# matiasrodlo/arxiv-rag

Measured on AMD Instinct MI355X. Metric: chunks embedded/sec + QPS@top-10, all-mpnet-base-v2 768-d, 1/2/4/8 MI355X, higher is better.
Workload: dtype bf16

## Files before the change

arxiv_rag_amd/_lib.py:

```python
from __future__ import annotations

import ctypes as C
import os
from pathlib import Path

_HERE = Path(__file__).resolve().parent
LIB_PATH = Path(os.environ.get("ARX_LIB", _HERE / "libarx_hip.so"))

K_CLASSES = ["search_groupmax", "gemm_qkv", "gemm_oproj", "gemm_fc1", "gemm_fc2", "attention",
             "layernorm", "embed", "pool", "search_select", "search_rescore", "gemm_raw"]


class EncoderConfigC(C.Structure):
    _fields_ = [(n, C.c_int32) for n in ("arch", "vocab_size", "hidden", "layers", "heads", "ffn", "max_pos",
                                         "pool", "pad_id", "rel_buckets", "rel_max_distance")] + [("ln_eps", C.c_float)]


class LayerWeightsC(C.Structure):
    _fields_ = [(n, C.c_void_p) for n in ("w_qkv", "b_qkv", "w_o", "b_o", "ln1_g", "ln1_b",
                                          "w_fc1", "b_fc1", "w_fc2", "b_fc2", "ln2_g", "ln2_b")]


class EncoderWeightsC(C.Structure):
    _fields_ = [(n, C.c_void_p) for n in ("word_emb", "pos_emb", "type_emb", "emb_ln_g", "emb_ln_b", "rel_bias")] \
               + [("layers", C.POINTER(LayerWeightsC))]


class TopkOptionsC(C.Structure):
    _fields_ = [("struct_bytes", C.c_int32), ("i8_max_queries", C.c_int32), ("max_row_norm", C.c_float), ("cu_limit", C.c_int32),
                ("flags", C.c_int32), ("debug_tau_mult", C.c_float), ("debug_drop_best", C.c_int32)]

    def __init__(self, **kw):
        super().__init__(**kw)
        self.struct_bytes = C.sizeof(TopkOptionsC)


class PairHeadC(C.Structure):
    _fields_ = [("struct_bytes", C.c_int32), ("n_labels", C.c_int32)] \
               + [(n, C.c_void_p) for n in ("type_emb", "pooler_w", "pooler_b", "cls_w", "cls_b")]

    def __init__(self, **kw):
        super().__init__(**kw)
        self.struct_bytes = C.sizeof(PairHeadC)


class GemmEpilogueC(C.Structure):
    _fields_ = [("struct_bytes", C.c_int32), ("mode", C.c_int32), ("variant", C.c_int32), ("eps", C.c_float)] \
               + [(n, C.c_void_p) for n in ("bias", "resid", "a_mean", "a_rstd", "s_vec", "r_mean", "r_rstd", "r_gamma", "r_beta")] \
               + [("row_cap", C.c_int64), ("part_sum", C.c_void_p), ("part_sq", C.c_void_p), ("part_ld", C.c_int64),
                  ("out_mean", C.c_void_p), ("out_rstd", C.c_void_p), ("n_rows", C.c_void_p)]

    def __init__(self, **kw):
        super().__init__(**kw)
        self.struct_bytes = C.sizeof(GemmEpilogueC)


TOPK_NO_PERSISTENT, TOPK_SCAN_ONLY, TOPK_TAIL_ONLY, TOPK_NO_SINGLE_ROW_TAIL, TOPK_I8_CENTRE_QUERY = 1, 2, 4, 8, 16


EXPORTS = {
    "arx_version": (C.c_int32, []),
    "arx_last_error": (C.c_char_p, []),
    "arx_build_info": (C.c_int32, []),
    "arx_mpnet_bucket": (C.c_int32, [C.c_int32, C.c_int32, C.c_int32]),
    "arx_encoder_workspace_bytes": (C.c_int64, [C.POINTER(EncoderConfigC), C.c_int32, C.c_int32]),
    "arx_encoder_create": (C.c_int32, [C.POINTER(EncoderConfigC), C.POINTER(EncoderWeightsC), C.c_int32, C.c_int32,
                                       C.POINTER(C.c_void_p)]),
    "arx_encoder_destroy": (None, [C.c_void_p]),
    "arx_encoder_forward": (C.c_int32, [C.c_void_p, C.c_void_p, C.c_int32, C.c_void_p, C.c_int32, C.c_int32, C.c_int32,
                                        C.c_void_p, C.c_int64, C.c_void_p, C.c_int64, C.c_int32, C.c_void_p]),
    "arx_encoder_attention": (C.c_int32, [C.c_void_p, C.c_void_p, C.c_void_p, C.c_int32, C.c_int32, C.c_void_p, C.c_void_p]),
    "arx_encoder_set_tap": (C.c_int32, [C.c_void_p, C.c_int32]),
    "arx_encoder_set_low_latency": (C.c_int32, [C.c_void_p, C.c_int32]),
    "arx_encoder_debug_hidden": (C.c_int32, [C.c_void_p, C.c_int32, C.c_void_p, C.c_int32, C.c_void_p]),
    "arx_encoder_set_pair_head": (C.c_int32, [C.c_void_p, C.POINTER(PairHeadC)]),
    "arx_encoder_score_pairs": (C.c_int32, [C.c_void_p, C.c_void_p, C.c_int32, C.c_void_p, C.c_void_p, C.c_int32, C.c_int32, C.c_int32,
                                            C.c_void_p, C.c_int64, C.c_void_p]),
    "arx_encoder_debug_cls": (C.c_int32, [C.c_void_p, C.c_void_p, C.c_int32, C.c_void_p]),
    "arx_pair_head_forward": (C.c_int32, [C.c_void_p, C.c_int64, C.c_int32, C.c_int32, C.POINTER(PairHeadC), C.c_void_p, C.c_int64,
                                          C.c_void_p]),
    "arx_topk_workspace_bytes": (C.c_int64, [C.c_int64, C.c_int32, C.c_int32, C.c_int32]),
    "arx_topk_search": (C.c_int32, [C.c_void_p, C.c_int64, C.c_void_p, C.c_int32, C.c_int32, C.c_int32, C.c_void_p,
                                    C.c_void_p, C.c_int64, C.c_void_p, C.c_int64, C.c_void_p]),
    "arx_topk_i8_index_bytes": (C.c_int64, [C.c_int64, C.c_int32]),
    "arx_topk_i8_index_info": (C.c_int32, [C.c_void_p, C.c_int64, C.c_int32, C.POINTER(C.c_float), C.c_void_p]),
    "arx_topk_build_i8": (C.c_int32, [C.c_void_p, C.c_int64, C.c_int32, C.c_void_p, C.c_void_p]),
    "arx_topk_search_i8": (C.c_int32, [C.c_void_p, C.c_void_p, C.c_int64, C.c_void_p, C.c_int32, C.c_int32, C.c_int32, C.c_void_p,
                                       C.c_void_p, C.c_int64, C.c_void_p, C.c_int64, C.c_void_p]),
    "arx_topk_workspace_bytes_i8": (C.c_int64, [C.c_int64, C.c_int32, C.c_int32, C.c_int32]),
    "arx_topk_search_opt": (C.c_int32, [C.c_void_p, C.c_void_p, C.c_int64, C.c_void_p, C.c_int32, C.c_int32, C.c_int32, C.c_void_p,
                                        C.c_void_p, C.c_int64, C.c_void_p, C.c_int64, C.POINTER(TopkOptionsC), C.c_void_p]),
    "arx_rows_max_norm_f16": (C.c_int32, [C.c_void_p, C.c_int64, C.c_int32, C.c_void_p, C.c_void_p]),
    "arx_stream_create_cu_mask": (C.c_int32, [C.POINTER(C.c_uint32), C.c_int32, C.POINTER(C.c_void_p)]),
    "arx_stream_destroy": (C.c_int32, [C.c_void_p]),
    "arx_device_cu_count": (C.c_int32, []),
    "arx_debug_cu_census": (C.c_int32, [C.c_void_p, C.c_int32, C.c_int32, C.c_void_p]),
    "arx_topk_stats": (C.c_int32, [C.c_void_p, C.POINTER(C.c_int64), C.POINTER(C.c_int64), C.c_void_p]),
    "arx_topk_merge": (C.c_int32, [C.c_void_p, C.c_void_p, C.c_int32, C.c_int32, C.c_int32, C.c_void_p, C.c_void_p,
                                   C.c_void_p]),
    "arx_topk_filtered_workspace_bytes": (C.c_int64, [C.c_int64, C.c_int32, C.c_int32, C.c_int32]),
    "arx_topk_search_filtered": (C.c_int32, [C.c_void_p, C.c_int64, C.c_void_p, C.c_int64, C.c_void_p, C.c_int32, C.c_int32, C.c_int32,
                                             C.c_void_p, C.c_void_p, C.c_int64, C.c_float, C.c_void_p, C.c_int64, C.c_void_p]),
    "arx_topk_search_filtered_tuned": (C.c_int32, [C.c_void_p, C.c_int64, C.c_void_p, C.c_int64, C.c_void_p, C.c_int32, C.c_int32, C.c_int32,
                                                   C.c_void_p, C.c_void_p, C.c_int64, C.c_float, C.c_void_p, C.c_int64, C.c_int32, C.c_int32,
                                                   C.c_void_p]),
    "arx_topk_filtered_stats": (C.c_int32, [C.c_void_p, C.POINTER(C.c_int64), C.POINTER(C.c_int64), C.c_void_p]),
    "arx_topk_prefix_workspace_bytes": (C.c_int64, [C.c_int64, C.c_int32, C.c_int32, C.c_int32]),
    "arx_topk_search_prefix": (C.c_int32, [C.c_void_p, C.c_int64, C.c_void_p, C.c_void_p, C.c_int32, C.c_int32, C.c_int32, C.c_void_p,
                                           C.c_void_p, C.c_int64, C.c_float, C.c_void_p, C.c_int64, C.c_void_p]),
    "arx_topk_search_prefix_tuned": (C.c_int32, [C.c_void_p, C.c_int64, C.c_void_p, C.c_void_p, C.c_int32, C.c_int32, C.c_int32, C.c_void_p,
                                                 C.c_void_p, C.c_int64, C.c_float, C.c_void_p, C.c_int64, C.c_int32, C.c_int32, C.c_void_p]),
    "arx_topk_prefix_stats": (C.c_int32, [C.c_void_p, C.POINTER(C.c_int64), C.POINTER(C.c_int64), C.c_void_p]),
    "arx_text_contains": (C.c_int32, [C.c_void_p, C.c_void_p, C.c_int64, C.c_void_p, C.c_void_p, C.c_int32, C.c_void_p, C.c_void_p]),
    "arx_bitmap_count": (C.c_int32, [C.c_void_p, C.c_int64, C.c_void_p, C.c_void_p]),
    "arx_gather_rows": (C.c_int32, [C.c_void_p, C.c_int64, C.c_int32, C.c_int64, C.c_void_p, C.c_int64, C.c_void_p, C.c_void_p]),
    "arx_mmr_select": (C.c_int32, [C.c_void_p, C.c_void_p, C.c_void_p, C.c_int32, C.c_int32, C.c_int32, C.c_int32, C.c_float, C.c_void_p,
                                   C.c_void_p, C.c_void_p]),
    "arx_bm25_workspace_bytes": (C.c_int64, [C.c_int64, C.c_int32, C.c_int32]),
    "arx_bm25_search": (C.c_int32, [C.c_void_p, C.c_void_p, C.c_void_p, C.c_int32, C.c_int64, C.c_void_p, C.c_void_p, C.c_int32, C.c_int32,
                                    C.c_void_p, C.c_void_p, C.c_int64, C.c_void_p, C.c_int64, C.c_void_p]),
    "arx_bm25_search_tuned": (C.c_int32, [C.c_void_p, C.c_void_p, C.c_void_p, C.c_int32, C.c_int64, C.c_void_p, C.c_void_p, C.c_int32,
                                          C.c_int32, C.c_void_p, C.c_void_p, C.c_int64, C.c_void_p, C.c_int64, C.c_int32, C.c_int32,
                                          C.c_void_p]),
    "arx_bm25_scores": (C.c_int32, [C.c_void_p, C.c_void_p, C.c_void_p, C.c_int32, C.c_int64, C.c_void_p, C.c_int32, C.c_int64, C.c_int64,
                                    C.c_int32, C.c_void_p, C.c_void_p]),
    "arx_gemm_bf16": (C.c_int32, [C.c_void_p, C.c_void_p, C.c_void_p, C.c_void_p, C.c_void_p, C.c_int32, C.c_int32, C.c_int32,
                                  C.c_int32, C.c_int32, C.c_void_p]),
    "arx_gemm_bf16_ex": (C.c_int32, [C.c_void_p, C.c_void_p, C.c_void_p, C.c_int32, C.c_int32, C.c_int32, C.POINTER(GemmEpilogueC),
                                     C.c_void_p]),
    "arx_fold_ln": (C.c_int32, [C.c_void_p, C.c_void_p, C.c_void_p, C.c_void_p, C.c_void_p, C.c_void_p, C.c_void_p, C.c_int32, C.c_int32,
                                C.c_void_p]),
    "arx_prof_classes": (C.c_int32, [C.c_uint32]),
    "arx_wp_create": (C.c_int32, [C.c_char_p, C.c_void_p, C.c_int32, C.c_int32, C.c_int32, C.c_int32, C.c_int32, C.c_int32, C.c_int32,
                                  C.c_char_p, C.c_void_p, C.c_int32, C.POINTER(C.c_void_p)]),
    "arx_wp_destroy": (None, [C.c_void_p]),
    "arx_wp_encode": (C.c_int32, [C.c_void_p, C.c_char_p, C.c_void_p, C.c_int64, C.c_int32, C.c_void_p, C.c_void_p, C.c_void_p, C.c_int32]),
    "arx_wp_miss_count": (C.c_int32, [C.c_void_p, C.POINTER(C.c_int64), C.POINTER(C.c_int64)]),
    "arx_wp_miss_fetch": (C.c_int32, [C.c_void_p, C.c_void_p, C.c_void_p]),
    "arx_wp_cache_add": (C.c_int32, [C.c_void_p, C.c_char_p, C.c_void_p, C.c_int64, C.c_void_p, C.c_void_p]),
    "arx_wp_cache_size": (C.c_int64, [C.c_void_p]),
    "arx_wp_version": (C.c_int32, []),
    "arx_adjacent_cosine": (C.c_int32, [C.c_void_p, C.c_int64, C.c_int32, C.c_int32, C.c_void_p, C.c_void_p]),
    "arx_f32_to_bf16": (C.c_int32, [C.c_void_p, C.c_void_p, C.c_int64, C.c_void_p]),
    "arx_fill_unit_rows_f16": (C.c_int32, [C.c_void_p, C.c_int64, C.c_int32, C.c_uint64, C.c_void_p]),
    "arx_fill_unit_rows_f16_at": (C.c_int32, [C.c_void_p, C.c_int64, C.c_int32, C.c_uint64, C.c_int64, C.c_void_p]),
    "arx_fill_clustered_rows_f16_at": (C.c_int32, [C.c_void_p, C.c_int64, C.c_int32, C.c_uint64, C.c_int64, C.c_int32, C.c_float, C.c_int32,
                                                   C.c_float, C.c_void_p]),
    "arx_prof_enable": (C.c_int32, [C.c_int32]),
    "arx_prof_reset": (C.c_int32, []),
    "arx_prof_read": (C.c_int32, [C.c_int32, C.POINTER(C.c_float), C.POINTER(C.c_int32)]),
}

_lib = None


class ArxError(RuntimeError):
    pass


def load():
    global _lib
    if _lib is not None:
        return _lib
    if not LIB_PATH.exists():
        raise ArxError(
            f"{LIB_PATH} not found: the HIP extension is not built. Run `python -c 'import __graft_entry__ as g; "
            f"g.build()'` (or arxiv_rag_amd/csrc/build.sh). There is no CPU fallback for this path.")
    lib = C.CDLL(str(LIB_PATH))
    for name, (res, args) in EXPORTS.items():
        fn = getattr(lib, name)
        fn.restype = res
        fn.argtypes = args
    _lib = lib
    return lib


def check(rc: int, what: str = ""):
    if rc != 0:
        msg = load().arx_last_error().decode("utf-8", "replace")
        raise ArxError(f"{what} failed (rc={rc}): {msg}")


def prof_classes(names=None):
    mask = 0xFFFFFFFF if names is None else sum(1 << K_CLASSES.index(n) for n in names)
    check(load().arx_prof_classes(mask), "arx_prof_classes")


def prof_enable(on: bool):
    check(load().arx_prof_enable(1 if on else 0), "arx_prof_enable")


def prof_reset():
    check(load().arx_prof_reset(), "arx_prof_reset")


def prof_read():
    lib = load()
    out = {}
    for i, name in enumerate(K_CLASSES):
        ms, n = C.c_float(0), C.c_int32(0)
        check(lib.arx_prof_read(i, C.byref(ms), C.byref(n)), "arx_prof_read")
        out[name] = (float(ms.value), int(n.value))
    return out
```

arxiv_rag_amd/csrc/encoder.hip:

```cpp
#include <math.h>
#include <stdlib.h>
#include <string.h>

#include <mutex>
#include <vector>

#include "arx_common.h"
#include "encoder_kernels.h"
#include "gemm.h"
#include "gemm8.h"
#include "gemm_small.h"

extern "C" int32_t arx_mpnet_bucket(int32_t rel, int32_t num_buckets, int32_t max_distance) {
    int n = -rel;
    const int nb = num_buckets / 2;
    int ret = 0;
    if (n < 0) { ret = nb; n = -n; }
    const int max_exact = nb / 2;
    if (n < max_exact) return ret + n;
    int v = max_exact + (int)floor(log((double)n / max_exact) / log((double)max_distance / max_exact) * (nb - max_exact) + 1e-6);
    if (v > nb - 1) v = nb - 1;
    return ret + v;
}

struct arx_encoder {
    arx_encoder_config cfg;
    arx_encoder_weights w;
    std::vector<arx_layer_weights> layers;
    int max_tokens, max_seqs, tok_pad;
    char* ws = nullptr;
    int64_t ws_bytes = 0;
    int32_t* cu = nullptr;
    uint16_t *x = nullptr, *x1 = nullptr, *qkv = nullptr, *ctx = nullptr, *y = nullptr, *hbuf = nullptr;
    float* bias_tbl = nullptr;
    uint16_t* tap = nullptr;
    int tap_layer = -1;
    int ln_fold = 1;
    char* fold_ws = nullptr;
    std::vector<uint16_t*> wqkv_f, wfc1_f;
    std::vector<float*> s_qkv, c_qkv, s_fc1, c_fc1;
    float *st1_sum = nullptr, *st1_sq = nullptr, *st2_sum = nullptr, *st2_sq = nullptr;
    float *part_s = nullptr, *part_q = nullptr;
    int variant = 89;
    int low_latency = 0;
    float* small_ws = nullptr;
    int attn_variant = 1;
    int attn_dev_word = 0;
    unsigned long long* attn_stamps = nullptr;
    arx_pair_head pair{};
    int has_pair = 0;
    float* cls_ws = nullptr;
};

struct WsLayout {
    int64_t cu, x, x1, qkv, ctx, y, hbuf, bias, stats, total;
};
static WsLayout ws_layout(const arx_encoder_config& c, int max_tokens, int max_seqs) {
    const int64_t tp = round_up64(max_tokens, 256);
    WsLayout l;
    int64_t o = 0;
    auto take = [&](int64_t bytes) { int64_t r = o; o += round_up64(bytes, 256); return r; };
    l.cu = take((int64_t)(max_seqs + 1) * 4);
    l.x = take(tp * c.hidden * 2);
    l.x1 = take(tp * c.hidden * 2);
    l.qkv = take(tp * c.hidden * 3 * 2);
    l.ctx = take(tp * c.hidden * 2);
    l.y = take(tp * c.hidden * 2);
    l.hbuf = take(tp * c.ffn * 2);
    l.bias = take((int64_t)c.heads * ARX_BIAS_ROW * 4);
    l.stats = take(tp * 4 * 4 + 2 * (int64_t)(c.hidden / 64) * tp * 4);
    l.total = o;
    return l;
}

static int check_cfg(const arx_encoder_config* c) {
    ARX_REQUIRE(c != nullptr, "cfg is null");
    ARX_REQUIRE(c->arch == ARX_ARCH_MPNET || c->arch == ARX_ARCH_BERT, "unknown arch %d", c->arch);
    ARX_REQUIRE(c->hidden > 0 && c->hidden % 64 == 0 && c->hidden <= 1024, "hidden=%d must be a multiple of 64, <= 1024", c->hidden);
    ARX_REQUIRE(c->heads > 0 && c->hidden % c->heads == 0, "hidden %% heads != 0");
    const int dh = c->hidden / c->heads;
    ARX_REQUIRE(dh == 32 || dh == 64, "head_dim=%d unsupported (32 or 64)", dh);
    ARX_REQUIRE(c->ffn > 0 && c->ffn % 64 == 0, "ffn=%d must be a multiple of 64", c->ffn);
    ARX_REQUIRE(c->layers > 0 && c->vocab_size > 0 && c->max_pos > 0, "bad layers/vocab/max_pos");
    ARX_REQUIRE(c->pool == ARX_POOL_MEAN || c->pool == ARX_POOL_CLS, "unknown pool %d", c->pool);
    return ARX_OK;
}

extern "C" int64_t arx_encoder_workspace_bytes(const arx_encoder_config* cfg, int32_t max_tokens, int32_t max_seqs) {
    if (check_cfg(cfg) != ARX_OK || max_tokens <= 0 || max_seqs <= 0) return -1;
    return ws_layout(*cfg, max_tokens, max_seqs).total;
}

extern "C" int32_t arx_encoder_create(const arx_encoder_config* cfg, const arx_encoder_weights* w, int32_t max_tokens,
                                      int32_t max_seqs, arx_encoder** out) {
    int rc = check_cfg(cfg);
    if (rc != ARX_OK) return rc;
    ARX_REQUIRE(w && out, "null weights/out");
    ARX_REQUIRE(max_tokens > 0 && max_seqs > 0, "max_tokens/max_seqs must be positive");
    ARX_REQUIRE(w->word_emb && w->pos_emb && w->emb_ln_g && w->emb_ln_b && w->layers, "missing embedding weights");
    ARX_REQUIRE(cfg->arch != ARX_ARCH_BERT || w->type_emb, "BERT needs type_emb");
    ARX_REQUIRE(cfg->arch != ARX_ARCH_MPNET || w->rel_bias, "MPNet needs rel_bias");
    for (int i = 0; i < cfg->layers; ++i) {
        const arx_layer_weights& L = w->layers[i];
        ARX_REQUIRE(L.w_qkv && L.b_qkv && L.w_o && L.b_o && L.ln1_g && L.ln1_b && L.w_fc1 && L.b_fc1 && L.w_fc2 &&
                        L.b_fc2 && L.ln2_g && L.ln2_b, "layer %d: missing weights", i);
    }
    arx_encoder* h = new arx_encoder();
    auto fail = [&](int code) {
        if (h->ws) (void)hipFree(h->ws);
        if (h->fold_ws) (void)hipFree(h->fold_ws);
        delete h;
        return code;
    };
    h->cfg = *cfg;
    h->w = *w;
    h->layers.assign(w->layers, w->layers + cfg->layers);
    h->w.layers = h->layers.data();
    h->max_tokens = max_tokens;
    h->max_seqs = max_seqs;
    h->tok_pad = (int)round_up64(max_tokens, 256);
    const char* e = getenv("ARX_GEMM_VARIANT");
    h->variant = e ? atoi(e) : 89;
    const char* av = getenv("ARX_ATTN_VARIANT");
    h->attn_variant = av ? atoi(av) : 1;
#ifdef ARX_DEV_VARIANTS
    const char* g = getenv("ARX_GEMM_GLDS");
    if (g && g[0] == '0') h->variant = 4;
#endif
    const WsLayout l = ws_layout(*cfg, max_tokens, max_seqs);
    hipError_t he = hipMalloc((void**)&h->ws, l.total);
    if (he != hipSuccess) {
        arx_set_error("hipMalloc(%lld bytes workspace): %s", (long long)l.total, hipGetErrorString(he));
        h->ws = nullptr;
        return fail(ARX_ERR_HIP);
    }
    h->ws_bytes = l.total;
    (void)hipMemset(h->ws, 0, l.total);
    h->cu = (int32_t*)(h->ws + l.cu);
    h->x = (uint16_t*)(h->ws + l.x);
    h->x1 = (uint16_t*)(h->ws + l.x1);
    h->qkv = (uint16_t*)(h->ws + l.qkv);
    h->ctx = (uint16_t*)(h->ws + l.ctx);
    h->y = (uint16_t*)(h->ws + l.y);
    h->hbuf = (uint16_t*)(h->ws + l.hbuf);
    h->bias_tbl = (float*)(h->ws + l.bias);
    {
        const int64_t tp = round_up64(max_tokens, 256);
        float* st = (float*)(h->ws + l.stats);
        h->st1_sum = st; h->st1_sq = st + tp; h->st2_sum = st + 2 * tp; h->st2_sq = st + 3 * tp;
        h->part_s = st + 4 * tp; h->part_q = h->part_s + (int64_t)(cfg->hidden / 64) * tp;
    }
    const char* lf = getenv("ARX_LN_FOLD");
    h->ln_fold = lf ? atoi(lf) : 1;
    if (h->ln_fold) {
        const int64_t H = cfg->hidden, F = cfg->ffn, Lc = cfg->layers;
        const int64_t per = round_up64(3 * H * H * 2, 256) + round_up64(F * H * 2, 256) + 2 * round_up64(3 * H * 4, 256) + 2 * round_up64(F * 4, 256);
        he = hipMalloc((void**)&h->fold_ws, per * Lc);
        if (he != hipSuccess) {
            arx_set_error("hipMalloc(folded weights): %s", hipGetErrorString(he));
            h->fold_ws = nullptr;
            return fail(ARX_ERR_HIP);
        }
        char* pws = h->fold_ws;
        auto takep = [&](int64_t bytes) { char* r = pws; pws += round_up64(bytes, 256); return r; };
        for (int i = 0; i < Lc; ++i) {
            const arx_layer_weights& L = h->layers[i];
            uint16_t* wq = (uint16_t*)takep(3 * H * H * 2); uint16_t* w1 = (uint16_t*)takep(F * H * 2);
            float* sq = (float*)takep(3 * H * 4); float* cq = (float*)takep(3 * H * 4);
            float* s1 = (float*)takep(F * 4); float* c1 = (float*)takep(F * 4);
            h->wqkv_f.push_back(wq); h->wfc1_f.push_back(w1);
            h->s_qkv.push_back(sq); h->c_qkv.push_back(cq); h->s_fc1.push_back(s1); h->c_fc1.push_back(c1);
            fold_ln_kernel<<<cdiv(F, 4), 256>>>((const uint16_t*)L.w_fc1, L.ln1_g, L.ln1_b, L.b_fc1, w1, s1, c1, (int)F, (int)H);
            if (i > 0) {
                const arx_layer_weights& P = h->layers[i - 1];
                fold_ln_kernel<<<cdiv(3 * H, 4), 256>>>((const uint16_t*)L.w_qkv, P.ln2_g, P.ln2_b, L.b_qkv, wq, sq, cq, (int)(3 * H), (int)H);
            }
        }
        he = hipDeviceSynchronize();
        if (he != hipSuccess) {
            arx_set_error("fold_ln_kernel: %s", hipGetErrorString(he));
            return fail(ARX_ERR_HIP);
        }
    }
    if (cfg->arch == ARX_ARCH_MPNET) {
        std::vector<float> rb((size_t)cfg->rel_buckets * cfg->heads);
        he = hipMemcpy(rb.data(), w->rel_bias, rb.size() * 4, hipMemcpyDeviceToHost);
        if (he != hipSuccess) {
            arx_set_error("copy rel_bias: %s", hipGetErrorString(he));
            return fail(ARX_ERR_HIP);
        }
        std::vector<float> tbl((size_t)cfg->heads * ARX_BIAS_ROW);
        const float log2e = 1.4426950408889634f;
        for (int d = -ARX_BIAS_CENTER; d <= ARX_BIAS_CENTER; ++d) {
            const int bk = arx_mpnet_bucket(d, cfg->rel_buckets, cfg->rel_max_distance);
            for (int hd = 0; hd < cfg->heads; ++hd)
                tbl[(size_t)hd * ARX_BIAS_ROW + d + ARX_BIAS_CENTER] = rb[(size_t)bk * cfg->heads + hd] * log2e;
        }
        he = hipMemcpy(h->bias_tbl, tbl.data(), tbl.size() * 4, hipMemcpyHostToDevice);
        if (he != hipSuccess) {
            arx_set_error("upload bias table: %s", hipGetErrorString(he));
            return fail(ARX_ERR_HIP);
        }
    }
    *out = h;
    return ARX_OK;
}

extern "C" void arx_encoder_destroy(arx_encoder* h) {
    if (!h) return;
    if (h->ws) (void)hipFree(h->ws);
    if (h->tap) (void)hipFree(h->tap);
    if (h->fold_ws) (void)hipFree(h->fold_ws);
    if (h->small_ws) (void)hipFree(h->small_ws);
    if (h->cls_ws) (void)hipFree(h->cls_ws);
    delete h;
}

extern "C" int32_t arx_encoder_set_low_latency(arx_encoder* h, int32_t on) {
    ARX_REQUIRE(h, "null handle");
    if (on && !h->small_ws) ARX_HIP_CHECK(hipMalloc((void**)&h->small_ws, ARX_SMALL_WS_BYTES));
    h->low_latency = on ? 1 : 0;
    return ARX_OK;
}

extern "C" int32_t arx_encoder_set_tap(arx_encoder* h, int32_t layer) {
    ARX_REQUIRE(h, "null handle");
    ARX_REQUIRE(layer >= -1 && layer <= h->cfg.layers, "tap layer out of range");
    if (layer >= 0 && !h->tap) ARX_HIP_CHECK(hipMalloc((void**)&h->tap, (int64_t)h->tok_pad * h->cfg.hidden * 2));
    h->tap_layer = layer;
    return ARX_OK;
}

extern "C" int32_t arx_encoder_debug_hidden(arx_encoder* h, int32_t , float* dst, int32_t n_tokens, void* stream) {
    ARX_REQUIRE(h && h->tap && dst, "no tap recorded");
    ARX_REQUIRE(n_tokens > 0 && n_tokens <= h->max_tokens, "n_tokens out of range");
    const int64_t n = (int64_t)n_tokens * h->cfg.hidden;
    bf16_to_f32_kernel<<<cdiv(n, 256), 256, 0, (hipStream_t)stream>>>(h->tap, dst, n);
    ARX_HIP_CHECK(hipGetLastError());
    return ARX_OK;
}

template <typename Kern>
static int launch_gemm_kernel(Kern kern, int smem, int threads, int BM, int BN, const uint16_t* A, int64_t lda,
                              const uint16_t* W, int64_t ldw, int M, int N, int K, const EpiParams& ep, hipStream_t st) {
    ARX_HIP_CHECK(arx_func_smem((const void*)kern, smem));
    const int tm = cdiv(M, BM), tn = cdiv(N, BN);
    kern<<<tm * tn, threads, smem, st>>>((const bf16_t*)A, lda, (const bf16_t*)W, ldw, M, N, K, tm, tn, ep);
    ARX_HIP_CHECK(hipGetLastError());
    return ARX_OK;
}

static bool fits_u32_offsets(int64_t M, int64_t lda, int64_t N, int64_t ldw, const EpiParams& ep) {
    return M * lda < (1ll << 31) && N * ldw < (1ll << 31) && M * ep.ldc < (1ll << 32) && (!ep.resid || M * ep.ldr < (1ll << 32));
}

template <int MODE>
int arx_launch_gemm(int variant, const uint16_t* A, int64_t lda, const uint16_t* W, int64_t ldw, int M, int N, int K,
                    const EpiParams& ep, hipStream_t st) {
    if (K % 64 != 0 || N % 8 != 0) {
        arx_set_error("gemm: K=%d must be a multiple of 64 and N=%d of 8", K, N);
        return ARX_ERR_ARG;
    }
    const bool wide = (N % 256 == 0);
    const bool wide8 = (N % 128 == 0 && N >= 256);
#ifdef ARX_DEV_VARIANTS
    if constexpr (MODE <= EPI_BIAS_RESID) {
        if (variant == 0) {
            if (wide) return launch_gemm_kernel(gemm_bf16_kernel<256, 256, 2, 4, true, MODE>, GemmMainloop<bf16_t, 256, 256, 2, 4, true>::SMEM_BYTES, 512, 256, 256, A, lda, W, ldw, M, N, K, ep, st);
            return launch_gemm_kernel(gemm_bf16_kernel<256, 128, 4, 2, true, MODE>, GemmMainloop<bf16_t, 256, 128, 4, 2, true>::SMEM_BYTES, 512, 256, 128, A, lda, W, ldw, M, N, K, ep, st);
        }
        if (variant == 4) {
            if (wide) return launch_gemm_kernel(gemm_bf16_kernel<256, 256, 2, 4, false, MODE>, GemmMainloop<bf16_t, 256, 256, 2, 4, false>::SMEM_BYTES, 512, 256, 256, A, lda, W, ldw, M, N, K, ep, st);
            return launch_gemm_kernel(gemm_bf16_kernel<256, 128, 4, 2, false, MODE>, GemmMainloop<bf16_t, 256, 128, 4, 2, false>::SMEM_BYTES, 512, 256, 128, A, lda, W, ldw, M, N, K, ep, st);
        }
    }
#endif
    if (variant == 71)
        return launch_gemm_kernel(gemm_v0e2_kernel<128, 128, 2, 2, MODE, 67>, GemmMainloop<bf16_t, 128, 128, 2, 2, true, 67>::SMEM_BYTES, 256, 128, 128, A, lda, W, ldw, M, N, K, ep, st);
    if (variant == 89) variant = (K <= 1024) ? 9 : 8;
    if (variant == 9 && (K / 64) % 2 != 0) variant = 8;
    if ((variant == 8 || variant == 9) && wide8 && !fits_u32_offsets(M, lda, N, ldw, ep)) {
        static bool said = false;
        if (!said) {
            said = true;
            fprintf(stderr, "[arx] gemm M=%d N=%d K=%d: operand or output offsets exceed 32 bits, using the 2-stage kernel (64-bit offsets)\n", M, N, K);
        }
        variant = 13;
    }
    if (variant == 9 && wide8) {
        auto kern = gemm_8phase_persistent_kernel<MODE>;
        ARX_HIP_CHECK(arx_func_smem((const void*)kern, Gemm8Phase<bf16_t, 0>::SMEM_BYTES));
        const int n_cu = arx_device_cus();
        const int tm = cdiv(M, 256), tn = cdiv(N, 256);
        int grid = TileWalk::grid(tm, tn) < n_cu ? TileWalk::grid(tm, tn) : n_cu;
        grid = grid / 8 * 8 > 0 ? grid / 8 * 8 : grid;
        kern<<<grid, 512, Gemm8Phase<bf16_t, 0>::SMEM_BYTES, st>>>((const bf16_t*)A, lda, (const bf16_t*)W, ldw, M, N, K, tm, tn, ep);
        ARX_HIP_CHECK(hipGetLastError());
        return ARX_OK;
    }
    if (variant == 8 && wide8) {
        auto kern = gemm_8phase_kernel<MODE>;
        ARX_HIP_CHECK(arx_func_smem((const void*)kern, Gemm8Phase<bf16_t, 0>::SMEM_BYTES));
        const int tm = cdiv(M, 256), tn = cdiv(N, 256);
        kern<<<TileWalk::grid(tm, tn), 512, Gemm8Phase<bf16_t, 0>::SMEM_BYTES, st>>>((const bf16_t*)A, lda, (const bf16_t*)W, ldw, M, N, K, tm, tn, ep);
        ARX_HIP_CHECK(hipGetLastError());
        return ARX_OK;
    }
#ifdef ARX_DEV_VARIANTS
    if (variant == 34 && wide)
        return launch_gemm_kernel(gemm_v0e2_kernel<256, 256, 2, 4, MODE, 64 + 4096>, GemmMainloop<bf16_t, 256, 256, 2, 4, true, 64 + 4096>::SMEM_BYTES, 512, 256, 256, A, lda, W, ldw, M, N, K, ep, st);
    if (variant == 33 && wide)
        return launch_gemm_kernel(gemm_a3w2_kernel<256, 256, 2, 4, MODE>, 3 * 256 * 128 + 2 * 256 * 128, 512, 256, 256, A, lda, W, ldw, M, N, K, ep, st);
    if (variant == 1) {
        if (wide) return launch_gemm_kernel(gemm_v0e2_kernel<256, 256, 2, 4, MODE>, GemmMainloop<bf16_t, 256, 256, 2, 4, true>::SMEM_BYTES, 512, 256, 256, A, lda, W, ldw, M, N, K, ep, st);
        return launch_gemm_kernel(gemm_v0e2_kernel<256, 128, 4, 2, MODE>, GemmMainloop<bf16_t, 256, 128, 4, 2, true>::SMEM_BYTES, 512, 256, 128, A, lda, W, ldw, M, N, K, ep, st);
    }
    if (variant == 15 && wide)
        return launch_gemm_kernel(gemm_v0e2_kernel<256, 256, 2, 4, MODE, 3>, GemmMainloop<bf16_t, 256, 256, 2, 4, true, 3>::SMEM_BYTES, 512, 256, 256, A, lda, W, ldw, M, N, K, ep, st);
    if (variant == 3 && wide)
        return launch_gemm_kernel(gemm_ring_kernel<256, 256, 2, 4, 4, MODE>, GemmRing<bf16_t, 256, 256, 2, 4, 4>::SMEM_BYTES, 512, 256, 256, A, lda, W, ldw, M, N, K, ep, st);
    if (variant == 2 || variant == 3)
        return launch_gemm_kernel(gemm_ring_kernel<256, 128, 2, 2, 3, MODE>, GemmRing<bf16_t, 256, 128, 2, 2, 3>::SMEM_BYTES, 256, 256, 128, A, lda, W, ldw, M, N, K, ep, st);
#endif
    if (!wide) return launch_gemm_kernel(gemm_v0e2_kernel<256, 128, 4, 2, MODE, 67>, GemmMainloop<bf16_t, 256, 128, 4, 2, true, 67>::SMEM_BYTES, 512, 256, 128, A, lda, W, ldw, M, N, K, ep, st);
    return launch_gemm_kernel(gemm_v0e2_kernel<256, 256, 2, 4, MODE, 67>, GemmMainloop<bf16_t, 256, 256, 2, 4, true, 67>::SMEM_BYTES, 512, 256, 256, A, lda, W, ldw, M, N, K, ep, st);
}

template <int MODE>
static int launch_gemm(int cls, int variant, const uint16_t* A, int64_t lda, const uint16_t* W, int64_t ldw, int M, int N, int K,
                       const EpiParams& ep, hipStream_t st, float* small_ws = nullptr) {
    ProfScope ps(cls, st);
    if (variant == 70) return launch_gemm_small<MODE>(A, lda, W, ldw, M, N, K, ep, small_ws, st);
#ifdef ARX_DEV_VARIANTS
    static const int dev_bw = getenv("ARX_DEV_BW") ? atoi(getenv("ARX_DEV_BW")) : 0;
    const char* stg = getenv("ARX_DEV_STAGGER");
    if (dev_bw || stg) {
        EpiParams e2 = ep; e2.dev_bw = dev_bw;
        if (stg) { int a = 0, b = 8, c = 0; sscanf(stg, "%d,%d,%d", &a, &b, &c); e2.dev_stagger = a; e2.dev_slots = b > 0 ? b : 8; e2.dev_store = c; }
        return arx_launch_gemm<MODE>(variant, A, lda, W, ldw, M, N, K, e2, st);
    }
#endif
    return arx_launch_gemm<MODE>(variant, A, lda, W, ldw, M, N, K, ep, st);
}

extern "C" int32_t arx_gemm_bf16(const void* A, const void* W, const float* bias, const void* resid, void* C, int32_t M,
                                 int32_t N, int32_t K, int32_t mode, int32_t variant, void* stream) {
    ARX_REQUIRE(A && W && bias && C, "null pointer argument");
    ARX_REQUIRE(M > 0 && N > 0 && K > 0, "bad sizes");
    ARX_REQUIRE(mode != EPI_BIAS_RESID || resid, "mode 2 needs resid");
    EpiParams ep{(uint16_t*)C, N, bias, (const uint16_t*)resid, N};
    hipStream_t st = (hipStream_t)stream;
#ifdef ARX_DEV_VARIANTS
    ep.dev_store = (variant / 100) % 10; ep.dev_bw = variant / 1000; variant %= 100;
    if (const char* stg = getenv("ARX_DEV_STAGGER")) { int a = 0, b = 8; sscanf(stg, "%d,%d", &a, &b); ep.dev_stagger = a; ep.dev_slots = b > 0 ? b : 8; }
#endif
#ifdef ARX_STAMP
    {
        static unsigned long long* d = nullptr;
        const int tiles = cdiv(M, 256) * cdiv(N, 256);
        if (!d) ARX_HIP_CHECK(hipMalloc(&d, (size_t)8 * 32 * 2 * 16384));
        if (getenv("ARX_STAMP_DUMP") && tiles <= 16384) {
            ep.stamps = d;
            int rc = ARX_ERR_ARG;
            if (mode == EPI_BIAS) rc = arx_launch_gemm<EPI_BIAS>(variant, (const uint16_t*)A, K, (const uint16_t*)W, K, M, N, K, ep, st);
            if (mode == EPI_BIAS_GELU) rc = arx_launch_gemm<EPI_BIAS_GELU>(variant, (const uint16_t*)A, K, (const uint16_t*)W, K, M, N, K, ep, st);
            if (mode == EPI_BIAS_RESID) rc = arx_launch_gemm<EPI_BIAS_RESID>(variant, (const uint16_t*)A, K, (const uint16_t*)W, K, M, N, K, ep, st);
            ARX_HIP_CHECK(hipStreamSynchronize(st));
            std::vector<unsigned long long> hbuf((size_t)tiles * 64);
            ARX_HIP_CHECK(hipMemcpy(hbuf.data(), d, hbuf.size() * 8, hipMemcpyDeviceToHost));
            double loop[2] = {0, 0}, epi[2] = {0, 0}, pro[2] = {0, 0}, x45[2] = {0, 0}, x67[2] = {0, 0};
            unsigned long long tmin = ~0ull, tmax = 0;
            for (int t = 0; t < tiles; ++t)
                for (int g = 0; g < 2; ++g) {
                    const unsigned long long* o = &hbuf[((size_t)t * 2 + g) * 32];
                    loop[g] += (double)(o[1] - o[3]); epi[g] += (double)(o[2] - o[1]); pro[g] += (double)(o[3] - o[0]);
                    if (variant == 9) { x45[g] += (double)(o[5] - o[4]); x67[g] += (double)(o[7] - o[6]); }
                    else x45[g] += (double)(o[4] - o[2]);
                    tmin = o[0] < tmin ? o[0] : tmin; tmax = o[2] > tmax ? o[2] : tmax;
                }
            if (variant == 9) {
                double gap = 0, period = 0; int n = 0;
                for (int t = 0; t + 256 < tiles; ++t) { const unsigned long long* a = &hbuf[(size_t)t * 64]; const unsigned long long* b = &hbuf[(size_t)(t + 256) * 64];
                    gap += (double)(b[0] - a[2]); period += (double)(b[0] - a[0]); ++n; }
                if (n) fprintf(stderr, "[stamp] persistent: g0 tile period %.0f clk, epilogue-end -> next loop start %.0f clk\n", period / n, gap / n);
            }
            if (const char* sf = getenv("ARX_STAMP_FILE")) {
                if (FILE* f = fopen(sf, "wb")) { fwrite(hbuf.data(), 8, hbuf.size(), f); fclose(f); }
            }
            if (variant == 9) {
                const int nkt = K / 64 < 16 ? K / 64 : 16;
                fprintf(stderr, "[stamp] k-tile durations g0:");
                for (int k = 0; k + 1 < nkt; ++k) { double a = 0; int n = 0; for (int t = 256; t < tiles; ++t) { const unsigned long long* o = &hbuf[(size_t)t * 64]; a += (double)(o[9 + k] - o[8 + k]); ++n; } fprintf(stderr, " %.0f", a / (n ? n : 1)); }
                fprintf(stderr, "\n");
            }
            fprintf(stderr, "[stamp] %s g0 %.0f g1 %.0f clk%s g0 %.0f g1 %.0f\n", variant == 9 ? "wait at k-tile 0:" : "store drain after the epilogue:", x45[0] / tiles, x45[1] / tiles,
                    variant == 9 ? ", at k-tile 1:" : " (-)", x67[0] / tiles, x67[1] / tiles);
            fprintf(stderr, "[stamp] M=%d N=%d K=%d mode=%d tiles=%d: prologue %.0f / %.0f, loop g0 %.0f g1 %.0f clk, epilogue g0 %.0f g1 %.0f clk, span %.0f clk, tiles/CU %.1f\n",
                    M, N, K, mode, tiles, pro[0] / tiles, pro[1] / tiles, loop[0] / tiles, loop[1] / tiles, epi[0] / tiles, epi[1] / tiles, (double)(tmax - tmin), tiles / 256.0);
            return rc;
        }
    }
#endif
    ProfScope ps(ARX_K_GEMM_RAW, st);
    if (variant == 70) {
        float* ws = nullptr;
        ARX_HIP_CHECK(hipMallocAsync((void**)&ws, ARX_SMALL_WS_BYTES, st));
        int rc = ARX_ERR_ARG;
        switch (mode) {
        case EPI_BIAS: rc = launch_gemm_small<EPI_BIAS>((const uint16_t*)A, K, (const uint16_t*)W, K, M, N, K, ep, ws, st); break;
        case EPI_BIAS_GELU: rc = launch_gemm_small<EPI_BIAS_GELU>((const uint16_t*)A, K, (const uint16_t*)W, K, M, N, K, ep, ws, st); break;
        case EPI_BIAS_RESID: rc = launch_gemm_small<EPI_BIAS_RESID>((const uint16_t*)A, K, (const uint16_t*)W, K, M, N, K, ep, ws, st); break;
        default: arx_set_error("unknown gemm mode %d", mode);
        }
        (void)hipFreeAsync(ws, st);
        return rc;
    }
    switch (mode) {
    case EPI_BIAS: return arx_launch_gemm<EPI_BIAS>(variant, (const uint16_t*)A, K, (const uint16_t*)W, K, M, N, K, ep, st);
    case EPI_BIAS_GELU: return arx_launch_gemm<EPI_BIAS_GELU>(variant, (const uint16_t*)A, K, (const uint16_t*)W, K, M, N, K, ep, st);
    case EPI_BIAS_RESID: return arx_launch_gemm<EPI_BIAS_RESID>(variant, (const uint16_t*)A, K, (const uint16_t*)W, K, M, N, K, ep, st);
    }
    arx_set_error("unknown gemm mode %d", mode);
    return ARX_ERR_ARG;
}

template <int DH, bool HB, int NW>
static int launch_attn_cfg(arx_encoder* h, int n_seqs, int max_len, hipStream_t st) {
    auto kern = attention_kernel<DH, HB, NW>;
    const int Lk = (max_len + 31) & ~31;
    const int smem = AttnSmem<DH>::total(Lk, HB);
    ARX_HIP_CHECK(arx_func_smem((const void*)kern, smem));
    const float scale_log2e = 1.4426950408889634f / sqrtf((float)DH);
    dim3 grid(cdiv(max_len, 32 * NW), h->cfg.heads, n_seqs);
    ProfScope ps(ARX_K_ATTENTION, st);
    kern<<<grid, NW * 64, smem, st>>>(h->qkv, h->ctx, h->cu, h->bias_tbl, h->cfg.hidden, scale_log2e);
    ARX_HIP_CHECK(hipGetLastError());
    return ARX_OK;
}

template <int DH, bool HB, int NW>
static int launch_attn_tr_cfg(arx_encoder* h, int n_seqs, int max_len, hipStream_t st) {
    auto kern = attention_tr_kernel<DH, HB, NW>;
    const int Lk = (max_len + 31) & ~31;
    const int smem = AttnSmem3<DH>::total(Lk, HB);
    ARX_HIP_CHECK(arx_func_smem((const void*)kern, smem));
    const float scale_log2e = 1.4426950408889634f / sqrtf((float)DH);
    dim3 grid(cdiv(max_len, 32 * NW), h->cfg.heads, n_seqs);
    ProfScope ps(ARX_K_ATTENTION, st);
    kern<<<grid, NW * 64, smem, st>>>(h->qkv, h->ctx, h->cu, h->bias_tbl, h->cfg.hidden, scale_log2e, h->attn_dev_word, h->attn_stamps);
    ARX_HIP_CHECK(hipGetLastError());
    return ARX_OK;
}

#ifdef ARX_DEV_VARIANTS
template <int DH, bool HB, int NSLOT>
static int launch_attn_ring_cfg(arx_encoder* h, int n_seqs, int max_len, hipStream_t st) {
    auto kern = attention_ring_kernel<DH, HB, NSLOT>;
    const int C0 = (max_len + 31) & ~31;
    const int smem = AttnRing<DH, NSLOT>::total(C0, HB);
    ARX_HIP_CHECK(arx_func_smem((const void*)kern, smem));
    int G = arx_device_cus() / h->cfg.heads;
    G = G < 1 ? 1 : (G > n_seqs ? n_seqs : G);
    const float scale_log2e = 1.4426950408889634f / sqrtf((float)DH);
    ProfScope ps(ARX_K_ATTENTION, st);
    kern<<<G * h->cfg.heads, 512, smem, st>>>(h->qkv, h->ctx, h->cu, h->bias_tbl, h->cfg.hidden, n_seqs, C0, scale_log2e);
    ARX_HIP_CHECK(hipGetLastError());
    return ARX_OK;
}

template <bool HB>
static int launch_attn_ring16_cfg(arx_encoder* h, int n_seqs, int max_len, hipStream_t st) {
    auto kern = attention_ring16_kernel<HB>;
    const int C0 = (max_len + 31) & ~31;
    const int smem = AttnRing16<8>::total(C0, HB);
    ARX_HIP_CHECK(arx_func_smem((const void*)kern, smem));
    int G = arx_device_cus() / h->cfg.heads;
    G = G < 1 ? 1 : (G > n_seqs ? n_seqs : G);
    const float scale_log2e = 1.4426950408889634f / sqrtf(64.0f);
    ProfScope ps(ARX_K_ATTENTION, st);
    kern<<<G * h->cfg.heads, 1024, smem, st>>>(h->qkv, h->ctx, h->cu, h->bias_tbl, h->cfg.hidden, n_seqs, C0, scale_log2e);
    ARX_HIP_CHECK(hipGetLastError());
    return ARX_OK;
}

#endif

static int launch_attn(arx_encoder* h, int n_seqs, int max_len, hipStream_t st) {
    const int dh = h->cfg.hidden / h->cfg.heads;
    const bool hb = h->cfg.arch == ARX_ARCH_MPNET;
#ifdef ARX_DEV_VARIANTS
    if (h->attn_variant == 4 && dh == 64 && max_len > 128 && max_len <= 256)
        return hb ? launch_attn_ring16_cfg<true>(h, n_seqs, max_len, st) : launch_attn_ring16_cfg<false>(h, n_seqs, max_len, st);
    if (h->attn_variant == 2 && max_len > 128 && max_len <= 256) {
        if (dh == 64) return hb ? launch_attn_ring_cfg<64, true, 8>(h, n_seqs, max_len, st) : launch_attn_ring_cfg<64, false, 8>(h, n_seqs, max_len, st);
        return hb ? launch_attn_ring_cfg<32, true, 8>(h, n_seqs, max_len, st) : launch_attn_ring_cfg<32, false, 8>(h, n_seqs, max_len, st);
    }
#endif
    if (h->attn_variant >= 1) {
        const bool w8 = max_len > 128;
        if (dh == 64) {
            if (hb) return w8 ? launch_attn_tr_cfg<64, true, 8>(h, n_seqs, max_len, st) : launch_attn_tr_cfg<64, true, 4>(h, n_seqs, max_len, st);
            return w8 ? launch_attn_tr_cfg<64, false, 8>(h, n_seqs, max_len, st) : launch_attn_tr_cfg<64, false, 4>(h, n_seqs, max_len, st);
        }
        if (hb) return w8 ? launch_attn_tr_cfg<32, true, 8>(h, n_seqs, max_len, st) : launch_attn_tr_cfg<32, true, 4>(h, n_seqs, max_len, st);
        return w8 ? launch_attn_tr_cfg<32, false, 8>(h, n_seqs, max_len, st) : launch_attn_tr_cfg<32, false, 4>(h, n_seqs, max_len, st);
    }
    const bool big = max_len > 256;
    if (dh == 64) {
        if (hb) return big ? launch_attn_cfg<64, true, 8>(h, n_seqs, max_len, st) : launch_attn_cfg<64, true, 4>(h, n_seqs, max_len, st);
        return big ? launch_attn_cfg<64, false, 8>(h, n_seqs, max_len, st) : launch_attn_cfg<64, false, 4>(h, n_seqs, max_len, st);
    }
    if (hb) return big ? launch_attn_cfg<32, true, 8>(h, n_seqs, max_len, st) : launch_attn_cfg<32, true, 4>(h, n_seqs, max_len, st);
    return big ? launch_attn_cfg<32, false, 8>(h, n_seqs, max_len, st) : launch_attn_cfg<32, false, 4>(h, n_seqs, max_len, st);
}

extern "C" int32_t arx_encoder_attention(arx_encoder* h, const void* qkv, const int32_t* lens, int32_t n_seqs, int32_t max_len,
                                         void* ctx, void* stream) {
    ARX_REQUIRE(h && qkv && lens && ctx, "null pointer argument");
    ARX_REQUIRE(n_seqs > 0 && n_seqs <= h->max_seqs && max_len > 0 && max_len <= 512, "bad n_seqs/max_len");
    hipStream_t st = (hipStream_t)stream;
    scan_lens_kernel<<<1, 256, 0, st>>>(lens, h->cu, n_seqs);
    ARX_HIP_CHECK(hipGetLastError());
    uint16_t* q0 = h->qkv; uint16_t* c0 = h->ctx;
    h->qkv = (uint16_t*)qkv; h->ctx = (uint16_t*)ctx;
    const int rc = launch_attn(h, n_seqs, max_len, st);
    h->qkv = q0; h->ctx = c0;
    return rc;
}

static void launch_ln_finalize(int T, int nparts, const float* ps, const float* pq, int64_t ld, const int32_t* n_rows, float inv_h,
                               float eps, float* mean, float* rstd, hipStream_t st) {
    const int grid = cdiv(T, 256);
    switch (nparts) {
    case 6: ln_finalize_kernel<6><<<grid, 256, 0, st>>>(ps, pq, ld, nparts, n_rows, inv_h, eps, mean, rstd); break;
    case 12: ln_finalize_kernel<12><<<grid, 256, 0, st>>>(ps, pq, ld, nparts, n_rows, inv_h, eps, mean, rstd); break;
    case 16: ln_finalize_kernel<16><<<grid, 256, 0, st>>>(ps, pq, ld, nparts, n_rows, inv_h, eps, mean, rstd); break;
    default: ln_finalize_kernel<0><<<grid, 256, 0, st>>>(ps, pq, ld, nparts, n_rows, inv_h, eps, mean, rstd); break;
    }
}

template <int MODE>
static int gemm_ex_run(int variant, const uint16_t* A, const uint16_t* W, int M, int N, int K, const EpiParams& ep, const arx_gemm_epilogue* e,
                       hipStream_t st) {
    constexpr bool STATS = (MODE == EPI_RESID_STATS || MODE == EPI_LNRESID_STATS);
    int rc;
    if (variant == 70) {
        float* ws = nullptr;
        ARX_HIP_CHECK(hipMallocAsync((void**)&ws, ARX_SMALL_WS_BYTES, st));
        rc = launch_gemm<MODE>(ARX_K_GEMM_RAW, variant, A, K, W, K, M, N, K, ep, st, ws);
        (void)hipFreeAsync(ws, st);
        return rc;
    }
    if ((rc = launch_gemm<MODE>(ARX_K_GEMM_RAW, variant, A, K, W, K, M, N, K, ep, st)) != ARX_OK) return rc;
    if (STATS) {
        launch_ln_finalize(M, N / 64, e->part_sum, e->part_sq, e->part_ld, e->n_rows, ep.inv_h, ep.eps, e->out_mean, e->out_rstd, st);
        ARX_HIP_CHECK(hipGetLastError());
    }
    return ARX_OK;
}

extern "C" int32_t arx_gemm_bf16_ex(const void* A, const void* W, void* C, int32_t M, int32_t N, int32_t K, const arx_gemm_epilogue* e,
                                    void* stream) {
    ARX_REQUIRE(A && W && C && e, "null pointer argument");
    ARX_REQUIRE(e->struct_bytes == (int32_t)sizeof(arx_gemm_epilogue), "arx_gemm_epilogue: struct_bytes=%d, this library expects %d",
                e->struct_bytes, (int)sizeof(arx_gemm_epilogue));
    ARX_REQUIRE(M > 0 && N > 0 && K > 0, "bad sizes");
    ARX_REQUIRE(K % 64 == 0 && N % 8 == 0, "gemm: K=%d must be a multiple of 64 and N=%d of 8", K, N);
    const int mode = e->mode, variant = e->variant;
    ARX_REQUIRE(mode >= EPI_BIAS && mode <= EPI_LNRESID_STATS, "unknown gemm mode %d", mode);
    ARX_REQUIRE(variant == 89 || variant == 8 || variant == 9 || variant == 13 || variant == 70 || variant == 71,
                "gemm variant %d is not a shipped schedule (89, 8, 9, 13, 70, 71)", variant);
    const bool ln_in = (mode == EPI_LN_BIAS || mode == EPI_LN_BIAS_GELU), stats = (mode == EPI_RESID_STATS || mode == EPI_LNRESID_STATS);
    const bool staged = (variant == 89 || variant == 8 || variant == 9);
    ARX_REQUIRE(e->bias, "mode %d needs bias", mode);
    ARX_REQUIRE(!(mode == EPI_BIAS_RESID || stats) || e->resid, "mode %d needs resid", mode);
    ARX_REQUIRE(!ln_in || (e->a_mean && e->a_rstd && e->s_vec), "mode %d needs a_mean, a_rstd and s_vec", mode);
    ARX_REQUIRE(mode != EPI_LNRESID_STATS || (e->r_mean && e->r_rstd && e->r_gamma && e->r_beta), "mode 6 needs r_mean, r_rstd, r_gamma and r_beta");
    if (ln_in || mode == EPI_LNRESID_STATS)
        ARX_REQUIRE(e->row_cap >= (staged ? round_up64(M, 256) : (int64_t)M),
                    "row_cap=%lld: the row vectors must be readable up to row %lld (M=%d%s)", (long long)e->row_cap,
                    (long long)(staged ? round_up64(M, 256) : (int64_t)M), M, staged ? " rounded up to 256: variants 89, 8, 9 stage whole tiles" : "");
    if (stats) {
        ARX_REQUIRE(N % 64 == 0, "statistics modes need N %% 64 == 0 (one partial per 64-column slice), N=%d", N);
        ARX_REQUIRE(e->out_mean && e->out_rstd, "mode %d needs out_mean and out_rstd", mode);
        if (variant != 70) ARX_REQUIRE(e->part_sum && e->part_sq && e->part_ld >= M && e->n_rows,
                                       "mode %d on a tile kernel needs part_sum, part_sq, part_ld >= M and n_rows", mode);
    }
    if (variant == 70) {
        ARX_REQUIRE(M <= ARX_SMALL_M && N % 64 == 0, "small-batch gemm: M=%d (<= %d) N=%d (%% 64)", M, ARX_SMALL_M, N);
        ARX_REQUIRE(!stats || N <= 1024, "small-batch gemm: statistics modes take N <= 1024, N=%d", N);
    }
    EpiParams ep{(uint16_t*)C, N, e->bias, (const uint16_t*)e->resid, N};
    ep.a_sum = e->a_mean; ep.a_sq = e->a_rstd; ep.s_vec = e->s_vec;
    ep.r_sum = e->r_mean; ep.r_sq = e->r_rstd; ep.r_gamma = e->r_gamma; ep.r_beta = e->r_beta;
    ep.o_sum = e->part_sum; ep.o_sq = e->part_sq; ep.o_ld = e->part_ld;
    ep.fin_mean = e->out_mean; ep.fin_rstd = e->out_rstd;
    ep.inv_h = 1.0f / (float)N; ep.eps = e->eps;
    hipStream_t st = (hipStream_t)stream;
    const uint16_t* a = (const uint16_t*)A; const uint16_t* w = (const uint16_t*)W;
    switch (mode) {
    case EPI_BIAS: return gemm_ex_run<EPI_BIAS>(variant, a, w, M, N, K, ep, e, st);
    case EPI_BIAS_GELU: return gemm_ex_run<EPI_BIAS_GELU>(variant, a, w, M, N, K, ep, e, st);
    case EPI_BIAS_RESID: return gemm_ex_run<EPI_BIAS_RESID>(variant, a, w, M, N, K, ep, e, st);
    case EPI_LN_BIAS: return gemm_ex_run<EPI_LN_BIAS>(variant, a, w, M, N, K, ep, e, st);
    case EPI_LN_BIAS_GELU: return gemm_ex_run<EPI_LN_BIAS_GELU>(variant, a, w, M, N, K, ep, e, st);
    case EPI_RESID_STATS: return gemm_ex_run<EPI_RESID_STATS>(variant, a, w, M, N, K, ep, e, st);
    default: return gemm_ex_run<EPI_LNRESID_STATS>(variant, a, w, M, N, K, ep, e, st);
    }
}

extern "C" int32_t arx_fold_ln(const void* W, const float* gamma, const float* beta, const float* bias, void* Wf, float* s, float* c,
                               int32_t N, int32_t K, void* stream) {
    ARX_REQUIRE(W && gamma && beta && bias && Wf && s && c, "null pointer argument");
    ARX_REQUIRE(N > 0 && K > 0, "bad sizes");
    fold_ln_kernel<<<cdiv(N, 4), 256, 0, (hipStream_t)stream>>>((const uint16_t*)W, gamma, beta, bias, (uint16_t*)Wf, s, c, (int)N, (int)K);
    ARX_HIP_CHECK(hipGetLastError());
    return ARX_OK;
}

static int32_t encoder_run(arx_encoder* h, const int32_t* ids, int32_t seq_stride, const int32_t* lens, const int32_t* seg_b,
                           int32_t n_seqs, int32_t max_len, int32_t total_tokens, float* out_f32,
                           int64_t out_stride, void* out_f16, int64_t out16_stride, int32_t normalize,
                           void* stream) {
    ARX_REQUIRE(h && ids && lens, "null handle/ids/lens");
    ARX_REQUIRE(out_f32 || out_f16, "no output buffer");
    ARX_REQUIRE(n_seqs > 0 && max_len > 0 && max_len <= 512, "n_seqs=%d max_len=%d (max_len must be in 1..512)", n_seqs, max_len);
    ARX_REQUIRE(seq_stride >= max_len, "seq_stride < max_len");
    ARX_REQUIRE(total_tokens > 0 && (int64_t)total_tokens <= (int64_t)n_seqs * max_len, "total_tokens out of range");
    if (n_seqs > h->max_seqs || total_tokens > h->max_tokens) {
        arx_set_error("batch (%d seqs, %d tokens) exceeds handle capacity (%d, %d)", n_seqs, total_tokens, h->max_seqs, h->max_tokens);
        return ARX_ERR_CAPACITY;
    }
    ARX_REQUIRE(!out_f32 || out_stride >= h->cfg.hidden, "out_stride < hidden");
    ARX_REQUIRE(!out_f16 || out16_stride >= h->cfg.hidden, "out16_stride < hidden");
    hipStream_t st = (hipStream_t)stream;
    const arx_encoder_config& c = h->cfg;
    const int H = c.hidden, F = c.ffn, T = total_tokens;
    int rc;

    scan_lens_kernel<<<1, 256, 0, st>>>(lens, h->cu, n_seqs);
    ARX_HIP_CHECK(hipGetLastError());
    {
        ProfScope ps(ARX_K_EMBED, st);
        dim3 grid(cdiv(max_len, 4), n_seqs);
        if (c.arch == ARX_ARCH_MPNET)
            embed_ln_kernel<ARX_ARCH_MPNET><<<grid, 256, 0, st>>>(ids, seq_stride, lens, h->cu, h->w.word_emb, h->w.pos_emb, nullptr,
                                                                  h->w.emb_ln_g, h->w.emb_ln_b, h->x, H, c.vocab_size, c.max_pos, c.pad_id, c.ln_eps);
        else if (seg_b)
            embed_ln_kernel<ARX_ARCH_BERT, true><<<grid, 256, 0, st>>>(ids, seq_stride, lens, h->cu, h->w.word_emb, h->w.pos_emb,
                                                                       h->pair.type_emb, h->w.emb_ln_g, h->w.emb_ln_b, h->x, H,
                                                                       c.vocab_size, c.max_pos, c.pad_id, c.ln_eps, seg_b);
        else
            embed_ln_kernel<ARX_ARCH_BERT><<<grid, 256, 0, st>>>(ids, seq_stride, lens, h->cu, h->w.word_emb, h->w.pos_emb, h->w.type_emb,
                                                                 h->w.emb_ln_g, h->w.emb_ln_b, h->x, H, c.vocab_size, c.max_pos, c.pad_id, c.ln_eps);
        ARX_HIP_CHECK(hipGetLastError());
    }
    const int ln_grid = cdiv(T, 4);
    const int64_t tp = round_up64(h->max_tokens, 256);
    if (!h->ln_fold) {
        auto tap = [&](int layer) -> int {
            if (h->tap_layer == layer && h->tap) ARX_HIP_CHECK(hipMemcpyAsync(h->tap, h->x, (int64_t)T * H * 2, hipMemcpyDeviceToDevice, st));
            return ARX_OK;
        };
        if ((rc = tap(0)) != ARX_OK) return rc;
        for (int li = 0; li < c.layers; ++li) {
            const arx_layer_weights& L = h->layers[li];
            EpiParams ep;
            ep = EpiParams{h->qkv, 3 * (int64_t)H, L.b_qkv, nullptr, 0};
            if ((rc = launch_gemm<EPI_BIAS>(ARX_K_GEMM_QKV, h->variant, h->x, H, (const uint16_t*)L.w_qkv, H, T, 3 * H, H, ep, st)) != ARX_OK) return rc;
            if ((rc = launch_attn(h, n_seqs, max_len, st)) != ARX_OK) return rc;
            ep = EpiParams{h->y, H, L.b_o, h->x, H};
            if ((rc = launch_gemm<EPI_BIAS_RESID>(ARX_K_GEMM_OPROJ, h->variant, h->ctx, H, (const uint16_t*)L.w_o, H, T, H, H, ep, st)) != ARX_OK) return rc;
            { ProfScope ps(ARX_K_LAYERNORM, st);
              layernorm_kernel<<<ln_grid, 256, 0, st>>>(h->y, h->x1, L.ln1_g, L.ln1_b, h->cu + n_seqs, H, c.ln_eps); }
            ARX_HIP_CHECK(hipGetLastError());
            ep = EpiParams{h->hbuf, F, L.b_fc1, nullptr, 0};
            if ((rc = launch_gemm<EPI_BIAS_GELU>(ARX_K_GEMM_FC1, h->variant, h->x1, H, (const uint16_t*)L.w_fc1, H, T, F, H, ep, st)) != ARX_OK) return rc;
            ep = EpiParams{h->y, H, L.b_fc2, h->x1, H};
            if ((rc = launch_gemm<EPI_BIAS_RESID>(ARX_K_GEMM_FC2, h->variant, h->hbuf, F, (const uint16_t*)L.w_fc2, F, T, H, F, ep, st)) != ARX_OK) return rc;
            { ProfScope ps(ARX_K_LAYERNORM, st);
              layernorm_kernel<<<ln_grid, 256, 0, st>>>(h->y, h->x, L.ln2_g, L.ln2_b, h->cu + n_seqs, H, c.ln_eps); }
            ARX_HIP_CHECK(hipGetLastError());
            if ((rc = tap(li + 1)) != ARX_OK) return rc;
        }
        ProfScope pps(ARX_K_POOL, st);
        pool_norm_kernel<<<n_seqs, 256, 0, st>>>(h->x, h->cu, H, c.pool, normalize, out_f32, out_stride, (f16_t*)out_f16, out16_stride,
                                                 nullptr, nullptr, nullptr, nullptr, 0.f);
        ARX_HIP_CHECK(hipGetLastError());
        return ARX_OK;
    }

    const float inv_h = 1.0f / (float)H;
    const int gv = !h->low_latency ? h->variant : (T <= ARX_SMALL_M ? 70 : (T <= ARX_MEDIUM_M ? 71 : h->variant));
    if (h->tap_layer == 0 && h->tap) ARX_HIP_CHECK(hipMemcpyAsync(h->tap, h->x, (int64_t)T * H * 2, hipMemcpyDeviceToDevice, st));
    for (int li = 0; li < c.layers; ++li) {
        const arx_layer_weights& L = h->layers[li];
        EpiParams ep;
        if (li == 0) {
            ep = EpiParams{h->qkv, 3 * (int64_t)H, L.b_qkv, nullptr, 0};
            if ((rc = launch_gemm<EPI_BIAS>(ARX_K_GEMM_QKV, gv, h->x, H, (const uint16_t*)L.w_qkv, H, T, 3 * H, H, ep, st, h->small_ws)) != ARX_OK) return rc;
        } else {
            ep = EpiParams{h->qkv, 3 * (int64_t)H, h->c_qkv[li], nullptr, 0};
            ep.a_sum = h->st2_sum; ep.a_sq = h->st2_sq; ep.s_vec = h->s_qkv[li]; ep.inv_h = inv_h; ep.eps = c.ln_eps;
            if ((rc = launch_gemm<EPI_LN_BIAS>(ARX_K_GEMM_QKV, gv, h->x, H, h->wqkv_f[li], H, T, 3 * H, H, ep, st, h->small_ws)) != ARX_OK) return rc;
        }
        if ((rc = launch_attn(h, n_seqs, max_len, st)) != ARX_OK) return rc;
        ep = EpiParams{h->x1, H, L.b_o, h->x, H};
        ep.o_sum = h->part_s; ep.o_sq = h->part_q; ep.o_ld = tp; ep.inv_h = inv_h; ep.eps = c.ln_eps;
        ep.fin_mean = h->st1_sum; ep.fin_rstd = h->st1_sq;
        if (li == 0) {
            if ((rc = launch_gemm<EPI_RESID_STATS>(ARX_K_GEMM_OPROJ, gv, h->ctx, H, (const uint16_t*)L.w_o, H, T, H, H, ep, st, h->small_ws)) != ARX_OK) return rc;
        } else {
            const arx_layer_weights& P = h->layers[li - 1];
            ep.r_sum = h->st2_sum; ep.r_sq = h->st2_sq; ep.r_gamma = P.ln2_g; ep.r_beta = P.ln2_b;
            if ((rc = launch_gemm<EPI_LNRESID_STATS>(ARX_K_GEMM_OPROJ, gv, h->ctx, H, (const uint16_t*)L.w_o, H, T, H, H, ep, st, h->small_ws)) != ARX_OK) return rc;
        }
        if (gv != 70) { ProfScope ps(ARX_K_LAYERNORM, st);
          launch_ln_finalize(T, H / 64, h->part_s, h->part_q, tp, h->cu + n_seqs, inv_h, c.ln_eps, h->st1_sum, h->st1_sq, st); }
        ARX_HIP_CHECK(hipGetLastError());
        ep = EpiParams{h->hbuf, F, h->c_fc1[li], nullptr, 0};
        ep.a_sum = h->st1_sum; ep.a_sq = h->st1_sq; ep.s_vec = h->s_fc1[li]; ep.inv_h = inv_h; ep.eps = c.ln_eps;
        if ((rc = launch_gemm<EPI_LN_BIAS_GELU>(ARX_K_GEMM_FC1, gv, h->x1, H, h->wfc1_f[li], H, T, F, H, ep, st, h->small_ws)) != ARX_OK) return rc;
        ep = EpiParams{h->x, H, L.b_fc2, h->x1, H};
        ep.r_sum = h->st1_sum; ep.r_sq = h->st1_sq; ep.r_gamma = L.ln1_g; ep.r_beta = L.ln1_b;
        ep.o_sum = h->part_s; ep.o_sq = h->part_q; ep.o_ld = tp; ep.inv_h = inv_h; ep.eps = c.ln_eps;
        ep.fin_mean = h->st2_sum; ep.fin_rstd = h->st2_sq;
        if ((rc = launch_gemm<EPI_LNRESID_STATS>(ARX_K_GEMM_FC2, gv, h->hbuf, F, (const uint16_t*)L.w_fc2, F, T, H, F, ep, st, h->small_ws)) != ARX_OK) return rc;
        if (gv != 70) { ProfScope ps(ARX_K_LAYERNORM, st);
          launch_ln_finalize(T, H / 64, h->part_s, h->part_q, tp, h->cu + n_seqs, inv_h, c.ln_eps, h->st2_sum, h->st2_sq, st); }
        ARX_HIP_CHECK(hipGetLastError());
        if (h->tap_layer == li + 1 && h->tap) {
            layernorm_kernel<<<ln_grid, 256, 0, st>>>(h->x, h->tap, L.ln2_g, L.ln2_b, h->cu + n_seqs, H, c.ln_eps);
            ARX_HIP_CHECK(hipGetLastError());
        }
    }
    {
        const arx_layer_weights& Ll = h->layers[c.layers - 1];
        ProfScope pps(ARX_K_POOL, st);
        pool_norm_kernel<<<n_seqs, 256, 0, st>>>(h->x, h->cu, H, c.pool, normalize, out_f32, out_stride, (f16_t*)out_f16, out16_stride,
                                                 h->st2_sum, h->st2_sq, Ll.ln2_g, Ll.ln2_b, c.ln_eps);
        ARX_HIP_CHECK(hipGetLastError());
    }
    return ARX_OK;
}

extern "C" int32_t arx_encoder_forward(arx_encoder* h, const int32_t* ids, int32_t seq_stride, const int32_t* lens,
                                       int32_t n_seqs, int32_t max_len, int32_t total_tokens, float* out_f32,
                                       int64_t out_stride, void* out_f16, int64_t out16_stride, int32_t normalize,
                                       void* stream) {
    return encoder_run(h, ids, seq_stride, lens, nullptr, n_seqs, max_len, total_tokens, out_f32, out_stride, out_f16, out16_stride,
                       normalize, stream);
}

static int check_pair_head(const arx_pair_head* p, int hidden) {
    ARX_REQUIRE(p, "null pair head");
    ARX_REQUIRE(p->struct_bytes >= (int32_t)sizeof(arx_pair_head), "arx_pair_head.struct_bytes=%d < %d", p->struct_bytes,
                (int)sizeof(arx_pair_head));
    ARX_REQUIRE(p->n_labels >= 1 && p->n_labels <= 16, "n_labels=%d must be in 1..16", p->n_labels);
    ARX_REQUIRE(p->pooler_w && p->pooler_b && p->cls_w && p->cls_b, "pair head: missing pooler / classifier weights");
    ARX_REQUIRE(hidden > 0 && hidden <= 1024, "hidden=%d must be in 1..1024", hidden);
    return ARX_OK;
}

static int launch_pair_head(const float* cls, int64_t ld, int n, int H, const arx_pair_head& p, float* out, int64_t ld_out,
                            hipStream_t st) {
    const int smem = 2 * PH_ROWS * H * (int)sizeof(float);
    ARX_HIP_CHECK(arx_func_smem((const void*)pair_head_kernel, smem));
    pair_head_kernel<<<cdiv(n, PH_ROWS), 256, smem, st>>>(cls, ld, n, H, p.pooler_w, p.pooler_b, p.cls_w, p.cls_b, p.n_labels, out,
                                                            ld_out);
    ARX_HIP_CHECK(hipGetLastError());
    return ARX_OK;
}

extern "C" int32_t arx_encoder_set_pair_head(arx_encoder* h, const arx_pair_head* head) {
    ARX_REQUIRE(h, "null handle");
    ARX_REQUIRE(h->cfg.arch == ARX_ARCH_BERT && h->cfg.pool == ARX_POOL_CLS, "a pair head needs a BERT handle with CLS pooling");
    const int rc = check_pair_head(head, h->cfg.hidden);
    if (rc != ARX_OK) return rc;
    ARX_REQUIRE(head->type_emb, "pair head: missing token-type table");
    if (!h->cls_ws) ARX_HIP_CHECK(hipMalloc((void**)&h->cls_ws, (int64_t)h->max_seqs * h->cfg.hidden * sizeof(float)));
    h->pair = *head;
    h->has_pair = 1;
    return ARX_OK;
}

extern "C" int32_t arx_encoder_score_pairs(arx_encoder* h, const int32_t* ids, int32_t seq_stride, const int32_t* lens,
                                           const int32_t* seg_b, int32_t n_seqs, int32_t max_len, int32_t total_tokens,
                                           float* out_logits, int64_t out_stride, void* stream) {
    ARX_REQUIRE(h && out_logits, "null handle/out_logits");
    ARX_REQUIRE(h->has_pair, "no pair head set (arx_encoder_set_pair_head)");
    ARX_REQUIRE(out_stride >= h->pair.n_labels, "out_stride < n_labels");
    int rc = encoder_run(h, ids, seq_stride, lens, seg_b, n_seqs, max_len, total_tokens, h->cls_ws, h->cfg.hidden, nullptr, 0, 0,
                         stream);
    if (rc != ARX_OK) return rc;
    return launch_pair_head(h->cls_ws, h->cfg.hidden, n_seqs, h->cfg.hidden, h->pair, out_logits, out_stride, (hipStream_t)stream);
}

extern "C" int32_t arx_encoder_debug_cls(arx_encoder* h, float* dst, int32_t n, void* stream) {
    ARX_REQUIRE(h && h->cls_ws && dst, "no pair head set / null dst");
    ARX_REQUIRE(n > 0 && n <= h->max_seqs, "n out of range");
    ARX_HIP_CHECK(hipMemcpyAsync(dst, h->cls_ws, (int64_t)n * h->cfg.hidden * sizeof(float), hipMemcpyDeviceToDevice, (hipStream_t)stream));
    return ARX_OK;
}

extern "C" int32_t arx_pair_head_forward(const float* cls_rows, int64_t ld, int32_t n, int32_t hidden, const arx_pair_head* head,
                                         float* out_logits, int64_t out_stride, void* stream) {
    const int rc = check_pair_head(head, hidden);
    if (rc != ARX_OK) return rc;
    ARX_REQUIRE(n >= 0 && ld >= hidden && out_stride >= head->n_labels, "bad n / ld / out_stride");
    if (n == 0) return ARX_OK;
    ARX_REQUIRE(cls_rows && out_logits, "null cls_rows/out_logits");
    return launch_pair_head(cls_rows, ld, n, hidden, *head, out_logits, out_stride, (hipStream_t)stream);
}

#ifdef ARX_DEV_VARIANTS
extern "C" int32_t arx_dev_attn_set(arx_encoder* h, int32_t word, void* stamps) {
    h->attn_dev_word = word;
    h->attn_stamps = (unsigned long long*)stamps;
    return ARX_OK;
}
#endif

extern "C" int32_t arx_build_info(void) {
#ifdef ARX_DEV_VARIANTS
    return 1;
#else
    return 0;
#endif
}

extern "C" int32_t arx_adjacent_cosine(const float* emb, int64_t ld, int32_t n, int32_t dim, float* out, void* stream) {
    ARX_REQUIRE(n >= 0 && dim > 0 && dim % 4 == 0 && ld >= dim, "bad sizes (dim must be a multiple of 4)");
    if (n < 2) return ARX_OK;
    ARX_REQUIRE(emb && out, "null pointer argument");
    adjacent_cosine_kernel<<<cdiv(n - 1, 4), 256, 0, (hipStream_t)stream>>>(emb, ld, n, dim, out);
    ARX_HIP_CHECK(hipGetLastError());
    return ARX_OK;
}

extern "C" int32_t arx_f32_to_bf16(const float* src, void* dst, int64_t n, void* stream) {
    ARX_REQUIRE(src && dst && n >= 0, "bad args");
    if (n == 0) return ARX_OK;
    f32_to_bf16_kernel<<<cdiv(n, 256), 256, 0, (hipStream_t)stream>>>(src, (uint16_t*)dst, n);
    ARX_HIP_CHECK(hipGetLastError());
    return ARX_OK;
}
```

arxiv_rag_amd/csrc/encoder_kernels.h:

```cpp
#pragma once
#include <type_traits>

#include "arx_common.h"

__global__ void scan_lens_kernel(const int32_t* __restrict__ lens, int32_t* __restrict__ cu, int n) {
    __shared__ int32_t part[1024];
    const int tid = threadIdx.x, nt = blockDim.x;
    const int per = (n + nt - 1) / nt;
    const int b0 = tid * per, b1 = min(n, b0 + per);
    int s = 0;
    for (int b = b0; b < b1; ++b) s += lens[b];
    part[tid] = s;
    __syncthreads();
    if (tid == 0) {
        int run = 0;
        for (int i = 0; i < nt; ++i) { int v = part[i]; part[i] = run; run += v; }
        cu[n] = run;
    }
    __syncthreads();
    int run = part[tid];
    for (int b = b0; b < b1; ++b) { cu[b] = run; run += lens[b]; }
}

template <int ARCH, bool SEG = false>
__global__ __launch_bounds__(256) void embed_ln_kernel(const int32_t* __restrict__ ids, int seq_stride,
                                                        const int32_t* __restrict__ lens, const int32_t* __restrict__ cu,
                                                        const float* __restrict__ word, const float* __restrict__ pos,
                                                        const float* __restrict__ type0, const float* __restrict__ g,
                                                        const float* __restrict__ bta, uint16_t* __restrict__ x,
                                                        int H, int vocab, int max_pos, int pad_id, float eps,
                                                        const int32_t* __restrict__ seg_b = nullptr) {
    const int b = blockIdx.y, lane = threadIdx.x & 63, w = threadIdx.x >> 6;
    const int s = blockIdx.x * 4 + w;
    const int L = lens[b];
    if (s >= L) return;
    const int32_t* row = ids + (int64_t)b * seq_stride;
    int id = row[s];
    id = id < 0 ? 0 : (id >= vocab ? vocab - 1 : id);
    int pid;
    if (ARCH == ARX_ARCH_MPNET) {
        int cnt = 0;
        for (int c0 = 0; c0 <= s; c0 += 64) {
            const int i = c0 + lane;
            const bool np = (i <= s) && (row[i] != pad_id);
            cnt += __popcll(__ballot(np));
        }
        pid = (row[s] != pad_id) ? cnt + pad_id : pad_id;
    } else {
        pid = s;
    }
    pid = pid >= max_pos ? max_pos - 1 : pid;
    const float* wr = word + (int64_t)id * H;
    const float* pr = pos + (int64_t)pid * H;
    const float* tr = type0;
    if (SEG) tr += (s >= seg_b[b]) ? H : 0;
    f32x4 v[4];
    float sum = 0.f;
    const int nch = H >> 2;
#pragma unroll
    for (int c = 0; c < 4; ++c) {
        const int ch = lane + 64 * c;
        if (ch < nch) {
            f32x4 a = *reinterpret_cast<const f32x4*>(wr + ch * 4);
            const f32x4 p4 = *reinterpret_cast<const f32x4*>(pr + ch * 4);
            a += p4;
            if (ARCH == ARX_ARCH_BERT) a += *reinterpret_cast<const f32x4*>(tr + ch * 4);
            v[c] = a;
            sum += a[0] + a[1] + a[2] + a[3];
        } else {
            v[c] = f32x4{0.f, 0.f, 0.f, 0.f};
        }
    }
    const float mean = wave_sum(sum) / (float)H;
    float sq = 0.f;
#pragma unroll
    for (int c = 0; c < 4; ++c) {
        const int ch = lane + 64 * c;
        if (ch < nch) {
            const f32x4 d = v[c] - mean;
            sq += d[0] * d[0] + d[1] * d[1] + d[2] * d[2] + d[3] * d[3];
        }
    }
    const float rstd = rsqrtf(wave_sum(sq) / (float)H + eps);
    uint16_t* out = x + (int64_t)(cu[b] + s) * H;
#pragma unroll
    for (int c = 0; c < 4; ++c) {
        const int ch = lane + 64 * c;
        if (ch < nch) {
            const f32x4 gg = *reinterpret_cast<const f32x4*>(g + ch * 4);
            const f32x4 bb = *reinterpret_cast<const f32x4*>(bta + ch * 4);
            const f32x4 y = (v[c] - mean) * rstd * gg + bb;
            u32x2 o;
            o[0] = pack_bf16x2(y[0], y[1]); o[1] = pack_bf16x2(y[2], y[3]);
            *reinterpret_cast<u32x2*>(out + ch * 4) = o;
        }
    }
}

__global__ __launch_bounds__(256) void layernorm_kernel(const uint16_t* __restrict__ y, uint16_t* __restrict__ x,
                                                         const float* __restrict__ g, const float* __restrict__ bta,
                                                         const int32_t* __restrict__ n_rows_ptr, int H, float eps) {
    const int lane = threadIdx.x & 63;
    const int r = blockIdx.x * 4 + (threadIdx.x >> 6);
    if (r >= *n_rows_ptr) return;
    const uint16_t* in = y + (int64_t)r * H;
    const int nch = H >> 3;
    float v[2][8];
    float sum = 0.f;
#pragma unroll
    for (int c = 0; c < 2; ++c) {
        const int ch = lane + 64 * c;
        if (ch < nch) {
            const u32x4 q = *reinterpret_cast<const u32x4*>(in + ch * 8);
#pragma unroll
            for (int e = 0; e < 4; ++e) {
                unpack_bf16x2(q[e], v[c][2 * e], v[c][2 * e + 1]);
                sum += v[c][2 * e] + v[c][2 * e + 1];
            }
        }
    }
    const float mean = wave_sum(sum) / (float)H;
    float sq = 0.f;
#pragma unroll
    for (int c = 0; c < 2; ++c)
        if (lane + 64 * c < nch) {
#pragma unroll
            for (int e = 0; e < 8; ++e) { const float d = v[c][e] - mean; sq += d * d; }
        }
    const float rstd = rsqrtf(wave_sum(sq) / (float)H + eps);
    uint16_t* out = x + (int64_t)r * H;
#pragma unroll
    for (int c = 0; c < 2; ++c) {
        const int ch = lane + 64 * c;
        if (ch < nch) {
            const f32x4 g0 = *reinterpret_cast<const f32x4*>(g + ch * 8), g1 = *reinterpret_cast<const f32x4*>(g + ch * 8 + 4);
            const f32x4 b0 = *reinterpret_cast<const f32x4*>(bta + ch * 8), b1 = *reinterpret_cast<const f32x4*>(bta + ch * 8 + 4);
            float o[8];
#pragma unroll
            for (int e = 0; e < 4; ++e) {
                o[e] = (v[c][e] - mean) * rstd * g0[e] + b0[e];
                o[e + 4] = (v[c][e + 4] - mean) * rstd * g1[e] + b1[e];
            }
            u32x4 q;
            q[0] = pack_bf16x2(o[0], o[1]); q[1] = pack_bf16x2(o[2], o[3]);
            q[2] = pack_bf16x2(o[4], o[5]); q[3] = pack_bf16x2(o[6], o[7]);
            *reinterpret_cast<u32x4*>(out + ch * 8) = q;
        }
    }
}

template <int DH> struct AttnSmem {
    static __host__ __device__ int k_bytes(int Lk) { return Lk * DH * 2; }
    static __host__ __device__ int vt_stride(int Lk) { return Lk + 8; }
    static __host__ __device__ int vt_bytes(int Lk) { return DH * (Lk + 8) * 2; }
    static __host__ __device__ int bias_stride(int Lk) { return 2 * Lk + 8; }
    static __host__ __device__ int bias_bytes(int Lk, bool has) { return has ? 4 * (2 * Lk + 8) * 4 : 0; }
    static __host__ __device__ int total(int Lk, bool has) { return k_bytes(Lk) + vt_bytes(Lk) + bias_bytes(Lk, has); }
};

#define ARX_BIAS_CENTER 640
#define ARX_BIAS_ROW (2 * ARX_BIAS_CENTER + 1)

template <int DH, bool HAS_BIAS, int NW>
__global__ __launch_bounds__(NW * 64) void attention_kernel(const uint16_t* __restrict__ qkv, uint16_t* __restrict__ ctx,
                                                             const int32_t* __restrict__ cu,
                                                             const float* __restrict__ bias_tbl,
                                                             int H, float scale_log2e) {
    constexpr int NT = NW * 64;
    constexpr int CPR = DH / 8;
    constexpr int RPB = 256 / (DH * 2);
    constexpr int KS = DH / 16;
    constexpr int DB = DH / 32;
    extern __shared__ __attribute__((aligned(16))) char smem[];

    const int b = blockIdx.z, h = blockIdx.y;
    const int t0 = cu[b];
    const int L = cu[b + 1] - t0;
    const int q0 = blockIdx.x * (32 * NW);
    if (q0 >= L) return;
    const int Lk = (L + 31) & ~31;
    const int tid = threadIdx.x, lane = tid & 63, wid = tid >> 6;
    const int64_t ld = 3 * (int64_t)H;
    const uint16_t* Qg = qkv + (int64_t)t0 * ld + h * DH;
    const uint16_t* Kg = Qg + H;
    const uint16_t* Vg = Qg + 2 * H;

    char* Ks = smem;
    uint16_t* Vt = reinterpret_cast<uint16_t*>(smem + AttnSmem<DH>::k_bytes(Lk));
    float* Bs = reinterpret_cast<float*>(smem + AttnSmem<DH>::k_bytes(Lk) + AttnSmem<DH>::vt_bytes(Lk));
    const int vts = AttnSmem<DH>::vt_stride(Lk);
    const int bst = AttnSmem<DH>::bias_stride(Lk);

    for (int cid = tid; cid < Lk * CPR; cid += NT) {
        const int row = cid / CPR, pc = cid % CPR;
        const int c = pc ^ ((row / RPB) & (CPR - 1));
        u32x4 kv = u32x4{0u, 0u, 0u, 0u}, vv = u32x4{0u, 0u, 0u, 0u};
        if (row < L) {
            kv = *reinterpret_cast<const u32x4*>(Kg + (int64_t)row * ld + c * 8);
            vv = *reinterpret_cast<const u32x4*>(Vg + (int64_t)row * ld + pc * 8);
        }
        *reinterpret_cast<u32x4*>(Ks + (int64_t)cid * 16) = kv;
        const int k16 = row & 15;
        const int pos = (row & ~15) + (((k16 >> 2) & 1) << 3) + ((k16 >> 3) << 2) + (k16 & 3);
#pragma unroll
        for (int e = 0; e < 4; ++e) {
            Vt[(pc * 8 + 2 * e) * vts + pos] = (uint16_t)(vv[e] & 0xffffu);
            Vt[(pc * 8 + 2 * e + 1) * vts + pos] = (uint16_t)(vv[e] >> 16);
        }
    }
    if (HAS_BIAS) {
        const float* bt = bias_tbl + (int64_t)h * ARX_BIAS_ROW + ARX_BIAS_CENTER;
        for (int i = tid; i < 4 * bst; i += NT) {
            const int c = i / bst, j = i % bst;
            int d = j + c - Lk;
            d = d < -ARX_BIAS_CENTER ? -ARX_BIAS_CENTER : (d > ARX_BIAS_CENTER ? ARX_BIAS_CENTER : d);
            Bs[i] = bt[d];
        }
    }
    __syncthreads();

    const int qw = q0 + wid * 32;
    if (qw >= L) return;
    const int ql = lane & 31, hh = lane >> 5;
    const int q = qw + ql;
    const int qc = q < L ? q : L - 1;
    bf16x8 qf[KS];
#pragma unroll
    for (int ks = 0; ks < KS; ++ks)
        qf[ks] = *reinterpret_cast<const bf16x8*>(Qg + (int64_t)qc * ld + ks * 16 + hh * 8);

    f32x16 o[DB];
#pragma unroll
    for (int d = 0; d < DB; ++d)
#pragma unroll
        for (int r = 0; r < 16; ++r) o[d][r] = 0.f;
    float m_run = -INFINITY, l_run = 0.f;

    const int bc = (4 - (qc & 3)) & 3;
    const float* brow = Bs + bc * bst + (Lk - qc - bc);
    const int krow_sw = ((ql / RPB) & (CPR - 1));

    const int nkt = Lk >> 5;
    for (int kt = 0; kt < nkt; ++kt) {
        f32x16 s;
#pragma unroll
        for (int r = 0; r < 16; ++r) s[r] = 0.f;
        const char* krow = Ks + (int64_t)(kt * 32 + ql) * (DH * 2);
#pragma unroll
        for (int ks = 0; ks < KS; ++ks) {
            const bf16x8 kf = *reinterpret_cast<const bf16x8*>(krow + (((2 * ks + hh) ^ krow_sw) << 4));
            s = __builtin_amdgcn_mfma_f32_32x32x16_bf16(kf, qf[ks], s, 0, 0, 0);
        }
        float mx = -INFINITY;
#pragma unroll
        for (int g4 = 0; g4 < 4; ++g4) {
            const int kb = kt * 32 + 8 * g4 + 4 * hh;
            f32x4 bv = f32x4{0.f, 0.f, 0.f, 0.f};
            if (HAS_BIAS) bv = *reinterpret_cast<const f32x4*>(brow + kb);
#pragma unroll
            for (int e = 0; e < 4; ++e) {
                float v = s[g4 * 4 + e] * scale_log2e + bv[e];
                v = (kb + e < L) ? v : -INFINITY;
                s[g4 * 4 + e] = v;
                mx = fmaxf(mx, v);
            }
        }
        mx = fmaxf(mx, __shfl_xor(mx, 32));
        const float m_new = fmaxf(m_run, mx);
        const float alpha = exp2f(m_run - m_new);
        m_run = m_new;
        float rs = 0.f;
#pragma unroll
        for (int r = 0; r < 16; ++r) { s[r] = exp2f(s[r] - m_new); rs += s[r]; }
        l_run = l_run * alpha + rs;
#pragma unroll
        for (int d = 0; d < DB; ++d)
#pragma unroll
            for (int r = 0; r < 16; ++r) o[d][r] *= alpha;
        bf16x8 pf[2];
#pragma unroll
        for (int ss = 0; ss < 2; ++ss)
#pragma unroll
            for (int e = 0; e < 8; ++e) pf[ss][e] = (bf16_t)s[8 * ss + e];
#pragma unroll
        for (int d = 0; d < DB; ++d) {
            const uint16_t* vrow = Vt + (int64_t)(d * 32 + ql) * vts + kt * 32 + hh * 8;
#pragma unroll
            for (int ss = 0; ss < 2; ++ss) {
                const bf16x8 vf = *reinterpret_cast<const bf16x8*>(vrow + ss * 16);
                o[d] = __builtin_amdgcn_mfma_f32_32x32x16_bf16(vf, pf[ss], o[d], 0, 0, 0);
            }
        }
    }
    const float l_tot = l_run + __shfl_xor(l_run, 32);
    const float inv = 1.0f / l_tot;
    if (q < L) {
        uint16_t* orow = ctx + (int64_t)(t0 + q) * H + h * DH;
#pragma unroll
        for (int d = 0; d < DB; ++d)
#pragma unroll
            for (int g4 = 0; g4 < 4; ++g4) {
                u32x2 w2;
                w2[0] = pack_bf16x2(o[d][g4 * 4 + 0] * inv, o[d][g4 * 4 + 1] * inv);
                w2[1] = pack_bf16x2(o[d][g4 * 4 + 2] * inv, o[d][g4 * 4 + 3] * inv);
                *reinterpret_cast<u32x2*>(orow + d * 32 + 8 * g4 + 4 * hh) = w2;
            }
    }
}

typedef short s16x4 __attribute__((ext_vector_type(4)));
template <int DH> struct AttnSmem2 {
    static __host__ __device__ int kv_bytes(int Lk) { return Lk * DH * 2; }
    static __host__ __device__ int bias_stride(int Lk) { return 2 * Lk + 8; }
    static __host__ __device__ int total(int Lk, bool has) { return 2 * kv_bytes(Lk) + (has ? 4 * (2 * Lk + 8) * 4 : 0); }
};

template <int DH> struct AttnSmem3 {
    static __host__ __device__ int kv_bytes(int Lk) { return Lk * DH * 2; }
    static __host__ __device__ int bias_stride(int Lk) { return ((2 * Lk + 8 + 63) & ~63) + 64; }
    static __host__ __device__ int total(int Lk, bool has) { return 2 * kv_bytes(Lk) + (has ? 4 * bias_stride(Lk) * 4 : 0); }
};
__device__ __forceinline__ int attn_bias_off(int c) { return c == 0 ? 0 : (c == 1 ? 20 : (c == 2 ? 36 : 52)); }

template <int DH, bool HAS_BIAS, int NW>
__global__ __launch_bounds__(NW * 64, NW / 2) void attention_tr_kernel(const uint16_t* __restrict__ qkv, uint16_t* __restrict__ ctx,
                                                                        const int32_t* __restrict__ cu,
                                                                        const float* __restrict__ bias_tbl, int H,
                                                                        float scale_log2e, int dev_word, unsigned long long* dev_stamps) {
    constexpr int NT = NW * 64;
    constexpr int CPR = DH / 8;
    constexpr int RPB = 256 / (DH * 2);
#ifdef ARX_DEV_VARIANTS
    const unsigned lin = blockIdx.x + gridDim.x * (blockIdx.y + gridDim.y * blockIdx.z);
    if (dev_stamps && threadIdx.x == 0) {
        dev_stamps[4 * lin] = wall_clock64();
        dev_stamps[4 * lin + 3] = ((unsigned long long)__builtin_amdgcn_s_getreg((31 << 11) | 20) << 32) | (unsigned)__builtin_amdgcn_s_getreg((31 << 11) | 4);
    }
#endif
    constexpr int KS = DH / 16;
    constexpr int DB = DH / 32;
    constexpr int ROWB = DH * 2;
    constexpr int RPI = NT / CPR;
    extern __shared__ __attribute__((aligned(16))) char smem[];
    const int b = blockIdx.z, h = blockIdx.y;
    const int t0 = cu[b];
    const int L = cu[b + 1] - t0;
    const int q0 = blockIdx.x * (32 * NW);
    if (q0 >= L) return;
    const int Lk = (L + 31) & ~31;
    const int tid = threadIdx.x, lane = tid & 63, wid = tid >> 6;
    const uint32_t ld = 3u * (uint32_t)H;
    const uint16_t* Qg = qkv + (int64_t)t0 * ld + h * DH;
    const uint16_t* Kg = Qg + H;
    const uint16_t* Vg = Qg + 2 * H;
    char* Ks = smem;
    char* Vs = smem + AttnSmem3<DH>::kv_bytes(Lk);
    float* Bs = reinterpret_cast<float*>(smem + 2 * AttnSmem3<DH>::kv_bytes(Lk));
    const int bst = AttnSmem3<DH>::bias_stride(Lk);

    const int ql = lane & 31, hh = lane >> 5;
    const int qw = q0 + wid * 32;
    const int q = qw + ql;
    const int qc = q < L ? q : L - 1;
    bf16x8 qf[KS];
#pragma unroll
    for (int ks = 0; ks < KS; ++ks)
        qf[ks] = *reinterpret_cast<const bf16x8*>(Qg + (uint32_t)qc * ld + ks * 16 + hh * 8);
    {
        static_assert(RPI % 16 == 0, "staging pass must keep the swizzle terms constant per thread");
        typedef __attribute__((address_space(3))) void lds_v;
        typedef const __attribute__((address_space(1))) void gbl_v;
        const int pc = tid % CPR, r0 = tid / CPR;
        const int kc = pc ^ ((r0 / RPB) & (CPR - 1));
        const int vc = (DH == 64) ? (pc ^ (((r0 >> 1) & 1) << 2)) : pc;
        uint32_t lo = (uint32_t)(tid & ~63) * 16;
        int LkS = Lk;
#ifdef ARX_DEV_VARIANTS
        if (dev_word == 5) LkS = 0;
#endif
        for (int row = r0; row < LkS; row += RPI, lo += NT * 16) {
            const uint32_t gr = (uint32_t)(row < L ? row : L - 1) * ld;
            __builtin_amdgcn_global_load_lds((gbl_v*)(Kg + gr + kc * 8), (lds_v*)(Ks + lo), 16, 0, 0);
            __builtin_amdgcn_global_load_lds((gbl_v*)(Vg + gr + vc * 8), (lds_v*)(Vs + lo), 16, 0, 0);
        }
    }
    if (HAS_BIAS) {
        const float* bt = bias_tbl + (int64_t)h * ARX_BIAS_ROW + ARX_BIAS_CENTER;
        const int span = 2 * Lk + 8;
        for (int i = tid; i < 4 * span; i += NT) {
            const int c = (i >= span) + (i >= 2 * span) + (i >= 3 * span), j = i - c * span;
            int d = j + c - Lk;
            d = d < -ARX_BIAS_CENTER ? -ARX_BIAS_CENTER : (d > ARX_BIAS_CENTER ? ARX_BIAS_CENTER : d);
            Bs[c * bst + attn_bias_off(c) + j] = bt[d];
        }
    }
    __syncthreads();
#ifdef ARX_DEV_VARIANTS
    if (dev_stamps && threadIdx.x == 0) dev_stamps[4 * lin + 1] = wall_clock64();
    if (dev_word == 3) {
        if (q < L && qf[0][0] == 0x7fc1 && qf[1 % KS][1] == 0x7fc2) ctx[(int64_t)(t0 + q) * H + h * DH] = 1;
        return;
    }
#endif

    if (qw >= L) return;
    f32x16 o[DB];
    auto lds_bases = [&](const float*& bb, const char* (&kb)[KS], const char* (&vb)[DB]) {
        int lane = threadIdx.x & 63;
        asm volatile("" : "+v"(lane));
        const int ql = lane & 31, hh = lane >> 5;
        int qc = q0 + wid * 32 + ql;
        qc = qc < L ? qc : L - 1;
        const int bc = (4 - (qc & 3)) & 3;
        bb = Bs + bc * bst + attn_bias_off(bc) + (Lk - qc - bc) + 4 * hh;
        const int krow_sw = ((ql / RPB) & (CPR - 1));
#pragma unroll
        for (int ks = 0; ks < KS; ++ks) kb[ks] = Ks + ql * ROWB + (((2 * ks + hh) ^ krow_sw) << 4);
        const int g16 = lane >> 4, q_ = (lane & 15) >> 2, p_ = lane & 3;
        const int vsw = (DH == 64) ? (((q_ >> 1) & 1) << 2) : 0;
#pragma unroll
        for (int d = 0; d < DB; ++d) {
            const int col = 32 * d + 16 * (g16 & 1) + 4 * p_;
            vb[d] = Vs + (4 * hh + q_) * ROWB + (((col >> 3) ^ vsw) << 4) + ((p_ & 1) << 3);
        }
    };
    typedef __attribute__((address_space(3))) s16x4 lds_s16x4;
    typedef short s16x8 __attribute__((ext_vector_type(8)));
    f32x4 lsum;
    const s16x4 one4 = s16x4{0x3f80, 0x3f80, 0x3f80, 0x3f80};
    const int nkt = Lk >> 5;
    const int nfull = (L & 31) ? nkt - 1 : nkt;
    float l_tot;

    bool redo = false;
#ifdef ARX_DEV_VARIANTS
    redo = dev_word == 6;
#endif
    if (!redo) {
#pragma unroll
        for (int d = 0; d < DB; ++d)
#pragma unroll
            for (int r = 0; r < 16; ++r) o[d][r] = 0.f;
        lsum = f32x4{0.f, 0.f, 0.f, 0.f};
        typedef const __attribute__((address_space(3))) char* lds_cptr;
        typedef const __attribute__((address_space(3))) float* lds_fptr;
        lds_fptr bp;
        lds_cptr kp[KS], vp[DB];
        {
            const float* bb;
            const char* kb[KS];
            const char* vb[DB];
            lds_bases(bb, kb, vb);
            bp = (lds_fptr)bb;
#pragma unroll
            for (int ks = 0; ks < KS; ++ks) kp[ks] = (lds_cptr)kb[ks];
#pragma unroll
            for (int d = 0; d < DB; ++d) vp[d] = (lds_cptr)vb[d];
        }
        bf16x8 kf[KS];
#pragma unroll
        for (int ks = 0; ks < KS; ++ks) kf[ks] = *reinterpret_cast<const __attribute__((address_space(3))) bf16x8*>(kp[ks]);
        auto advance = [&](int n) {
            bp += 32 * n;
            asm volatile("" : "+v"(bp));
#pragma unroll
            for (int ks = 0; ks < KS; ++ks) { kp[ks] += 32 * ROWB * n; asm volatile("" : "+v"(kp[ks])); }
#pragma unroll
            for (int d = 0; d < DB; ++d) { vp[d] += 32 * ROWB * n; asm volatile("" : "+v"(vp[d])); }
            __builtin_amdgcn_sched_barrier(0);
        };
        auto fast = [&](auto masked_tag, auto off_tag, int kt) {
            constexpr bool MASKED = decltype(masked_tag)::value;
            constexpr int OFF = decltype(off_tag)::value;
            f32x16 s;
#pragma unroll
            for (int r = 0; r < 16; ++r) s[r] = 0.f;
#pragma unroll
            for (int ks = 0; ks < KS; ++ks) s = __builtin_amdgcn_mfma_f32_32x32x16_bf16(kf[ks], qf[ks], s, 0, 0, 0);
            __builtin_amdgcn_sched_barrier(0);
            f32x4 bv[4];
#pragma unroll
            for (int g4 = 0; g4 < 4; ++g4) bv[g4] = HAS_BIAS ? *reinterpret_cast<const __attribute__((address_space(3))) f32x4*>(bp + OFF * 32 + 8 * g4) : f32x4{0.f, 0.f, 0.f, 0.f};
            s16x4 vt[DB][4];
#pragma unroll
            for (int d = 0; d < DB; ++d)
#pragma unroll
                for (int j = 0; j < 4; ++j) vt[d][j] = __builtin_amdgcn_ds_read_tr16_b64_v4i16((lds_s16x4*)(vp[d] + (OFF * 32 + 8 * j) * ROWB));
            __builtin_amdgcn_sched_barrier(0);
            typedef float f32x2 __attribute__((ext_vector_type(2)));
            const f32x2 sc2 = f32x2{scale_log2e, scale_log2e};
#pragma unroll
            for (int g4 = 0; g4 < 4; ++g4)
#pragma unroll
                for (int e = 0; e < 4; e += 2) {
                    f32x2 v = __builtin_elementwise_fma(f32x2{s[g4 * 4 + e], s[g4 * 4 + e + 1]}, sc2, f32x2{bv[g4][e], bv[g4][e + 1]});
                    if (MASKED) {
                        v[0] = (kt * 32 + 8 * g4 + 4 * hh + e < L) ? v[0] : -INFINITY;
                        v[1] = (kt * 32 + 8 * g4 + 4 * hh + e + 1 < L) ? v[1] : -INFINITY;
                    }
                    s[g4 * 4 + e] = v[0]; s[g4 * 4 + e + 1] = v[1];
                }
            __builtin_amdgcn_sched_barrier(0);
#pragma unroll
            for (int r = 0; r < 16; ++r) s[r] = __builtin_amdgcn_exp2f(s[r]);
            uint32_t pw[8];
#pragma unroll
            for (int j = 0; j < 8; ++j) pw[j] = pack_bf16x2(s[2 * j], s[2 * j + 1]);
            __builtin_amdgcn_sched_barrier(0);
            if (!MASKED) {
#pragma unroll
                for (int ks = 0; ks < KS; ++ks) kf[ks] = *reinterpret_cast<const __attribute__((address_space(3))) bf16x8*>(kp[ks] + (OFF + 1) * 32 * ROWB);
            }
            __builtin_amdgcn_sched_barrier(0);
            bf16x8 pf[2];
#pragma unroll
            for (int ss = 0; ss < 2; ++ss) pf[ss] = __builtin_bit_cast(bf16x8, u32x4{pw[4 * ss], pw[4 * ss + 1], pw[4 * ss + 2], pw[4 * ss + 3]});
#pragma unroll
            for (int j = 0; j < 4; ++j)
                lsum = __builtin_amdgcn_mfma_f32_4x4x4bf16_1k(one4, __builtin_bit_cast(s16x4, u32x2{pw[2 * j], pw[2 * j + 1]}), lsum, 0, 0, 0);
#pragma unroll
            for (int d = 0; d < DB; ++d)
#pragma unroll
                for (int ss = 0; ss < 2; ++ss) {
                    s16x8 v8;
#pragma unroll
                    for (int e = 0; e < 4; ++e) { v8[e] = vt[d][2 * ss][e]; v8[4 + e] = vt[d][2 * ss + 1][e]; }
                    o[d] = __builtin_amdgcn_mfma_f32_32x32x16_bf16(__builtin_bit_cast(bf16x8, v8), pf[ss], o[d], 0, 0, 0);
                }
            __builtin_amdgcn_sched_barrier(0);
        };
        int kt = 0;
        for (; kt + 2 <= nfull; kt += 2) {
            fast(std::false_type{}, std::integral_constant<int, 0>{}, kt);
            fast(std::false_type{}, std::integral_constant<int, 1>{}, kt + 1);
            advance(2);
        }
        if (kt < nfull) { fast(std::false_type{}, std::integral_constant<int, 0>{}, kt); advance(1); }
        if (nfull < nkt) fast(std::true_type{}, std::integral_constant<int, 0>{}, nkt - 1);
        l_tot = lsum[0] + __shfl_xor(lsum[0], 32);
        redo = !__all(l_tot > 0x1p-100f && l_tot < 0x1p100f);
    }
    if (redo) {
#pragma unroll
    for (int d = 0; d < DB; ++d)
#pragma unroll
        for (int r = 0; r < 16; ++r) o[d][r] = 0.f;
    float m_run = -INFINITY;
    const float* bptr;
    const char* kptr[KS];
    const char* vptr[DB];
    lds_bases(bptr, kptr, vptr);
    constexpr float THR = 8.0f;
    const float inv_scale = 1.0f / scale_log2e;
    lsum = f32x4{0.f, 0.f, 0.f, 0.f};
    auto tile = [&](auto masked_tag, auto first_tag, int kt) {
        constexpr bool MASKED = decltype(masked_tag)::value;
        constexpr bool FIRST = decltype(first_tag)::value;
        f32x16 s;
        const float s0 = FIRST ? 0.f : -m_run * inv_scale;
#pragma unroll
        for (int r = 0; r < 16; ++r) s[r] = s0;
#pragma unroll
        for (int ks = 0; ks < KS; ++ks) {
            const bf16x8 kf = *reinterpret_cast<const bf16x8*>(kptr[ks]);
            s = __builtin_amdgcn_mfma_f32_32x32x16_bf16(kf, qf[ks], s, 0, 0, 0);
        }
#pragma unroll
        for (int g4 = 0; g4 < 4; ++g4) {
            f32x4 bv = f32x4{0.f, 0.f, 0.f, 0.f};
            if (HAS_BIAS) bv = *reinterpret_cast<const f32x4*>(bptr + 8 * g4);
#pragma unroll
            for (int e = 0; e < 4; ++e) {
                float v = fmaf(s[g4 * 4 + e], scale_log2e, bv[e]);
                if (MASKED) v = (kt * 32 + 8 * g4 + 4 * hh + e < L) ? v : -INFINITY;
                s[g4 * 4 + e] = v;
            }
        }
        float mx = -INFINITY;
#pragma unroll
        for (int r = 0; r < 16; r += 2) mx = fmaxf(mx, fmaxf(s[r], s[r + 1]));
        mx = fmaxf(mx, __shfl_xor(mx, 32));
        if (FIRST) {
            m_run = mx;
#pragma unroll
            for (int r = 0; r < 16; ++r) s[r] -= mx;
        } else if (__any(mx > THR)) {
            const float d = fmaxf(mx, 0.f);
            const float alpha = __builtin_amdgcn_exp2f(-d);
            m_run += d;
#pragma unroll
            for (int r = 0; r < 16; ++r) s[r] -= d;
#pragma unroll
            for (int r = 0; r < 4; ++r) lsum[r] *= alpha;
#pragma unroll
            for (int dd = 0; dd < DB; ++dd)
#pragma unroll
                for (int r = 0; r < 16; ++r) o[dd][r] *= alpha;
        }
#pragma unroll
        for (int r = 0; r < 16; ++r) s[r] = __builtin_amdgcn_exp2f(s[r]);
        uint32_t pw[8];
#pragma unroll
        for (int j = 0; j < 8; ++j) pw[j] = pack_bf16x2(s[2 * j], s[2 * j + 1]);
        bf16x8 pf[2];
#pragma unroll
        for (int ss = 0; ss < 2; ++ss) pf[ss] = __builtin_bit_cast(bf16x8, u32x4{pw[4 * ss], pw[4 * ss + 1], pw[4 * ss + 2], pw[4 * ss + 3]});
#pragma unroll
        for (int j = 0; j < 4; ++j)
            lsum = __builtin_amdgcn_mfma_f32_4x4x4bf16_1k(one4, __builtin_bit_cast(s16x4, u32x2{pw[2 * j], pw[2 * j + 1]}), lsum, 0, 0, 0);
#pragma unroll
        for (int d = 0; d < DB; ++d) {
#pragma unroll
            for (int ss = 0; ss < 2; ++ss) {
                const s16x4 lo = __builtin_amdgcn_ds_read_tr16_b64_v4i16((lds_s16x4*)(vptr[d] + (16 * ss) * ROWB));
                const s16x4 hi = __builtin_amdgcn_ds_read_tr16_b64_v4i16((lds_s16x4*)(vptr[d] + (16 * ss + 8) * ROWB));
                s16x8 v8;
#pragma unroll
                for (int e = 0; e < 4; ++e) { v8[e] = lo[e]; v8[4 + e] = hi[e]; }
                o[d] = __builtin_amdgcn_mfma_f32_32x32x16_bf16(__builtin_bit_cast(bf16x8, v8), pf[ss], o[d], 0, 0, 0);
            }
        }
        bptr += 32;
#pragma unroll
        for (int ks = 0; ks < KS; ++ks) kptr[ks] += 32 * ROWB;
#pragma unroll
        for (int d = 0; d < DB; ++d) vptr[d] += 32 * ROWB;
    };
    if (nfull > 0) tile(std::false_type{}, std::true_type{}, 0); else tile(std::true_type{}, std::true_type{}, 0);
    for (int kt = 1; kt < nfull; ++kt) tile(std::false_type{}, std::false_type{}, kt);
    if (nfull < nkt && nkt > 1) tile(std::true_type{}, std::false_type{}, nkt - 1);
    l_tot = lsum[0] + __shfl_xor(lsum[0], 32);
    }

    const float inv = 1.0f / l_tot;
    u32x4 pc[DB][2];
#pragma unroll
    for (int d = 0; d < DB; ++d) {
        uint32_t w[4][2];
#pragma unroll
        for (int g4 = 0; g4 < 4; ++g4) {
            w[g4][0] = pack_bf16x2(o[d][g4 * 4 + 0] * inv, o[d][g4 * 4 + 1] * inv);
            w[g4][1] = pack_bf16x2(o[d][g4 * 4 + 2] * inv, o[d][g4 * 4 + 3] * inv);
        }
#pragma unroll
        for (int g = 0; g < 2; ++g)
#pragma unroll
            for (int k = 0; k < 2; ++k) {
                const auto sw = __builtin_amdgcn_permlane32_swap(w[g][k], w[g + 2][k], false, false);
                pc[d][g][k] = sw[0]; pc[d][g][2 + k] = sw[1];
            }
    }
    if (q < L) {
        uint16_t* orow = ctx + (int64_t)(t0 + q) * H + h * DH + 16 * hh;
#pragma unroll
        for (int d = 0; d < DB; ++d) {
            *reinterpret_cast<u32x4*>(orow + d * 32) = pc[d][0];
            *reinterpret_cast<u32x4*>(orow + d * 32 + 8) = pc[d][1];
        }
    }
#ifdef ARX_DEV_VARIANTS
    if (dev_stamps && (threadIdx.x & 63) == 0) atomicMax(&dev_stamps[4 * lin + 2], (unsigned long long)wall_clock64());
#endif
}

#ifdef ARX_DEV_VARIANTS
template <int DH, int NSLOT_ = 8> struct AttnRing {
    static constexpr int NT = 512, NSLOT = NSLOT_, AHEAD = NSLOT - 1, SLOT_KEYS = 64;
    static constexpr int ROWB = DH * 2;
    static constexpr int SLOT_BYTES = 2 * SLOT_KEYS * ROWB;
    static constexpr int GPS = SLOT_BYTES / (NT * 16);
    static_assert(GPS >= 1 && GPS * NT * 16 == SLOT_BYTES, "slot must be whole passes of the block");
    static __host__ __device__ int bias_stride(int C0) { return (2 * C0 + 8 + 52 + 63) & ~63; }
    static __host__ __device__ int total(int C0, bool has) { return NSLOT * SLOT_BYTES + (has ? 4 * bias_stride(C0) * 4 : 0); }
};

#define ARX_VMCNT_CASE(N) case N: asm volatile("s_waitcnt vmcnt(" #N ")" ::: "memory"); break;
#define ARX_VMCNT_CASE4(A, B, C_, D) ARX_VMCNT_CASE(A) ARX_VMCNT_CASE(B) ARX_VMCNT_CASE(C_) ARX_VMCNT_CASE(D)
__device__ __forceinline__ void attn_wait_vm(int n) {
    switch (n) {
    ARX_VMCNT_CASE4(0, 1, 2, 3) ARX_VMCNT_CASE4(4, 5, 6, 7) ARX_VMCNT_CASE4(8, 9, 10, 11) ARX_VMCNT_CASE4(12, 13, 14, 15)
    ARX_VMCNT_CASE4(16, 17, 18, 19) ARX_VMCNT_CASE4(20, 21, 22, 23) ARX_VMCNT_CASE4(24, 25, 26, 27) ARX_VMCNT_CASE4(28, 29, 30, 31)
    ARX_VMCNT_CASE4(32, 33, 34, 35) ARX_VMCNT_CASE4(36, 37, 38, 39) ARX_VMCNT_CASE4(40, 41, 42, 43) ARX_VMCNT_CASE(44)
    default: asm volatile("s_waitcnt vmcnt(0)" ::: "memory"); break;
    }
}
#undef ARX_VMCNT_CASE4
#undef ARX_VMCNT_CASE

template <int DH, int NSLOT> struct AttnStream {
    using R = AttnRing<DH, NSLOT>;
    static constexpr int NT = R::NT, ROWB = R::ROWB, SLOT_BYTES = R::SLOT_BYTES, GPS = R::GPS, CPR = DH / 8, RPB = 256 / R::ROWB;
    const uint16_t* qkv; const int32_t* cu; char* ring;
    int H, h, G, n_seqs;
    uint32_t ld;
    int p_b, p_t0, p_L, p_step, p_nqp, p_nsteps, p_slot, c_slot;
    int inflight, pend_st;
    unsigned st_bits;

    __device__ __forceinline__ void p_load_item() {
        p_L = 0; p_step = 0;
        while (p_b < n_seqs) {
            const __attribute__((address_space(4))) int32_t* cuc = (const __attribute__((address_space(4))) int32_t*)cu;
            const int t0 = cuc[p_b], L = cuc[p_b + 1] - t0;
            if (L > 0) { p_t0 = t0; p_L = L; p_nqp = L > 128 ? 2 : 1; p_nsteps = p_nqp + ((L + 63) >> 6); break; }
            p_b += G;
        }
    }
    __device__ __forceinline__ void issue_next() {
        const uint16_t* base = qkv + (int64_t)p_t0 * ld + h * DH;
        const bool isq = p_step < p_nqp;
        const int r0 = isq ? 128 * p_step : 64 * (p_step - p_nqp);
        int t = threadIdx.x;
        asm volatile("" : "+v"(t));
        char* dst = ring + p_slot * SLOT_BYTES + (__builtin_amdgcn_readfirstlane(t) & ~63) * 16;
#pragma unroll
        for (int it = 0; it < GPS; ++it) {
            const int cid = it * NT + t, r128 = cid / CPR, pcn = cid % CPR;
            int row, col0, c;
            if (isq) { row = r0 + r128; col0 = 0; c = pcn ^ ((r128 / RPB) & (CPR - 1)); }
            else if (r128 < 64) { row = r0 + r128; col0 = H; c = pcn ^ ((r128 / RPB) & (CPR - 1)); }
            else { row = r0 + r128 - 64; col0 = 2 * H; c = (DH == 64) ? (pcn ^ (((r128 >> 1) & 1) << 2)) : pcn; }
            row = row < p_L ? row : p_L - 1;
            __builtin_amdgcn_global_load_lds((const __attribute__((address_space(1))) void*)(base + (uint32_t)row * ld + col0 + c * 8),
                                             (__attribute__((address_space(3))) void*)(dst + it * NT * 16), 16, 0, 0);
        }
        if (pend_st) st_bits |= 1u << inflight;
        pend_st = 0;
        ++inflight;
        p_slot = (p_slot + 1) & (R::NSLOT - 1);
        if (++p_step == p_nsteps) { p_b += G; p_load_item(); }
    }
    __device__ __forceinline__ const char* step_begin() {
        attn_wait_vm((inflight - 1) * GPS + (DH / 8) * __builtin_popcount(st_bits >> 1) + pend_st);
        asm volatile("" ::: "memory");
        __builtin_amdgcn_s_barrier();
        asm volatile("" ::: "memory");
        st_bits >>= 1;
        --inflight;
        if (p_L > 0) issue_next();
        const char* slot = ring + c_slot * SLOT_BYTES;
        c_slot = (c_slot + 1) & (R::NSLOT - 1);
        return slot;
    }
};

template <int DH, bool HAS_BIAS, bool MASKED, bool first>
__device__ __forceinline__ void attn_ring_tile(const char* kbase, int k0, int v0, const bf16x8 (&qf)[DH / 16], f32x16 (&o)[DH / 32],
                                               f32x4& lsum, float& m_run, const float* bp, int kt, int hh, int L,
                                               float scale_log2e, float inv_scale) {
    constexpr int KS = DH / 16, DB = DH / 32, ROWB = DH * 2;
    constexpr float THR = 8.0f;
    typedef __attribute__((address_space(3))) s16x4 lds_s16x4;
    typedef short s16x8 __attribute__((ext_vector_type(8)));
    f32x16 s;
    const float s0 = first ? 0.f : -m_run * inv_scale;
#pragma unroll
    for (int r = 0; r < 16; ++r) s[r] = s0;
#pragma unroll
    for (int ks = 0; ks < KS; ++ks) {
        const bf16x8 kf = *reinterpret_cast<const bf16x8*>(kbase + (k0 ^ (ks << 5)));
        s = __builtin_amdgcn_mfma_f32_32x32x16_bf16(kf, qf[ks], s, 0, 0, 0);
    }
#pragma unroll
    for (int g4 = 0; g4 < 4; ++g4) {
        f32x4 bv = f32x4{0.f, 0.f, 0.f, 0.f};
        if (HAS_BIAS) bv = *reinterpret_cast<const f32x4*>(bp + 8 * g4);
#pragma unroll
        for (int e = 0; e < 4; ++e) {
            float v = fmaf(s[g4 * 4 + e], scale_log2e, bv[e]);
            if (MASKED) v = (kt * 32 + 8 * g4 + 4 * hh + e < L) ? v : -INFINITY;
            s[g4 * 4 + e] = v;
        }
    }
    float mx = -INFINITY;
#pragma unroll
    for (int r = 0; r < 16; r += 2) mx = fmaxf(mx, fmaxf(s[r], s[r + 1]));
    mx = fmaxf(mx, __shfl_xor(mx, 32));
    if (first) {
        m_run = mx;
#pragma unroll
        for (int r = 0; r < 16; ++r) s[r] -= mx;
    } else if (__any(mx > THR)) {
        const float d = fmaxf(mx, 0.f);
        const float alpha = __builtin_amdgcn_exp2f(-d);
        m_run += d;
#pragma unroll
        for (int r = 0; r < 16; ++r) s[r] -= d;
#pragma unroll
        for (int r = 0; r < 4; ++r) lsum[r] *= alpha;
#pragma unroll
        for (int dd = 0; dd < DB; ++dd)
#pragma unroll
            for (int r = 0; r < 16; ++r) o[dd][r] *= alpha;
    }
#pragma unroll
    for (int r = 0; r < 16; ++r) s[r] = __builtin_amdgcn_exp2f(s[r]);
    uint32_t pw[8];
#pragma unroll
    for (int j = 0; j < 8; ++j) pw[j] = pack_bf16x2(s[2 * j], s[2 * j + 1]);
    bf16x8 pf[2];
#pragma unroll
    for (int ss = 0; ss < 2; ++ss) pf[ss] = __builtin_bit_cast(bf16x8, u32x4{pw[4 * ss], pw[4 * ss + 1], pw[4 * ss + 2], pw[4 * ss + 3]});
    const s16x4 one4 = s16x4{0x3f80, 0x3f80, 0x3f80, 0x3f80};
#pragma unroll
    for (int j = 0; j < 4; ++j)
        lsum = __builtin_amdgcn_mfma_f32_4x4x4bf16_1k(one4, __builtin_bit_cast(s16x4, u32x2{pw[2 * j], pw[2 * j + 1]}), lsum, 0, 0, 0);
    const uint32_t vaddr = (uint32_t)(size_t)(const __attribute__((address_space(3))) char*)kbase + (uint32_t)v0;
#pragma unroll
    for (int d = 0; d < DB; ++d) {
        const uint32_t va = vaddr ^ (uint32_t)(d << 6);
        s16x4 vt[2][2];
#pragma unroll
        for (int ss = 0; ss < 2; ++ss) {
            asm volatile("ds_read_b64_tr_b16 %0, %1 offset:%2" : "=v"(vt[ss][0]) : "v"(va), "n"((16 * ss) * ROWB));
            asm volatile("ds_read_b64_tr_b16 %0, %1 offset:%2" : "=v"(vt[ss][1]) : "v"(va), "n"((16 * ss + 8) * ROWB));
        }
        asm volatile("s_waitcnt lgkmcnt(0)" : "+v"(vt[0][0]), "+v"(vt[0][1]), "+v"(vt[1][0]), "+v"(vt[1][1]) :: "memory");
#pragma unroll
        for (int ss = 0; ss < 2; ++ss) {
            s16x8 v8;
#pragma unroll
            for (int e = 0; e < 4; ++e) { v8[e] = vt[ss][0][e]; v8[4 + e] = vt[ss][1][e]; }
            o[d] = __builtin_amdgcn_mfma_f32_32x32x16_bf16(__builtin_bit_cast(bf16x8, v8), pf[ss], o[d], 0, 0, 0);
        }
    }
}

template <int DH, bool HAS_BIAS, int NSLOT>
__global__ __launch_bounds__(512, 2) void attention_ring_kernel(const uint16_t* __restrict__ qkv, uint16_t* __restrict__ ctx,
                                                                 const int32_t* __restrict__ cu,
                                                                 const float* __restrict__ bias_tbl, int H, int n_seqs,
                                                                 int C0, float scale_log2e) {
    using R = AttnRing<DH, NSLOT>;
    constexpr int NT = R::NT, ROWB = R::ROWB, SLOT_BYTES = R::SLOT_BYTES, GPS = R::GPS;
    constexpr int CPR = DH / 8;
    constexpr int RPB = 256 / ROWB;
    constexpr int KS = DH / 16;
    constexpr int DB = DH / 32;
    constexpr int NSTORE = DB * 4;
    static_assert((R::AHEAD - 1) * GPS + 4 * NSTORE <= 44, "attn_wait_vm covers AHEAD - 1 younger slot-loads plus four items' stores");
    extern __shared__ __attribute__((aligned(16))) char smem[];
    const int tid = threadIdx.x, lane = tid & 63, wid = __builtin_amdgcn_readfirstlane(tid >> 6);
    const int heads = H / DH;
    const int h = blockIdx.x % heads, g = blockIdx.x / heads, G = gridDim.x / heads;
    float* const Bs = reinterpret_cast<float*>(smem + R::NSLOT * SLOT_BYTES);
    const int bst = R::bias_stride(C0);

    if (HAS_BIAS) {
        const float* bt = bias_tbl + (int64_t)h * ARX_BIAS_ROW + ARX_BIAS_CENTER;
        const int span = 2 * C0 + 8;
        for (int i = tid; i < 4 * span; i += NT) {
            const int c = i / span, j = i - c * span;
            int d = j + c - C0;
            d = d < -ARX_BIAS_CENTER ? -ARX_BIAS_CENTER : (d > ARX_BIAS_CENTER ? ARX_BIAS_CENTER : d);
            Bs[c * bst + attn_bias_off(c) + j] = bt[d];
        }
    }
    __syncthreads();

    AttnStream<DH, NSLOT> st;
    st.qkv = qkv; st.cu = cu; st.ring = smem; st.H = H; st.h = h; st.G = G; st.n_seqs = n_seqs; st.ld = 3u * (uint32_t)H;
    st.p_b = g; st.p_t0 = 0; st.p_L = 0; st.p_step = 0; st.p_nqp = 0; st.p_nsteps = 0; st.p_slot = 0; st.c_slot = 0;
    st.inflight = 0; st.pend_st = 0; st.st_bits = 0u;
    st.p_load_item();
    if (st.p_L == 0) return;
#pragma unroll 1
    for (int i = 0; i < R::AHEAD && st.p_L > 0; ++i) st.issue_next();

    const int ql = lane & 31, hh = lane >> 5;
    const int k0 = ql * ROWB + ((hh ^ ((ql / RPB) & (CPR - 1))) << 4);
    const int q_ = (lane & 15) >> 2, p_ = lane & 3;
    const int vsw = (DH == 64) ? (((q_ >> 1) & 1) << 2) : 0;
    const int v0 = 64 * ROWB + (4 * hh + q_) * ROWB + ((((16 * ((lane >> 4) & 1) + 4 * p_) >> 3) ^ vsw) << 4) + ((p_ & 1) << 3);
    const float inv_scale = 1.0f / scale_log2e;

    int b = g;
#pragma unroll 1
    for (;;) {
        int t0 = 0, L = 0;
        while (b < n_seqs) {
            const __attribute__((address_space(4))) int32_t* cuc = (const __attribute__((address_space(4))) int32_t*)cu;
            t0 = cuc[b]; L = cuc[b + 1] - t0;
            if (L > 0) break;
            b += G;
        }
        if (b >= n_seqs) break;
        const int nqp = L > 128 ? 2 : 1, nkv = (L + 63) >> 6, nkt = (L + 31) >> 5;
        const bool wave_on = wid * 32 < L;
        bf16x8 qf[KS];
        f32x16 o[DB];
        f32x4 lsum = f32x4{0.f, 0.f, 0.f, 0.f};
        float m_run = 0.f;
#pragma unroll
        for (int ks = 0; ks < KS; ++ks)
#pragma unroll
            for (int e = 0; e < 8; ++e) qf[ks][e] = (bf16_t)0.f;
#pragma unroll
        for (int d = 0; d < DB; ++d)
#pragma unroll
            for (int r = 0; r < 16; ++r) o[d][r] = 0.f;
        const int q = wid * 32 + ql, qc = q < L ? q : L - 1;
        const int bc = (4 - (qc & 3)) & 3;
        const float* bptr = Bs + bc * bst + attn_bias_off(bc) + (C0 - qc - bc) + 4 * hh;

#pragma unroll 1
        for (int p = 0; p < nqp; ++p) {
            const char* slot = st.step_begin();
            if (wave_on && (wid >> 2) == p) {
                const int r = (wid & 3) * 32 + ql;
                const char* qrow = slot + r * ROWB;
                const int sw = (r / RPB) & (CPR - 1);
#pragma unroll
                for (int ks = 0; ks < KS; ++ks) qf[ks] = *reinterpret_cast<const bf16x8*>(qrow + (((2 * ks + hh) ^ sw) << 4));
            }
        }
        const bool ragged = (L & 31) != 0;
#pragma unroll 1
        for (int sidx = 0; sidx < nkv; ++sidx) {
            const char* slot = st.step_begin();
            if (wave_on) {
#pragma unroll 1
                for (int t2 = 0; t2 < 2; ++t2) {
                    const int kt = 2 * sidx + t2;
                    if (kt >= nkt) break;
                    const char* kbase = slot + t2 * 32 * ROWB;
                    const bool msk = ragged && kt == nkt - 1;
                    if (kt == 0) {
                        if (msk) attn_ring_tile<DH, HAS_BIAS, true, true>(kbase, k0, v0, qf, o, lsum, m_run, bptr, kt, hh, L, scale_log2e, inv_scale);
                        else attn_ring_tile<DH, HAS_BIAS, false, true>(kbase, k0, v0, qf, o, lsum, m_run, bptr, kt, hh, L, scale_log2e, inv_scale);
                    } else {
                        if (msk) attn_ring_tile<DH, HAS_BIAS, true, false>(kbase, k0, v0, qf, o, lsum, m_run, bptr + 32 * kt, kt, hh, L, scale_log2e, inv_scale);
                        else attn_ring_tile<DH, HAS_BIAS, false, false>(kbase, k0, v0, qf, o, lsum, m_run, bptr + 32 * kt, kt, hh, L, scale_log2e, inv_scale);
                    }
                }
            }
        }
        if (wave_on) {
            const float l_tot = lsum[0] + __shfl_xor(lsum[0], 32);
            const float inv = 1.0f / l_tot;
            uint16_t* orow = ctx + (int64_t)(t0 + qc) * H + h * DH + 4 * hh;
            if (q < L) {
#pragma unroll
                for (int d = 0; d < DB; ++d)
#pragma unroll
                    for (int g4 = 0; g4 < 4; ++g4) {
                        u32x2 w2;
                        w2[0] = pack_bf16x2(o[d][g4 * 4 + 0] * inv, o[d][g4 * 4 + 1] * inv);
                        w2[1] = pack_bf16x2(o[d][g4 * 4 + 2] * inv, o[d][g4 * 4 + 3] * inv);
                        asm volatile("global_store_dwordx2 %0, %1, off\n\ts_nop 1" :: "v"(orow + d * 32 + 8 * g4), "v"(w2) : "memory");
                    }
            }
            st.pend_st += NSTORE;
        }
        b += G;
    }
}

template <int NSLOT_ = 8> struct AttnRing16 {
    static constexpr int DH = 64, NT = 1024, NSLOT = NSLOT_, AHEAD = NSLOT - 1;
    static constexpr int ROWB = DH * 2, SLOT_BYTES = 128 * ROWB;
    static __host__ __device__ int bias_stride(int C0) { return (2 * C0 + 8 + 52 + 63) & ~63; }
    static __host__ __device__ int total(int C0, bool has) { return NSLOT * SLOT_BYTES + (has ? 4 * bias_stride(C0) * 4 : 0); }
// ... 454 lines not shown
```

arxiv_rag_amd/encoder.py:

```python
from __future__ import annotations

import ctypes as C
from typing import Dict, List, Optional, Sequence, Union

import numpy as np
import torch

from . import _lib
from .config import ARCH_MPNET, EncoderConfig
from .weights import layer_keys


def _dev_ptr(t: Optional[torch.Tensor]) -> Optional[int]:
    return None if t is None else t.data_ptr()


class HipEncoder:

    def __init__(self, cfg: EncoderConfig, state_dict: Dict[str, np.ndarray], device: Union[str, torch.device] = "cuda:0",
                 max_tokens: int = 32 * 512, max_seqs: int = 32):
        self.lib = _lib.load()
        if not torch.cuda.is_available():
            raise _lib.ArxError("no HIP device visible: the encoder has no CPU path")
        self.cfg = cfg
        self.device = torch.device(device)
        torch.cuda.set_device(self.device)
        self._w: List[torch.Tensor] = []
        self._handle = C.c_void_p(None)
        self._cap = (0, 0)
        self._upload(state_dict)
        self._ensure_capacity(max_tokens, max_seqs)

    def _f32(self, a: np.ndarray) -> torch.Tensor:
        t = torch.from_numpy(np.ascontiguousarray(a, dtype=np.float32)).to(self.device)
        self._w.append(t)
        return t

    def _bf16(self, a: np.ndarray) -> torch.Tensor:
        src = torch.from_numpy(np.ascontiguousarray(a, dtype=np.float32)).to(self.device)
        dst = torch.empty(src.shape, dtype=torch.bfloat16, device=self.device)
        _lib.check(self.lib.arx_f32_to_bf16(src.data_ptr(), dst.data_ptr(), src.numel(),
                                            torch.cuda.current_stream().cuda_stream), "arx_f32_to_bf16")
        self._w.append(dst)
        return dst

    def _upload(self, sd: Dict[str, np.ndarray]):
        cfg = self.cfg
        self._layers_c = (_lib.LayerWeightsC * cfg.layers)()
        for i in range(cfg.layers):
            k = layer_keys(cfg, i)
            wqkv = np.concatenate([sd[k["q"] + ".weight"], sd[k["k"] + ".weight"], sd[k["v"] + ".weight"]], 0)
            bqkv = np.concatenate([sd[k["q"] + ".bias"], sd[k["k"] + ".bias"], sd[k["v"] + ".bias"]], 0)
            L = self._layers_c[i]
            L.w_qkv = self._bf16(wqkv).data_ptr(); L.b_qkv = self._f32(bqkv).data_ptr()
            L.w_o = self._bf16(sd[k["o"] + ".weight"]).data_ptr(); L.b_o = self._f32(sd[k["o"] + ".bias"]).data_ptr()
            L.ln1_g = self._f32(sd[k["ln1"] + ".weight"]).data_ptr(); L.ln1_b = self._f32(sd[k["ln1"] + ".bias"]).data_ptr()
            L.w_fc1 = self._bf16(sd[k["fc1"] + ".weight"]).data_ptr(); L.b_fc1 = self._f32(sd[k["fc1"] + ".bias"]).data_ptr()
            L.w_fc2 = self._bf16(sd[k["fc2"] + ".weight"]).data_ptr(); L.b_fc2 = self._f32(sd[k["fc2"] + ".bias"]).data_ptr()
            L.ln2_g = self._f32(sd[k["ln2"] + ".weight"]).data_ptr(); L.ln2_b = self._f32(sd[k["ln2"] + ".bias"]).data_ptr()
        w = _lib.EncoderWeightsC()
        w.word_emb = self._f32(sd["embeddings.word_embeddings.weight"]).data_ptr()
        w.pos_emb = self._f32(sd["embeddings.position_embeddings.weight"]).data_ptr()
        w.emb_ln_g = self._f32(sd["embeddings.LayerNorm.weight"]).data_ptr()
        w.emb_ln_b = self._f32(sd["embeddings.LayerNorm.bias"]).data_ptr()
        if cfg.arch == ARCH_MPNET:
            w.type_emb = None
            w.rel_bias = self._f32(sd["encoder.relative_attention_bias.weight"]).data_ptr()
        else:
            w.type_emb = self._f32(sd["embeddings.token_type_embeddings.weight"][0]).data_ptr()
            w.rel_bias = None
        w.layers = C.cast(self._layers_c, C.POINTER(_lib.LayerWeightsC))
        self._weights_c = w
        c = _lib.EncoderConfigC(cfg.arch, cfg.vocab_size, cfg.hidden, cfg.layers, cfg.heads, cfg.ffn, cfg.max_pos,
                                cfg.pool, cfg.pad_id, cfg.rel_buckets, cfg.rel_max_distance, cfg.ln_eps)
        self._cfg_c = c
        torch.cuda.synchronize(self.device)

    def _ensure_capacity(self, max_tokens: int, max_seqs: int):
        if max_tokens <= self._cap[0] and max_seqs <= self._cap[1]:
            return
        max_tokens = max(max_tokens, self._cap[0]); max_seqs = max(max_seqs, self._cap[1])
        self.close()
        h = C.c_void_p(None)
        _lib.check(self.lib.arx_encoder_create(C.byref(self._cfg_c), C.byref(self._weights_c), max_tokens, max_seqs,
                                               C.byref(h)), "arx_encoder_create")
        self._handle = h
        self._cap = (max_tokens, max_seqs)
        self._low_latency = False

    def close(self):
        if getattr(self, "_handle", None) is not None and self._handle.value:
            torch.cuda.synchronize(self.device)
            self.lib.arx_encoder_destroy(self._handle)
            self._handle = C.c_void_p(None)
            self._cap = (0, 0)

    def __del__(self):
        try:
            self.close()
        except Exception:
            pass

    def forward_tokens(self, ids: torch.Tensor, lens: torch.Tensor, max_len: int, total_tokens: int,
                       out: Optional[torch.Tensor] = None, out_f16: Optional[torch.Tensor] = None,
                       normalize: bool = True, low_latency: bool = False) -> Optional[torch.Tensor]:
        B, S = ids.shape
        assert ids.dtype == torch.int32 and lens.dtype == torch.int32 and ids.is_contiguous() and lens.is_contiguous()
        self._ensure_capacity(total_tokens, B)
        if bool(low_latency) != self._low_latency:
            _lib.check(self.lib.arx_encoder_set_low_latency(self._handle, 1 if low_latency else 0), "arx_encoder_set_low_latency")
            self._low_latency = bool(low_latency)
        if out is None and out_f16 is None:
            out = torch.empty((B, self.cfg.hidden), dtype=torch.float32, device=self.device)
        rc = self.lib.arx_encoder_forward(
            self._handle, ids.data_ptr(), S, lens.data_ptr(), B, max_len, total_tokens,
            _dev_ptr(out), 0 if out is None else out.stride(0),
            _dev_ptr(out_f16), 0 if out_f16 is None else out_f16.stride(0),
            1 if normalize else 0, torch.cuda.current_stream().cuda_stream)
        _lib.check(rc, "arx_encoder_forward")
        return out

    def encode_tokens(self, ids: np.ndarray, lens: np.ndarray, normalize: bool = True, low_latency: bool = False) -> torch.Tensor:
        ids = np.ascontiguousarray(ids, dtype=np.int32)
        lens = np.ascontiguousarray(lens, dtype=np.int32)
        if ids.shape[0] == 0:
            return torch.empty((0, self.cfg.hidden), dtype=torch.float32, device=self.device)
        max_len = max(int(lens.max()), 1)
        total = max(int(lens.sum()), 1)
        d_ids = torch.from_numpy(ids).to(self.device, non_blocking=True)
        d_lens = torch.from_numpy(lens).to(self.device, non_blocking=True)
        return self.forward_tokens(d_ids, d_lens, max_len, total, normalize=normalize, low_latency=low_latency)

    @staticmethod
    def _pad_batch(seqs: Sequence[Sequence[int]], idx: Sequence[int], pad_id: int):
        lens = np.fromiter((len(seqs[i]) for i in idx), np.int32, len(idx))
        S = max(int(lens.max()) if len(idx) else 1, 1)
        ids = np.full((len(idx), S), pad_id, np.int32)
        tot = int(lens.sum())
        if tot:
            flat = np.concatenate([np.asarray(seqs[i], np.int32) for i in idx if len(seqs[i])])
            rows = np.repeat(np.arange(len(idx)), lens)
            starts = np.cumsum(lens) - lens
            cols = np.arange(tot) - np.repeat(starts, lens)
            ids[rows, cols] = flat
        return ids, lens

    def encode_ragged(self, seqs: Sequence[Sequence[int]], batch_size: int = 256, normalize: bool = True,
                      on_device: bool = False, out_f16: Optional[torch.Tensor] = None, low_latency: bool = False):
        n = len(seqs)
        if n == 0:
            return (torch.zeros((0, self.cfg.hidden), dtype=torch.float32, device=self.device) if on_device
                    else np.zeros((0, self.cfg.hidden), np.float32))
        order = sorted(range(n), key=lambda i: -len(seqs[i]))
        dev_out = torch.empty((n, self.cfg.hidden), dtype=torch.float32, device=self.device)
        dev16 = self._f16_stage(n, out_f16)
        for s0 in range(0, n, batch_size):
            idx = order[s0:s0 + batch_size]
            ids, lens = self._pad_batch(seqs, idx, self.cfg.pad_id)
            d_ids = torch.from_numpy(ids).to(self.device, non_blocking=True)
            d_lens = torch.from_numpy(lens).to(self.device, non_blocking=True)
            self.forward_tokens(d_ids, d_lens, ids.shape[1], max(int(lens.sum()), 1), out=dev_out[s0:s0 + len(idx)],
                                out_f16=None if dev16 is None else dev16[s0:s0 + len(idx)], normalize=normalize,
                                low_latency=low_latency)
        order_t = torch.as_tensor(order, device=self.device) if (on_device or dev16 is not None) else None
        if dev16 is not None:
            out_f16[:, :self.cfg.hidden].index_copy_(0, order_t, dev16)
        if on_device:
            out = torch.empty_like(dev_out)
            out[order_t] = dev_out
            return out
        out = np.empty((n, self.cfg.hidden), np.float32)
        out[np.asarray(order)] = dev_out.cpu().numpy()
        return out

    def _f16_stage(self, n: int, out_f16: Optional[torch.Tensor]) -> Optional[torch.Tensor]:
        if out_f16 is None:
            return None
        assert out_f16.is_cuda and out_f16.dtype == torch.float16 and out_f16.dim() == 2 and out_f16.stride(1) == 1
        assert out_f16.shape[0] == n and out_f16.shape[1] >= self.cfg.hidden, "out_f16 must be [n, >= hidden]"
        return torch.empty((n, self.cfg.hidden), dtype=torch.float16, device=self.device)

    def encode_packed(self, ids: np.ndarray, lens: np.ndarray, batch_size: int = 256, normalize: bool = True,
                      on_device: bool = False, out_f16: Optional[torch.Tensor] = None, low_latency: bool = False):
        n = int(len(lens))
        if n == 0:
            return (torch.zeros((0, self.cfg.hidden), dtype=torch.float32, device=self.device) if on_device
                    else np.zeros((0, self.cfg.hidden), np.float32))
        lens = np.ascontiguousarray(lens, dtype=np.int32)
        order = np.argsort(-lens.astype(np.int64), kind="stable")
        dev_out = torch.empty((n, self.cfg.hidden), dtype=torch.float32, device=self.device)
        dev16 = self._f16_stage(n, out_f16)
        for s0 in range(0, n, batch_size):
            idx = order[s0:s0 + batch_size]
            bl = lens[idx]
            ml = max(int(bl.max()), 1)
            d_ids = torch.from_numpy(np.ascontiguousarray(ids[idx, :ml], dtype=np.int32)).to(self.device, non_blocking=True)
            d_lens = torch.from_numpy(np.ascontiguousarray(bl)).to(self.device, non_blocking=True)
            self.forward_tokens(d_ids, d_lens, ml, max(int(bl.sum()), 1), out=dev_out[s0:s0 + len(idx)],
                                out_f16=None if dev16 is None else dev16[s0:s0 + len(idx)], normalize=normalize,
                                low_latency=low_latency)
        order_t = torch.from_numpy(order).to(self.device) if (on_device or dev16 is not None) else None
        if dev16 is not None:
            out_f16[:, :self.cfg.hidden].index_copy_(0, order_t, dev16)
        if on_device:
            out = torch.empty_like(dev_out)
            out[order_t] = dev_out
            return out
        out = np.empty((n, self.cfg.hidden), np.float32)
        out[order] = dev_out.cpu().numpy()
        return out

    def tap_hidden(self, ids: np.ndarray, lens: np.ndarray, layer: int, low_latency: bool = False) -> np.ndarray:
        _lib.check(self.lib.arx_encoder_set_tap(self._handle, layer), "arx_encoder_set_tap")
        self.encode_tokens(ids, lens, low_latency=low_latency)
        T = int(np.asarray(lens).sum())
        dst = torch.empty((T, self.cfg.hidden), dtype=torch.float32, device=self.device)
        _lib.check(self.lib.arx_encoder_debug_hidden(self._handle, layer, dst.data_ptr(), T,
                                                     torch.cuda.current_stream().cuda_stream), "arx_encoder_debug_hidden")
        _lib.check(self.lib.arx_encoder_set_tap(self._handle, -1), "arx_encoder_set_tap")
        return dst.cpu().numpy()


def adjacent_cosines(embeddings: torch.Tensor) -> torch.Tensor:
    lib = _lib.load()
    e = embeddings
    assert e.is_cuda and e.dtype == torch.float32 and e.dim() == 2 and e.stride(1) == 1
    n, d = e.shape
    out = torch.empty((max(n - 1, 0),), dtype=torch.float32, device=e.device)
    _lib.check(lib.arx_adjacent_cosine(e.data_ptr(), e.stride(0), n, d, out.data_ptr(),
                                       torch.cuda.current_stream().cuda_stream), "arx_adjacent_cosine")
    return out


class HipSentenceEncoder:

    def __init__(self, cfg: EncoderConfig, state_dict, tokenizer, device="cuda:0", max_batch: int = 1024):
        self.cfg = cfg
        self.tokenizer = tokenizer
        self.max_seq_length = cfg.max_seq_length
        self.encoder = HipEncoder(cfg, state_dict, device=device)
        self.max_batch = max_batch
        self.slab_texts = 8192
        self.first_slab_texts = 1024
        self.coalesce_batches = True

    def get_sentence_embedding_dimension(self) -> int:
        return self.cfg.hidden

    def tokenize(self, sentences: Sequence[str]) -> List[List[int]]:
        return self.tokenizer.encode_batch(list(sentences), self.max_seq_length)

    def _tokenize_any(self, sentences: Sequence[str]):
        if hasattr(self.tokenizer, "encode_batch_packed"):
            ids, lens = self.tokenizer.encode_batch_packed(list(sentences), self.max_seq_length)
            return ("packed", ids, lens)
        return ("ragged", self.tokenize(sentences))

    def _encode_tokens_any(self, toks, bs: int, normalize: bool, on_device: bool = False, out_f16=None, low_latency: bool = False):
        if toks[0] == "packed":
            return self.encoder.encode_packed(toks[1], toks[2], batch_size=bs, normalize=normalize, on_device=on_device,
                                              out_f16=out_f16, low_latency=low_latency)
        return self.encoder.encode_ragged(toks[1], batch_size=bs, normalize=normalize, on_device=on_device, out_f16=out_f16,
                                          low_latency=low_latency)

    def encode_device(self, sentences: Sequence[str], batch_size: int = 32, normalize_embeddings: bool = False) -> torch.Tensor:
        bs = max(1, min(batch_size, self.max_batch))
        return self._encode_tokens_any(self._tokenize_any(list(sentences)), bs, normalize_embeddings, on_device=True)

    def encode(self, sentences, batch_size: int = 32, show_progress_bar=None, convert_to_numpy: bool = True,
               convert_to_tensor: bool = False, normalize_embeddings: bool = False, device_f16_out: Optional[torch.Tensor] = None,
               low_latency: bool = False, **_ignored):
        single = isinstance(sentences, str)
        if single:
            sentences = [sentences]
        sentences = list(sentences)
        bs = self.max_batch if self.coalesce_batches else max(1, min(batch_size, self.max_batch))
        slab = max(bs, self.slab_texts)
        first = max(bs, self.first_slab_texts)
        if len(sentences) <= first:
            emb = self._encode_tokens_any(self._tokenize_any(sentences), bs, normalize_embeddings, out_f16=device_f16_out,
                                          low_latency=low_latency)
        else:
            from concurrent.futures import ThreadPoolExecutor
            bounds, size, s0 = [], first, 0
            while s0 < len(sentences):
                bounds.append((s0, min(len(sentences), s0 + size)))
                s0 += size
                size = min(slab, size * 2)
            parts = []
            with ThreadPoolExecutor(max_workers=1) as ex:
                fut = ex.submit(self._tokenize_any, sentences[bounds[0][0]:bounds[0][1]])
                for bi in range(len(bounds)):
                    seqs = fut.result()
                    if bi + 1 < len(bounds):
                        fut = ex.submit(self._tokenize_any, sentences[bounds[bi + 1][0]:bounds[bi + 1][1]])
                    o16 = None if device_f16_out is None else device_f16_out[bounds[bi][0]:bounds[bi][1]]
                    parts.append(self._encode_tokens_any(seqs, bs, normalize_embeddings, out_f16=o16))
            emb = np.concatenate(parts, 0)
        if convert_to_tensor:
            emb = torch.from_numpy(emb)
        return emb[0] if single else emb
```

include/arx.h:

```cpp
#ifndef ARX_H
#define ARX_H

#include <stdint.h>

#ifdef __cplusplus
extern "C" {
#endif

#define ARX_VERSION 111

#define ARX_OK            0
#define ARX_ERR_ARG      -1
#define ARX_ERR_HIP      -2
#define ARX_ERR_CAPACITY -3

#define ARX_ARCH_MPNET 0
#define ARX_ARCH_BERT  1
#define ARX_POOL_MEAN  0
#define ARX_POOL_CLS   1

typedef struct {
    int32_t arch;
    int32_t vocab_size;
    int32_t hidden;
    int32_t layers;
    int32_t heads;
    int32_t ffn;
    int32_t max_pos;
    int32_t pool;
    int32_t pad_id;
    int32_t rel_buckets;
    int32_t rel_max_distance;
    float   ln_eps;
} arx_encoder_config;

typedef struct {
    const void*  w_qkv;
    const float* b_qkv;
    const void*  w_o;
    const float* b_o;
    const float* ln1_g; const float* ln1_b;
    const void*  w_fc1;
    const float* b_fc1;
    const void*  w_fc2;
    const float* b_fc2;
    const float* ln2_g; const float* ln2_b;
} arx_layer_weights;

typedef struct {
    const float* word_emb;
    const float* pos_emb;
    const float* type_emb;
    const float* emb_ln_g; const float* emb_ln_b;
    const float* rel_bias;
    const arx_layer_weights* layers;
} arx_encoder_weights;

typedef struct arx_encoder arx_encoder;

int32_t     arx_version(void);
const char* arx_last_error(void);

int32_t arx_mpnet_bucket(int32_t relative_position, int32_t num_buckets, int32_t max_distance);

int64_t arx_encoder_workspace_bytes(const arx_encoder_config* cfg, int32_t max_tokens, int32_t max_seqs);

int32_t arx_encoder_create(const arx_encoder_config* cfg, const arx_encoder_weights* w,
                           int32_t max_tokens, int32_t max_seqs, arx_encoder** out);
void    arx_encoder_destroy(arx_encoder* h);

int32_t arx_encoder_forward(arx_encoder* h, const int32_t* ids, int32_t seq_stride,
                            const int32_t* lens, int32_t n_seqs, int32_t max_len, int32_t total_tokens,
                            float* out_f32, int64_t out_stride,
                            void* out_f16, int64_t out16_stride,
                            int32_t normalize, void* stream);

int32_t arx_encoder_attention(arx_encoder* h, const void* qkv, const int32_t* lens, int32_t n_seqs, int32_t max_len,
                              void* ctx, void* stream);

int32_t arx_encoder_debug_hidden(arx_encoder* h, int32_t layer_slot, float* dst, int32_t n_tokens, void* stream);

int32_t arx_encoder_set_low_latency(arx_encoder* h, int32_t on);

int32_t arx_encoder_set_tap(arx_encoder* h, int32_t layer);

typedef struct {
    int32_t struct_bytes;
    int32_t n_labels;
    const float* type_emb;
    const float* pooler_w; const float* pooler_b;
    const float* cls_w;    const float* cls_b;
} arx_pair_head;

int32_t arx_encoder_set_pair_head(arx_encoder* h, const arx_pair_head* head);
int32_t arx_encoder_score_pairs(arx_encoder* h, const int32_t* ids, int32_t seq_stride, const int32_t* lens, const int32_t* seg_b,
                                int32_t n_seqs, int32_t max_len, int32_t total_tokens, float* out_logits, int64_t out_stride,
                                void* stream);
int32_t arx_encoder_debug_cls(arx_encoder* h, float* dst, int32_t n, void* stream);
int32_t arx_pair_head_forward(const float* cls_rows, int64_t ld, int32_t n, int32_t hidden, const arx_pair_head* head,
                              float* out_logits, int64_t out_stride, void* stream);

int32_t arx_build_info(void);

int64_t arx_topk_workspace_bytes(int64_t n_rows, int32_t n_queries, int32_t dim, int32_t k);
int32_t arx_topk_search(const void* corpus, int64_t n_rows, const void* queries, int32_t n_queries,
                        int32_t dim, int32_t k, float* out_scores, int64_t* out_ids, int64_t idx_base,
                        void* ws, int64_t ws_bytes, void* stream);

int64_t arx_topk_i8_index_bytes(int64_t n_rows, int32_t dim);
int64_t arx_topk_workspace_bytes_i8(int64_t n_rows, int32_t n_queries, int32_t dim, int32_t k);
int32_t arx_topk_build_i8(const void* corpus, int64_t n_rows, int32_t dim, void* index_i8, void* stream);
int32_t arx_topk_i8_index_info(const void* index_i8, int64_t n_rows, int32_t dim, float* host_out, void* stream);
int32_t arx_topk_search_i8(const void* corpus, const void* index_i8, int64_t n_rows, const void* queries, int32_t n_queries,
                           int32_t dim, int32_t k, float* out_scores, int64_t* out_ids, int64_t idx_base,
                           void* ws, int64_t ws_bytes, void* stream);

#define ARX_TOPK_NO_PERSISTENT 1
#define ARX_TOPK_NO_SINGLE_ROW_TAIL 8
#define ARX_TOPK_I8_CENTRE_QUERY 16
#define ARX_TOPK_SCAN_ONLY     2
#define ARX_TOPK_TAIL_ONLY     4
typedef struct {
    int32_t struct_bytes;
    int32_t i8_max_queries;
    float   max_row_norm;
    int32_t cu_limit;
    int32_t flags;
    float   debug_tau_mult;
    int32_t debug_drop_best;
} arx_topk_options;
int32_t arx_topk_search_opt(const void* corpus, const void* index_i8, int64_t n_rows, const void* queries, int32_t n_queries,
                            int32_t dim, int32_t k, float* out_scores, int64_t* out_ids, int64_t idx_base,
                            void* ws, int64_t ws_bytes, const arx_topk_options* opt, void* stream);

int32_t arx_rows_max_norm_f16(const void* rows, int64_t n_rows, int32_t dim, float* out_max, void* stream);

int32_t arx_topk_stats(const void* ws, int64_t* flagged_queries, int64_t* extra_groups, void* stream);

int32_t arx_stream_create_cu_mask(const uint32_t* cu_mask, int32_t n_words, void** out);
int32_t arx_stream_destroy(void* stream);
int32_t arx_device_cu_count(void);
int32_t arx_debug_cu_census(uint32_t* out, int32_t n_blocks, int32_t spin_cycles, void* stream);

int32_t arx_topk_merge(const float* scores, const int64_t* ids, int32_t n_parts, int32_t n_queries,
                       int32_t k, float* out_scores, int64_t* out_ids, void* stream);

int64_t arx_topk_filtered_workspace_bytes(int64_t n_rows, int32_t n_queries, int32_t dim, int32_t k);
int32_t arx_topk_search_filtered(const void* corpus, int64_t n_rows, const uint64_t* allow, int64_t n_allowed, const void* queries,
                                 int32_t n_queries, int32_t dim, int32_t k, float* out_scores, int64_t* out_ids, int64_t idx_base,
                                 float max_row_norm, void* ws, int64_t ws_bytes, void* stream);
int32_t arx_topk_search_filtered_tuned(const void* corpus, int64_t n_rows, const uint64_t* allow, int64_t n_allowed, const void* queries,
                                       int32_t n_queries, int32_t dim, int32_t k, float* out_scores, int64_t* out_ids, int64_t idx_base,
                                       float max_row_norm, void* ws, int64_t ws_bytes, int32_t path, int32_t cand_cap, void* stream);
int32_t arx_topk_filtered_stats(const void* ws, int64_t* overflowed_queries, int64_t* candidate_groups, void* stream);

int64_t arx_topk_prefix_workspace_bytes(int64_t n_rows, int32_t n_queries, int32_t dim, int32_t k);
int32_t arx_topk_search_prefix(const void* corpus, int64_t n_rows, const void* queries, const int64_t* row_limit, int32_t n_queries,
                               int32_t dim, int32_t k, float* out_scores, int64_t* out_ids, int64_t idx_base, float max_row_norm,
                               void* ws, int64_t ws_bytes, void* stream);
int32_t arx_topk_search_prefix_tuned(const void* corpus, int64_t n_rows, const void* queries, const int64_t* row_limit, int32_t n_queries,
                                     int32_t dim, int32_t k, float* out_scores, int64_t* out_ids, int64_t idx_base, float max_row_norm,
                                     void* ws, int64_t ws_bytes, int32_t path, int32_t cand_cap, void* stream);
int32_t arx_topk_prefix_stats(const void* ws, int64_t* overflowed_queries, int64_t* candidate_groups, void* stream);

int32_t arx_text_contains(const uint8_t* blob, const int64_t* row_off, int64_t n_rows,
                          const uint8_t* pat_blob, const int32_t* pat_off, int32_t n_pat,
                          uint64_t* out_bits, void* stream);
int32_t arx_bitmap_count(const uint64_t* bits, int64_t n_rows, int64_t* out_count, void* stream);

int32_t arx_gather_rows(const void* shard, int64_t n_rows, int32_t dim, int64_t idx_base, const int64_t* ids, int64_t count,
                        void* out, void* stream);
int32_t arx_mmr_select(const void* q, const void* cand, const int64_t* ids, int32_t n_queries, int32_t n, int32_t dim, int32_t m,
                       float lambda, int32_t* order, float* mmr, void* stream);

int64_t arx_bm25_workspace_bytes(int64_t n_rows, int32_t n_queries, int32_t n);
int32_t arx_bm25_search(const int64_t* term_ptr, const uint32_t* post_row, const float* post_w, int32_t vocab, int64_t n_rows,
                        const int32_t* q_terms, const int32_t* q_nterms, int32_t n_queries, int32_t n, float* out_scores,
                        int64_t* out_ids, int64_t idx_base, void* ws, int64_t ws_bytes, void* stream);
int32_t arx_bm25_search_tuned(const int64_t* term_ptr, const uint32_t* post_row, const float* post_w, int32_t vocab, int64_t n_rows,
                              const int32_t* q_terms, const int32_t* q_nterms, int32_t n_queries, int32_t n, float* out_scores,
                              int64_t* out_ids, int64_t idx_base, void* ws, int64_t ws_bytes, int32_t tile_rows, int32_t max_blocks,
                              void* stream);
int32_t arx_bm25_scores(const int64_t* term_ptr, const uint32_t* post_row, const float* post_w, int32_t vocab, int64_t n_rows,
                        const int32_t* q_terms, int32_t n_terms, int64_t row_lo, int64_t row_hi, int32_t tile_rows, float* out,
                        void* stream);

int32_t arx_gemm_bf16(const void* A, const void* W, const float* bias, const void* resid, void* C,
                      int32_t M, int32_t N, int32_t K, int32_t mode, int32_t variant, void* stream);

typedef struct {
    int32_t struct_bytes;
    int32_t mode;
    int32_t variant;
    float eps;
    const float* bias;
    const void* resid;
    const float *a_mean, *a_rstd;
    const float* s_vec;
    const float *r_mean, *r_rstd;
    const float *r_gamma, *r_beta;
    int64_t row_cap;
    float *part_sum, *part_sq;
    int64_t part_ld;
    float *out_mean, *out_rstd;
    const int32_t* n_rows;
} arx_gemm_epilogue;
int32_t arx_gemm_bf16_ex(const void* A, const void* W, void* C, int32_t M, int32_t N, int32_t K, const arx_gemm_epilogue* e, void* stream);

int32_t arx_fold_ln(const void* W, const float* gamma, const float* beta, const float* bias, void* Wf, float* s, float* c,
                    int32_t N, int32_t K, void* stream);

int32_t arx_adjacent_cosine(const float* emb, int64_t ld, int32_t n, int32_t dim, float* out, void* stream);

int32_t arx_wp_create(const char* vocab_blob, const int64_t* vocab_off , int32_t n_vocab, int32_t unk_id,
                      int32_t bos_id, int32_t eos_id, int32_t pad_id, int32_t lowercase, int32_t max_chars_per_word,
                      const char* trigger_blob, const int64_t* trigger_off , int32_t n_triggers, void** out);
void arx_wp_destroy(void* tokenizer);
int32_t arx_wp_encode(void* tokenizer, const char* text_blob, const int64_t* text_off , int64_t n, int32_t max_len,
                      int32_t* ids, int32_t* lens, uint8_t* fallback, int32_t n_threads);
int32_t arx_wp_miss_count(void* tokenizer, int64_t* n_strings, int64_t* n_bytes);
int32_t arx_wp_miss_fetch(void* tokenizer, char* blob, int64_t* off );
int32_t arx_wp_cache_add(void* tokenizer, const char* seg_blob, const int64_t* seg_off , int64_t n, const int32_t* ids,
                         const int64_t* ids_off );
int64_t arx_wp_cache_size(void* tokenizer);
int32_t arx_wp_version(void);

int32_t arx_f32_to_bf16(const float* src, void* dst, int64_t n, void* stream);
int32_t arx_fill_unit_rows_f16(void* dst, int64_t n_rows, int32_t dim, uint64_t seed, void* stream);
int32_t arx_fill_unit_rows_f16_at(void* dst, int64_t n_rows, int32_t dim, uint64_t seed, int64_t row_base, void* stream);
int32_t arx_fill_clustered_rows_f16_at(void* dst, int64_t n_rows, int32_t dim, uint64_t seed, int64_t row_base, int32_t n_clusters,
                                       float spread, int32_t n_hot_dims, float hot_gain, void* stream);

#define ARX_K_SEARCH_GROUPMAX 0
#define ARX_K_GEMM_QKV        1
#define ARX_K_GEMM_OPROJ      2
#define ARX_K_GEMM_FC1        3
#define ARX_K_GEMM_FC2        4
#define ARX_K_ATTENTION       5
#define ARX_K_LAYERNORM       6
#define ARX_K_EMBED           7
#define ARX_K_POOL            8
#define ARX_K_SEARCH_SELECT   9
#define ARX_K_SEARCH_RESCORE 10
#define ARX_K_GEMM_RAW       11
#define ARX_K_CLASSES        12
int32_t arx_prof_enable(int32_t on);
int32_t arx_prof_classes(uint32_t mask);
int32_t arx_prof_reset(void);
int32_t arx_prof_read(int32_t kernel_class, float* total_ms, int32_t* launches);

#ifdef __cplusplus
}
#endif
#endif
```

Baseline: 22160.

## Fuse QKV projection GEMM with attention in one per-sequence-head kernel

Adds a kernel that computes one head's Q, K and V slice for a block of sequences, applies the bias and folded layernorm epilogue, keeps the tiles in LDS, and runs attention from there. It replaces the separate QKV GEMM plus attention launch when batches are dense, max_len ≤ 256 and head dim is 64. The goal is to avoid writing the full QKV tensor to global memory and reading it back, and to drop one launch per layer. The cost is a GEMM with less reuse across heads and sequences, heavy LDS use that may lower occupancy, and fragile applicability conditions.

```diff
diff --git a/arxiv_rag_amd/_lib.py b/arxiv_rag_amd/_lib.py
--- a/arxiv_rag_amd/_lib.py
+++ b/arxiv_rag_amd/_lib.py
@@ -8,7 +8,7 @@
 LIB_PATH = Path(os.environ.get("ARX_LIB", _HERE / "libarx_hip.so"))
 
 K_CLASSES = ["search_groupmax", "gemm_qkv", "gemm_oproj", "gemm_fc1", "gemm_fc2", "attention",
-             "layernorm", "embed", "pool", "search_select", "search_rescore", "gemm_raw"]
+             "layernorm", "embed", "pool", "search_select", "search_rescore", "gemm_raw", "qkv_attention"]
 
 
 class EncoderConfigC(C.Structure):
@@ -72,6 +72,8 @@
     "arx_encoder_attention": (C.c_int32, [C.c_void_p, C.c_void_p, C.c_void_p, C.c_int32, C.c_int32, C.c_void_p, C.c_void_p]),
     "arx_encoder_set_tap": (C.c_int32, [C.c_void_p, C.c_int32]),
     "arx_encoder_set_low_latency": (C.c_int32, [C.c_void_p, C.c_int32]),
+    "arx_encoder_set_fused_attention": (C.c_int32, [C.c_void_p, C.c_int32]),
+    "arx_encoder_debug_ctx": (C.c_int32, [C.c_void_p, C.c_void_p, C.c_int32, C.c_void_p]),
     "arx_encoder_debug_hidden": (C.c_int32, [C.c_void_p, C.c_int32, C.c_void_p, C.c_int32, C.c_void_p]),
     "arx_encoder_set_pair_head": (C.c_int32, [C.c_void_p, C.POINTER(PairHeadC)]),
     "arx_encoder_score_pairs": (C.c_int32, [C.c_void_p, C.c_void_p, C.c_int32, C.c_void_p, C.c_void_p, C.c_int32, C.c_int32, C.c_int32,
diff --git a/arxiv_rag_amd/csrc/encoder.hip b/arxiv_rag_amd/csrc/encoder.hip
--- a/arxiv_rag_amd/csrc/encoder.hip
+++ b/arxiv_rag_amd/csrc/encoder.hip
@@ -10,6 +10,7 @@
 #include "gemm.h"
 #include "gemm8.h"
 #include "gemm_small.h"
+#include "qkv_attention.h"
 
 extern "C" int32_t arx_mpnet_bucket(int32_t rel, int32_t num_buckets, int32_t max_distance) {
     int n = -rel;
@@ -45,6 +46,8 @@
     int low_latency = 0;
     float* small_ws = nullptr;
     int attn_variant = 1;
+    int fused_qkv_attn = 1;
+    int qkv_dev_dump = 0;
     int attn_dev_word = 0;
     unsigned long long* attn_stamps = nullptr;
     arx_pair_head pair{};
@@ -223,6 +226,13 @@
     return ARX_OK;
 }
 
+extern "C" int32_t arx_encoder_set_fused_attention(arx_encoder* h, int32_t on) {
+    ARX_REQUIRE(h, "null handle");
+    ARX_REQUIRE(on >= 0 && on <= 2, "mode must be 0 (off), 1 (dense batches: the default) or 2 (wherever the kernel applies)");
+    h->fused_qkv_attn = on;
+    return ARX_OK;
+}
+
 extern "C" int32_t arx_encoder_set_tap(arx_encoder* h, int32_t layer) {
     ARX_REQUIRE(h, "null handle");
     ARX_REQUIRE(layer >= -1 && layer <= h->cfg.layers, "tap layer out of range");
@@ -237,6 +247,13 @@
     const int64_t n = (int64_t)n_tokens * h->cfg.hidden;
     bf16_to_f32_kernel<<<cdiv(n, 256), 256, 0, (hipStream_t)stream>>>(h->tap, dst, n);
     ARX_HIP_CHECK(hipGetLastError());
+    return ARX_OK;
+}
+
+extern "C" int32_t arx_encoder_debug_ctx(arx_encoder* h, void* dst, int32_t n_tokens, void* stream) {
+    ARX_REQUIRE(h && dst, "null handle/dst");
+    ARX_REQUIRE(n_tokens > 0 && n_tokens <= h->max_tokens, "n_tokens out of range");
+    ARX_HIP_CHECK(hipMemcpyAsync(dst, h->ctx, (int64_t)n_tokens * h->cfg.hidden * 2, hipMemcpyDeviceToDevice, (hipStream_t)stream));
     return ARX_OK;
 }
 
@@ -514,6 +531,42 @@
     return big ? launch_attn_cfg<32, false, 8>(h, n_seqs, max_len, st) : launch_attn_cfg<32, false, 4>(h, n_seqs, max_len, st);
 }
 
+static bool fused_qkv_attn_applies(const arx_encoder* h, int gv, int n_seqs, int max_len, int total_tokens) {
+    const arx_encoder_config& c = h->cfg;
+    const bool dense = (int64_t)total_tokens * 32 >= (int64_t)n_seqs * 256 * 31;
+    return (h->fused_qkv_attn == 2 || (h->fused_qkv_attn == 1 && dense)) && h->attn_variant == 1 && gv == 89 && h->tap_layer < 0 && c.hidden / c.heads == 64 && c.heads >= 2 &&
+           max_len <= 256 && (int64_t)h->tok_pad * c.hidden * 2 < (1ll << 32);
+}
+
+template <bool HB, bool LN>
+static int launch_qkv_attention_cfg(arx_encoder* h, const uint16_t* W, const float* bias, const float* s_vec, int n_seqs, hipStream_t st) {
+    auto kern = qkv_attention_kernel<64, HB, LN>;
+    const int smem = QkvAttnSmem::total(HB);
+    ARX_HIP_CHECK(arx_func_smem((const void*)kern, smem));
+    const float scale_log2e = 1.4426950408889634f / sqrtf(64.0f);
+    const int grid = 8 * cdiv(n_seqs, 8) * h->cfg.heads;
+    uint16_t* dump = nullptr;
+#ifdef ARX_DEV_VARIANTS
+    if (h->qkv_dev_dump) dump = h->qkv;
+#endif
+    ProfScope ps(ARX_K_QKV_ATTENTION, st);
+    kern<<<grid, 512, smem, st>>>(h->x, W, bias, s_vec, h->st2_sum, h->st2_sq, h->ctx, h->cu, h->bias_tbl, h->cfg.hidden, h->cfg.heads,
+                                  n_seqs, scale_log2e, dump);
+    ARX_HIP_CHECK(hipGetLastError());
+    return ARX_OK;
+}
+
+static int launch_qkv_attention(arx_encoder* h, int li, int n_seqs, hipStream_t st) {
+    const bool hb = h->cfg.arch == ARX_ARCH_MPNET;
+    if (li == 0) {
+        const uint16_t* W = (const uint16_t*)h->layers[0].w_qkv;
+        const float* b = h->layers[0].b_qkv;
+        return hb ? launch_qkv_attention_cfg<true, false>(h, W, b, nullptr, n_seqs, st) : launch_qkv_attention_cfg<false, false>(h, W, b, nullptr, n_seqs, st);
+    }
+    return hb ? launch_qkv_attention_cfg<true, true>(h, h->wqkv_f[li], h->c_qkv[li], h->s_qkv[li], n_seqs, st)
+              : launch_qkv_attention_cfg<false, true>(h, h->wqkv_f[li], h->c_qkv[li], h->s_qkv[li], n_seqs, st);
+}
+
 extern "C" int32_t arx_encoder_attention(arx_encoder* h, const void* qkv, const int32_t* lens, int32_t n_seqs, int32_t max_len,
                                          void* ctx, void* stream) {
     ARX_REQUIRE(h && qkv && lens && ctx, "null pointer argument");
@@ -692,11 +745,17 @@
 
     const float inv_h = 1.0f / (float)H;
     const int gv = !h->low_latency ? h->variant : (T <= ARX_SMALL_M ? 70 : (T <= ARX_MEDIUM_M ? 71 : h->variant));
+    const bool fused = fused_qkv_attn_applies(h, gv, n_seqs, max_len, T);
     if (h->tap_layer == 0 && h->tap) ARX_HIP_CHECK(hipMemcpyAsync(h->tap, h->x, (int64_t)T * H * 2, hipMemcpyDeviceToDevice, st));
     for (int li = 0; li < c.layers; ++li) {
         const arx_layer_weights& L = h->layers[li];
         EpiParams ep;
-        if (li == 0) {
+        if (fused) {
+            if ((rc = launch_qkv_attention(h, li, n_seqs, st)) != ARX_OK) return rc;
+#ifdef ARX_DEV_VARIANTS
+            if (h->qkv_dev_dump && (rc = launch_attn(h, n_seqs, max_len, st)) != ARX_OK) return rc;
+#endif
+        } else if (li == 0) {
             ep = EpiParams{h->qkv, 3 * (int64_t)H, L.b_qkv, nullptr, 0};
             if ((rc = launch_gemm<EPI_BIAS>(ARX_K_GEMM_QKV, gv, h->x, H, (const uint16_t*)L.w_qkv, H, T, 3 * H, H, ep, st, h->small_ws)) != ARX_OK) return rc;
         } else {
@@ -704,7 +763,7 @@
             ep.a_sum = h->st2_sum; ep.a_sq = h->st2_sq; ep.s_vec = h->s_qkv[li]; ep.inv_h = inv_h; ep.eps = c.ln_eps;
             if ((rc = launch_gemm<EPI_LN_BIAS>(ARX_K_GEMM_QKV, gv, h->x, H, h->wqkv_f[li], H, T, 3 * H, H, ep, st, h->small_ws)) != ARX_OK) return rc;
         }
-        if ((rc = launch_attn(h, n_seqs, max_len, st)) != ARX_OK) return rc;
+        if (!fused && (rc = launch_attn(h, n_seqs, max_len, st)) != ARX_OK) return rc;
         ep = EpiParams{h->x1, H, L.b_o, h->x, H};
         ep.o_sum = h->part_s; ep.o_sq = h->part_q; ep.o_ld = tp; ep.inv_h = inv_h; ep.eps = c.ln_eps;
         ep.fin_mean = h->st1_sum; ep.fin_rstd = h->st1_sq;
@@ -814,6 +873,7 @@
 }
 
 #ifdef ARX_DEV_VARIANTS
+extern "C" int32_t arx_dev_qkv_dump(arx_encoder* h, int32_t on) { h->qkv_dev_dump = on; return ARX_OK; }
 extern "C" int32_t arx_dev_attn_set(arx_encoder* h, int32_t word, void* stamps) {
     h->attn_dev_word = word;
     h->attn_stamps = (unsigned long long*)stamps;
diff --git a/arxiv_rag_amd/csrc/encoder_kernels.h b/arxiv_rag_amd/csrc/encoder_kernels.h
--- a/arxiv_rag_amd/csrc/encoder_kernels.h
+++ b/arxiv_rag_amd/csrc/encoder_kernels.h
@@ -322,6 +322,283 @@
 };
 __device__ __forceinline__ int attn_bias_off(int c) { return c == 0 ? 0 : (c == 1 ? 20 : (c == 2 ? 36 : 52)); }
 
+template <int NT>
+__device__ __forceinline__ void attention_tr_stage_bias(float* Bs, int bst, const float* __restrict__ bias_tbl, int h, int Lk, int tid) {
+    const float* bt = bias_tbl + (int64_t)h * ARX_BIAS_ROW + ARX_BIAS_CENTER;
+    const int span = 2 * Lk + 8;
+    for (int i = tid; i < 4 * span; i += NT) {
+        const int c = (i >= span) + (i >= 2 * span) + (i >= 3 * span), j = i - c * span;
+        int d = j + c - Lk;
+        d = d < -ARX_BIAS_CENTER ? -ARX_BIAS_CENTER : (d > ARX_BIAS_CENTER ? ARX_BIAS_CENTER : d);
+        Bs[c * bst + attn_bias_off(c) + j] = bt[d];
+    }
+}
+
+template <int DH, bool HAS_BIAS>
+__device__ __forceinline__ void attention_tr_body(const bf16x8 (&qf)[DH / 16], const char* Ks, const char* Vs, const float* Bs, int bst, int L, int Lk,
+                                                  int q0, int wid, uint16_t* __restrict__ ctx, int t0, int H, int h, float scale_log2e, int dev_word) {
+    constexpr int CPR = DH / 8, RPB = 256 / (DH * 2), KS = DH / 16, DB = DH / 32, ROWB = DH * 2;
+    const int hh = (threadIdx.x & 63) >> 5;
+    const int qw = q0 + wid * 32;
+    const int q = qw + (threadIdx.x & 31);
+    (void)dev_word;
+    if (qw >= L) return;
+    f32x16 o[DB];
+    auto lds_bases = [&](const float*& bb, const char* (&kb)[KS], const char* (&vb)[DB]) {
+        int lane = threadIdx.x & 63;
+        asm volatile("" : "+v"(lane));
+        const int ql = lane & 31, hh = lane >> 5;
+        int qc = q0 + wid * 32 + ql;
+        qc = qc < L ? qc : L - 1;
+        const int bc = (4 - (qc & 3)) & 3;
+        bb = Bs + bc * bst + attn_bias_off(bc) + (Lk - qc - bc) + 4 * hh;
+        const int krow_sw = ((ql / RPB) & (CPR - 1));
+#pragma unroll
+        for (int ks = 0; ks < KS; ++ks) kb[ks] = Ks + ql * ROWB + (((2 * ks + hh) ^ krow_sw) << 4);
+        const int g16 = lane >> 4, q_ = (lane & 15) >> 2, p_ = lane & 3;
+        const int vsw = (DH == 64) ? (((q_ >> 1) & 1) << 2) : 0;
+#pragma unroll
+        for (int d = 0; d < DB; ++d) {
+            const int col = 32 * d + 16 * (g16 & 1) + 4 * p_;
+            vb[d] = Vs + (4 * hh + q_) * ROWB + (((col >> 3) ^ vsw) << 4) + ((p_ & 1) << 3);
+        }
+    };
+    typedef __attribute__((address_space(3))) s16x4 lds_s16x4;
+    typedef short s16x8 __attribute__((ext_vector_type(8)));
+    f32x4 lsum;
+    const s16x4 one4 = s16x4{0x3f80, 0x3f80, 0x3f80, 0x3f80};
+    const int nkt = Lk >> 5;
+    const int nfull = (L & 31) ? nkt - 1 : nkt;
+    float l_tot;
+
+    bool redo = false;
+#ifdef ARX_DEV_VARIANTS
+    redo = dev_word == 6;
+#endif
+    if (!redo) {
+#pragma unroll
+        for (int d = 0; d < DB; ++d)
+#pragma unroll
+            for (int r = 0; r < 16; ++r) o[d][r] = 0.f;
+        lsum = f32x4{0.f, 0.f, 0.f, 0.f};
+        typedef const __attribute__((address_space(3))) char* lds_cptr;
+        typedef const __attribute__((address_space(3))) float* lds_fptr;
+        lds_fptr bp;
+        lds_cptr kp[KS], vp[DB];
+        {
+            const float* bb;
+            const char* kb[KS];
+            const char* vb[DB];
+            lds_bases(bb, kb, vb);
+            bp = (lds_fptr)bb;
+#pragma unroll
+            for (int ks = 0; ks < KS; ++ks) kp[ks] = (lds_cptr)kb[ks];
+#pragma unroll
+            for (int d = 0; d < DB; ++d) vp[d] = (lds_cptr)vb[d];
+        }
+        bf16x8 kf[KS];
+#pragma unroll
+        for (int ks = 0; ks < KS; ++ks) kf[ks] = *reinterpret_cast<const __attribute__((address_space(3))) bf16x8*>(kp[ks]);
+        auto advance = [&](int n) {
+            bp += 32 * n;
+            asm volatile("" : "+v"(bp));
+#pragma unroll
+            for (int ks = 0; ks < KS; ++ks) { kp[ks] += 32 * ROWB * n; asm volatile("" : "+v"(kp[ks])); }
+#pragma unroll
+            for (int d = 0; d < DB; ++d) { vp[d] += 32 * ROWB * n; asm volatile("" : "+v"(vp[d])); }
+            __builtin_amdgcn_sched_barrier(0);
+        };
+        auto fast = [&](auto masked_tag, auto off_tag, int kt) {
+            constexpr bool MASKED = decltype(masked_tag)::value;
+            constexpr int OFF = decltype(off_tag)::value;
+            f32x16 s;
+#pragma unroll
+            for (int r = 0; r < 16; ++r) s[r] = 0.f;
+#pragma unroll
+            for (int ks = 0; ks < KS; ++ks) s = __builtin_amdgcn_mfma_f32_32x32x16_bf16(kf[ks], qf[ks], s, 0, 0, 0);
+            __builtin_amdgcn_sched_barrier(0);
+            f32x4 bv[4];
+#pragma unroll
+            for (int g4 = 0; g4 < 4; ++g4) bv[g4] = HAS_BIAS ? *reinterpret_cast<const __attribute__((address_space(3))) f32x4*>(bp + OFF * 32 + 8 * g4) : f32x4{0.f, 0.f, 0.f, 0.f};
+            s16x4 vt[DB][4];
+#pragma unroll
+            for (int d = 0; d < DB; ++d)
+#pragma unroll
+                for (int j = 0; j < 4; ++j) vt[d][j] = __builtin_amdgcn_ds_read_tr16_b64_v4i16((lds_s16x4*)(vp[d] + (OFF * 32 + 8 * j) * ROWB));
+            __builtin_amdgcn_sched_barrier(0);
+            typedef float f32x2 __attribute__((ext_vector_type(2)));
+            const f32x2 sc2 = f32x2{scale_log2e, scale_log2e};
+#pragma unroll
+            for (int g4 = 0; g4 < 4; ++g4)
+#pragma unroll
+                for (int e = 0; e < 4; e += 2) {
+                    f32x2 v = __builtin_elementwise_fma(f32x2{s[g4 * 4 + e], s[g4 * 4 + e + 1]}, sc2, f32x2{bv[g4][e], bv[g4][e + 1]});
+                    if (MASKED) {
+                        v[0] = (kt * 32 + 8 * g4 + 4 * hh + e < L) ? v[0] : -INFINITY;
+                        v[1] = (kt * 32 + 8 * g4 + 4 * hh + e + 1 < L) ? v[1] : -INFINITY;
+                    }
+                    s[g4 * 4 + e] = v[0]; s[g4 * 4 + e + 1] = v[1];
+                }
+            __builtin_amdgcn_sched_barrier(0);
+#pragma unroll
+            for (int r = 0; r < 16; ++r) s[r] = __builtin_amdgcn_exp2f(s[r]);
+            uint32_t pw[8];
+#pragma unroll
+            for (int j = 0; j < 8; ++j) pw[j] = pack_bf16x2(s[2 * j], s[2 * j + 1]);
+            __builtin_amdgcn_sched_barrier(0);
+            if (!MASKED) {
+#pragma unroll
+                for (int ks = 0; ks < KS; ++ks) kf[ks] = *reinterpret_cast<const __attribute__((address_space(3))) bf16x8*>(kp[ks] + (OFF + 1) * 32 * ROWB);
+            }
+            __builtin_amdgcn_sched_barrier(0);
+            bf16x8 pf[2];
+#pragma unroll
+            for (int ss = 0; ss < 2; ++ss) pf[ss] = __builtin_bit_cast(bf16x8, u32x4{pw[4 * ss], pw[4 * ss + 1], pw[4 * ss + 2], pw[4 * ss + 3]});
+#pragma unroll
+            for (int j = 0; j < 4; ++j)
+                lsum = __builtin_amdgcn_mfma_f32_4x4x4bf16_1k(one4, __builtin_bit_cast(s16x4, u32x2{pw[2 * j], pw[2 * j + 1]}), lsum, 0, 0, 0);
+#pragma unroll
+            for (int d = 0; d < DB; ++d)
+#pragma unroll
+                for (int ss = 0; ss < 2; ++ss) {
+                    s16x8 v8;
+#pragma unroll
+                    for (int e = 0; e < 4; ++e) { v8[e] = vt[d][2 * ss][e]; v8[4 + e] = vt[d][2 * ss + 1][e]; }
+                    o[d] = __builtin_amdgcn_mfma_f32_32x32x16_bf16(__builtin_bit_cast(bf16x8, v8), pf[ss], o[d], 0, 0, 0);
+                }
+            __builtin_amdgcn_sched_barrier(0);
+        };
+        int kt = 0;
+        for (; kt + 2 <= nfull; kt += 2) {
+            fast(std::false_type{}, std::integral_constant<int, 0>{}, kt);
+            fast(std::false_type{}, std::integral_constant<int, 1>{}, kt + 1);
+            advance(2);
+        }
+        if (kt < nfull) { fast(std::false_type{}, std::integral_constant<int, 0>{}, kt); advance(1); }
+        if (nfull < nkt) fast(std::true_type{}, std::integral_constant<int, 0>{}, nkt - 1);
+        l_tot = lsum[0] + __shfl_xor(lsum[0], 32);
+        redo = !__all(l_tot > 0x1p-100f && l_tot < 0x1p100f);
+    }
+    if (redo) {
+#pragma unroll
+    for (int d = 0; d < DB; ++d)
+#pragma unroll
+        for (int r = 0; r < 16; ++r) o[d][r] = 0.f;
+    float m_run = -INFINITY;
+    const float* bptr;
+    const char* kptr[KS];
+    const char* vptr[DB];
+    lds_bases(bptr, kptr, vptr);
+    constexpr float THR = 8.0f;
+    const float inv_scale = 1.0f / scale_log2e;
+    lsum = f32x4{0.f, 0.f, 0.f, 0.f};
+    auto tile = [&](auto masked_tag, auto first_tag, int kt) {
+        constexpr bool MASKED = decltype(masked_tag)::value;
+        constexpr bool FIRST = decltype(first_tag)::value;
+        f32x16 s;
+        const float s0 = FIRST ? 0.f : -m_run * inv_scale;
+#pragma unroll
+        for (int r = 0; r < 16; ++r) s[r] = s0;
+#pragma unroll
+        for (int ks = 0; ks < KS; ++ks) {
+            const bf16x8 kf = *reinterpret_cast<const bf16x8*>(kptr[ks]);
+            s = __builtin_amdgcn_mfma_f32_32x32x16_bf16(kf, qf[ks], s, 0, 0, 0);
+        }
+#pragma unroll
+        for (int g4 = 0; g4 < 4; ++g4) {
+            f32x4 bv = f32x4{0.f, 0.f, 0.f, 0.f};
+            if (HAS_BIAS) bv = *reinterpret_cast<const f32x4*>(bptr + 8 * g4);
+#pragma unroll
+            for (int e = 0; e < 4; ++e) {
+                float v = fmaf(s[g4 * 4 + e], scale_log2e, bv[e]);
+                if (MASKED) v = (kt * 32 + 8 * g4 + 4 * hh + e < L) ? v : -INFINITY;
+                s[g4 * 4 + e] = v;
+            }
+        }
+        float mx = -INFINITY;
+#pragma unroll
+        for (int r = 0; r < 16; r += 2) mx = fmaxf(mx, fmaxf(s[r], s[r + 1]));
+        mx = fmaxf(mx, __shfl_xor(mx, 32));
+        if (FIRST) {
+            m_run = mx;
+#pragma unroll
+            for (int r = 0; r < 16; ++r) s[r] -= mx;
+        } else if (__any(mx > THR)) {
+            const float d = fmaxf(mx, 0.f);
+            const float alpha = __builtin_amdgcn_exp2f(-d);
+            m_run += d;
+#pragma unroll
+            for (int r = 0; r < 16; ++r) s[r] -= d;
+#pragma unroll
+            for (int r = 0; r < 4; ++r) lsum[r] *= alpha;
+#pragma unroll
+            for (int dd = 0; dd < DB; ++dd)
+#pragma unroll
+                for (int r = 0; r < 16; ++r) o[dd][r] *= alpha;
+        }
+#pragma unroll
+        for (int r = 0; r < 16; ++r) s[r] = __builtin_amdgcn_exp2f(s[r]);
+        uint32_t pw[8];
+#pragma unroll
+        for (int j = 0; j < 8; ++j) pw[j] = pack_bf16x2(s[2 * j], s[2 * j + 1]);
+        bf16x8 pf[2];
+#pragma unroll
+        for (int ss = 0; ss < 2; ++ss) pf[ss] = __builtin_bit_cast(bf16x8, u32x4{pw[4 * ss], pw[4 * ss + 1], pw[4 * ss + 2], pw[4 * ss + 3]});
+#pragma unroll
+        for (int j = 0; j < 4; ++j)
+            lsum = __builtin_amdgcn_mfma_f32_4x4x4bf16_1k(one4, __builtin_bit_cast(s16x4, u32x2{pw[2 * j], pw[2 * j + 1]}), lsum, 0, 0, 0);
+#pragma unroll
+        for (int d = 0; d < DB; ++d) {
+#pragma unroll
+            for (int ss = 0; ss < 2; ++ss) {
+                const s16x4 lo = __builtin_amdgcn_ds_read_tr16_b64_v4i16((lds_s16x4*)(vptr[d] + (16 * ss) * ROWB));
+                const s16x4 hi = __builtin_amdgcn_ds_read_tr16_b64_v4i16((lds_s16x4*)(vptr[d] + (16 * ss + 8) * ROWB));
+                s16x8 v8;
+#pragma unroll
+                for (int e = 0; e < 4; ++e) { v8[e] = lo[e]; v8[4 + e] = hi[e]; }
+                o[d] = __builtin_amdgcn_mfma_f32_32x32x16_bf16(__builtin_bit_cast(bf16x8, v8), pf[ss], o[d], 0, 0, 0);
+            }
+        }
+        bptr += 32;
+#pragma unroll
+        for (int ks = 0; ks < KS; ++ks) kptr[ks] += 32 * ROWB;
+#pragma unroll
+        for (int d = 0; d < DB; ++d) vptr[d] += 32 * ROWB;
+    };
+    if (nfull > 0) tile(std::false_type{}, std::true_type{}, 0); else tile(std::true_type{}, std::true_type{}, 0);
+    for (int kt = 1; kt < nfull; ++kt) tile(std::false_type{}, std::false_type{}, kt);
+    if (nfull < nkt && nkt > 1) tile(std::true_type{}, std::false_type{}, nkt - 1);
+    l_tot = lsum[0] + __shfl_xor(lsum[0], 32);
+    }
+
+    const float inv = 1.0f / l_tot;
+    u32x4 pc[DB][2];
+#pragma unroll
+    for (int d = 0; d < DB; ++d) {
+        uint32_t w[4][2];
+#pragma unroll
+        for (int g4 = 0; g4 < 4; ++g4) {
+            w[g4][0] = pack_bf16x2(o[d][g4 * 4 + 0] * inv, o[d][g4 * 4 + 1] * inv);
+            w[g4][1] = pack_bf16x2(o[d][g4 * 4 + 2] * inv, o[d][g4 * 4 + 3] * inv);
+        }
+#pragma unroll
+        for (int g = 0; g < 2; ++g)
+#pragma unroll
+            for (int k = 0; k < 2; ++k) {
+                const auto sw = __builtin_amdgcn_permlane32_swap(w[g][k], w[g + 2][k], false, false);
+                pc[d][g][k] = sw[0]; pc[d][g][2 + k] = sw[1];
+            }
+    }
+    if (q < L) {
+        uint16_t* orow = ctx + (int64_t)(t0 + q) * H + h * DH + 16 * hh;
+#pragma unroll
+        for (int d = 0; d < DB; ++d) {
+            *reinterpret_cast<u32x4*>(orow + d * 32) = pc[d][0];
+            *reinterpret_cast<u32x4*>(orow + d * 32 + 8) = pc[d][1];
+        }
+    }
+}
+
 template <int DH, bool HAS_BIAS, int NW>
 __global__ __launch_bounds__(NW * 64, NW / 2) void attention_tr_kernel(const uint16_t* __restrict__ qkv, uint16_t* __restrict__ ctx,
                                                                         const int32_t* __restrict__ cu,
@@ -384,16 +661,7 @@
             __builtin_amdgcn_global_load_lds((gbl_v*)(Vg + gr + vc * 8), (lds_v*)(Vs + lo), 16, 0, 0);
         }
     }
-    if (HAS_BIAS) {
-        const float* bt = bias_tbl + (int64_t)h * ARX_BIAS_ROW + ARX_BIAS_CENTER;
-        const int span = 2 * Lk + 8;
-        for (int i = tid; i < 4 * span; i += NT) {
-            const int c = (i >= span) + (i >= 2 * span) + (i >= 3 * span), j = i - c * span;
-            int d = j + c - Lk;
-            d = d < -ARX_BIAS_CENTER ? -ARX_BIAS_CENTER : (d > ARX_BIAS_CENTER ? ARX_BIAS_CENTER : d);
-            Bs[c * bst + attn_bias_off(c) + j] = bt[d];
-        }
-    }
+    if (HAS_BIAS) attention_tr_stage_bias<NT>(Bs, bst, bias_tbl, h, Lk, tid);
     __syncthreads();
 #ifdef ARX_DEV_VARIANTS
     if (dev_stamps && threadIdx.x == 0) dev_stamps[4 * lin + 1] = wall_clock64();
@@ -403,261 +671,7 @@
     }
 #endif
 
-    if (qw >= L) return;
-    f32x16 o[DB];
-    auto lds_bases = [&](const float*& bb, const char* (&kb)[KS], const char* (&vb)[DB]) {
-        int lane = threadIdx.x & 63;
-        asm volatile("" : "+v"(lane));
-        const int ql = lane & 31, hh = lane >> 5;
-        int qc = q0 + wid * 32 + ql;
-        qc = qc < L ? qc : L - 1;
-        const int bc = (4 - (qc & 3)) & 3;
-        bb = Bs + bc * bst + attn_bias_off(bc) + (Lk - qc - bc) + 4 * hh;
-        const int krow_sw = ((ql / RPB) & (CPR - 1));
-#pragma unroll
-        for (int ks = 0; ks < KS; ++ks) kb[ks] = Ks + ql * ROWB + (((2 * ks + hh) ^ krow_sw) << 4);
-        const int g16 = lane >> 4, q_ = (lane & 15) >> 2, p_ = lane & 3;
-        const int vsw = (DH == 64) ? (((q_ >> 1) & 1) << 2) : 0;
-#pragma unroll
-        for (int d = 0; d < DB; ++d) {
-            const int col = 32 * d + 16 * (g16 & 1) + 4 * p_;
-            vb[d] = Vs + (4 * hh + q_) * ROWB + (((col >> 3) ^ vsw) << 4) + ((p_ & 1) << 3);
-        }
-    };
-    typedef __attribute__((address_space(3))) s16x4 lds_s16x4;
-    typedef short s16x8 __attribute__((ext_vector_type(8)));
-    f32x4 lsum;
-    const s16x4 one4 = s16x4{0x3f80, 0x3f80, 0x3f80, 0x3f80};
-    const int nkt = Lk >> 5;
-    const int nfull = (L & 31) ? nkt - 1 : nkt;
-    float l_tot;
-
-    bool redo = false;
-#ifdef ARX_DEV_VARIANTS
-    redo = dev_word == 6;
-#endif
-    if (!redo) {
-#pragma unroll
-        for (int d = 0; d < DB; ++d)
-#pragma unroll
-            for (int r = 0; r < 16; ++r) o[d][r] = 0.f;
-        lsum = f32x4{0.f, 0.f, 0.f, 0.f};
-        typedef const __attribute__((address_space(3))) char* lds_cptr;
-        typedef const __attribute__((address_space(3))) float* lds_fptr;
-        lds_fptr bp;
-        lds_cptr kp[KS], vp[DB];
-        {
-            const float* bb;
-            const char* kb[KS];
-            const char* vb[DB];
-            lds_bases(bb, kb, vb);
-            bp = (lds_fptr)bb;
-#pragma unroll
-            for (int ks = 0; ks < KS; ++ks) kp[ks] = (lds_cptr)kb[ks];
-#pragma unroll
-            for (int d = 0; d < DB; ++d) vp[d] = (lds_cptr)vb[d];
-        }
-        bf16x8 kf[KS];
-#pragma unroll
-        for (int ks = 0; ks < KS; ++ks) kf[ks] = *reinterpret_cast<const __attribute__((address_space(3))) bf16x8*>(kp[ks]);
-        auto advance = [&](int n) {
-            bp += 32 * n;
-            asm volatile("" : "+v"(bp));
-#pragma unroll
-            for (int ks = 0; ks < KS; ++ks) { kp[ks] += 32 * ROWB * n; asm volatile("" : "+v"(kp[ks])); }
-#pragma unroll
-            for (int d = 0; d < DB; ++d) { vp[d] += 32 * ROWB * n; asm volatile("" : "+v"(vp[d])); }
-            __builtin_amdgcn_sched_barrier(0);
-        };
-        auto fast = [&](auto masked_tag, auto off_tag, int kt) {
-            constexpr bool MASKED = decltype(masked_tag)::value;
-            constexpr int OFF = decltype(off_tag)::value;
-            f32x16 s;
-#pragma unroll
-            for (int r = 0; r < 16; ++r) s[r] = 0.f;
-#pragma unroll
-            for (int ks = 0; ks < KS; ++ks) s = __builtin_amdgcn_mfma_f32_32x32x16_bf16(kf[ks], qf[ks], s, 0, 0, 0);
-            __builtin_amdgcn_sched_barrier(0);
-            f32x4 bv[4];
-#pragma unroll
-            for (int g4 = 0; g4 < 4; ++g4) bv[g4] = HAS_BIAS ? *reinterpret_cast<const __attribute__((address_space(3))) f32x4*>(bp + OFF * 32 + 8 * g4) : f32x4{0.f, 0.f, 0.f, 0.f};
-            s16x4 vt[DB][4];
-#pragma unroll
-            for (int d = 0; d < DB; ++d)
-#pragma unroll
-                for (int j = 0; j < 4; ++j) vt[d][j] = __builtin_amdgcn_ds_read_tr16_b64_v4i16((lds_s16x4*)(vp[d] + (OFF * 32 + 8 * j) * ROWB));
-            __builtin_amdgcn_sched_barrier(0);
-            typedef float f32x2 __attribute__((ext_vector_type(2)));
-            const f32x2 sc2 = f32x2{scale_log2e, scale_log2e};
-#pragma unroll
-            for (int g4 = 0; g4 < 4; ++g4)
-#pragma unroll
-                for (int e = 0; e < 4; e += 2) {
-                    f32x2 v = __builtin_elementwise_fma(f32x2{s[g4 * 4 + e], s[g4 * 4 + e + 1]}, sc2, f32x2{bv[g4][e], bv[g4][e + 1]});
-                    if (MASKED) {
-                        v[0] = (kt * 32 + 8 * g4 + 4 * hh + e < L) ? v[0] : -INFINITY;
-                        v[1] = (kt * 32 + 8 * g4 + 4 * hh + e + 1 < L) ? v[1] : -INFINITY;
-                    }
-                    s[g4 * 4 + e] = v[0]; s[g4 * 4 + e + 1] = v[1];
-                }
-            __builtin_amdgcn_sched_barrier(0);
-#pragma unroll
-            for (int r = 0; r < 16; ++r) s[r] = __builtin_amdgcn_exp2f(s[r]);
-            uint32_t pw[8];
-#pragma unroll
-            for (int j = 0; j < 8; ++j) pw[j] = pack_bf16x2(s[2 * j], s[2 * j + 1]);
-            __builtin_amdgcn_sched_barrier(0);
-            if (!MASKED) {
-#pragma unroll
-                for (int ks = 0; ks < KS; ++ks) kf[ks] = *reinterpret_cast<const __attribute__((address_space(3))) bf16x8*>(kp[ks] + (OFF + 1) * 32 * ROWB);
-            }
-            __builtin_amdgcn_sched_barrier(0);
-            bf16x8 pf[2];
-#pragma unroll
-            for (int ss = 0; ss < 2; ++ss) pf[ss] = __builtin_bit_cast(bf16x8, u32x4{pw[4 * ss], pw[4 * ss + 1], pw[4 * ss + 2], pw[4 * ss + 3]});
-#pragma unroll
-            for (int j = 0; j < 4; ++j)
-                lsum = __builtin_amdgcn_mfma_f32_4x4x4bf16_1k(one4, __builtin_bit_cast(s16x4, u32x2{pw[2 * j], pw[2 * j + 1]}), lsum, 0, 0, 0);
-#pragma unroll
-            for (int d = 0; d < DB; ++d)
-#pragma unroll
-                for (int ss = 0; ss < 2; ++ss) {
-                    s16x8 v8;
-#pragma unroll
-                    for (int e = 0; e < 4; ++e) { v8[e] = vt[d][2 * ss][e]; v8[4 + e] = vt[d][2 * ss + 1][e]; }
-                    o[d] = __builtin_amdgcn_mfma_f32_32x32x16_bf16(__builtin_bit_cast(bf16x8, v8), pf[ss], o[d], 0, 0, 0);
-                }
-            __builtin_amdgcn_sched_barrier(0);
-        };
-        int kt = 0;
-        for (; kt + 2 <= nfull; kt += 2) {
-            fast(std::false_type{}, std::integral_constant<int, 0>{}, kt);
-            fast(std::false_type{}, std::integral_constant<int, 1>{}, kt + 1);
-            advance(2);
-        }
-        if (kt < nfull) { fast(std::false_type{}, std::integral_constant<int, 0>{}, kt); advance(1); }
-        if (nfull < nkt) fast(std::true_type{}, std::integral_constant<int, 0>{}, nkt - 1);
-        l_tot = lsum[0] + __shfl_xor(lsum[0], 32);
-        redo = !__all(l_tot > 0x1p-100f && l_tot < 0x1p100f);
-    }
-    if (redo) {
-#pragma unroll
-    for (int d = 0; d < DB; ++d)
-#pragma unroll
-        for (int r = 0; r < 16; ++r) o[d][r] = 0.f;
-    float m_run = -INFINITY;
-    const float* bptr;
-    const char* kptr[KS];
-    const char* vptr[DB];
-    lds_bases(bptr, kptr, vptr);
-    constexpr float THR = 8.0f;
-    const float inv_scale = 1.0f / scale_log2e;
-    lsum = f32x4{0.f, 0.f, 0.f, 0.f};
-    auto tile = [&](auto masked_tag, auto first_tag, int kt) {
-        constexpr bool MASKED = decltype(masked_tag)::value;
-        constexpr bool FIRST = decltype(first_tag)::value;
-        f32x16 s;
-        const float s0 = FIRST ? 0.f : -m_run * inv_scale;
-#pragma unroll
-        for (int r = 0; r < 16; ++r) s[r] = s0;
-#pragma unroll
-        for (int ks = 0; ks < KS; ++ks) {
-            const bf16x8 kf = *reinterpret_cast<const bf16x8*>(kptr[ks]);
-            s = __builtin_amdgcn_mfma_f32_32x32x16_bf16(kf, qf[ks], s, 0, 0, 0);
-        }
-#pragma unroll
-        for (int g4 = 0; g4 < 4; ++g4) {
-            f32x4 bv = f32x4{0.f, 0.f, 0.f, 0.f};
-            if (HAS_BIAS) bv = *reinterpret_cast<const f32x4*>(bptr + 8 * g4);
-#pragma unroll
-            for (int e = 0; e < 4; ++e) {
-                float v = fmaf(s[g4 * 4 + e], scale_log2e, bv[e]);
-                if (MASKED) v = (kt * 32 + 8 * g4 + 4 * hh + e < L) ? v : -INFINITY;
-                s[g4 * 4 + e] = v;
-            }
-        }
-        float mx = -INFINITY;
-#pragma unroll
-        for (int r = 0; r < 16; r += 2) mx = fmaxf(mx, fmaxf(s[r], s[r + 1]));
-        mx = fmaxf(mx, __shfl_xor(mx, 32));
-        if (FIRST) {
-            m_run = mx;
-#pragma unroll
-            for (int r = 0; r < 16; ++r) s[r] -= mx;
-        } else if (__any(mx > THR)) {
-            const float d = fmaxf(mx, 0.f);
-            const float alpha = __builtin_amdgcn_exp2f(-d);
-            m_run += d;
-#pragma unroll
-            for (int r = 0; r < 16; ++r) s[r] -= d;
-#pragma unroll
-            for (int r = 0; r < 4; ++r) lsum[r] *= alpha;
-#pragma unroll
-            for (int dd = 0; dd < DB; ++dd)
-#pragma unroll
-                for (int r = 0; r < 16; ++r) o[dd][r] *= alpha;
-        }
-#pragma unroll
-        for (int r = 0; r < 16; ++r) s[r] = __builtin_amdgcn_exp2f(s[r]);
-        uint32_t pw[8];
-#pragma unroll
-        for (int j = 0; j < 8; ++j) pw[j] = pack_bf16x2(s[2 * j], s[2 * j + 1]);
-        bf16x8 pf[2];
-#pragma unroll
-        for (int ss = 0; ss < 2; ++ss) pf[ss] = __builtin_bit_cast(bf16x8, u32x4{pw[4 * ss], pw[4 * ss + 1], pw[4 * ss + 2], pw[4 * ss + 3]});
-#pragma unroll
-        for (int j = 0; j < 4; ++j)
-            lsum = __builtin_amdgcn_mfma_f32_4x4x4bf16_1k(one4, __builtin_bit_cast(s16x4, u32x2{pw[2 * j], pw[2 * j + 1]}), lsum, 0, 0, 0);
-#pragma unroll
-        for (int d = 0; d < DB; ++d) {
-#pragma unroll
-            for (int ss = 0; ss < 2; ++ss) {
-                const s16x4 lo = __builtin_amdgcn_ds_read_tr16_b64_v4i16((lds_s16x4*)(vptr[d] + (16 * ss) * ROWB));
-                const s16x4 hi = __builtin_amdgcn_ds_read_tr16_b64_v4i16((lds_s16x4*)(vptr[d] + (16 * ss + 8) * ROWB));
-                s16x8 v8;
-#pragma unroll
-                for (int e = 0; e < 4; ++e) { v8[e] = lo[e]; v8[4 + e] = hi[e]; }
-                o[d] = __builtin_amdgcn_mfma_f32_32x32x16_bf16(__builtin_bit_cast(bf16x8, v8), pf[ss], o[d], 0, 0, 0);
-            }
-        }
-        bptr += 32;
-#pragma unroll
-        for (int ks = 0; ks < KS; ++ks) kptr[ks] += 32 * ROWB;
-#pragma unroll
-        for (int d = 0; d < DB; ++d) vptr[d] += 32 * ROWB;
-    };
-    if (nfull > 0) tile(std::false_type{}, std::true_type{}, 0); else tile(std::true_type{}, std::true_type{}, 0);
-    for (int kt = 1; kt < nfull; ++kt) tile(std::false_type{}, std::false_type{}, kt);
-    if (nfull < nkt && nkt > 1) tile(std::true_type{}, std::false_type{}, nkt - 1);
-    l_tot = lsum[0] + __shfl_xor(lsum[0], 32);
-    }
-
-    const float inv = 1.0f / l_tot;
-    u32x4 pc[DB][2];
-#pragma unroll
-    for (int d = 0; d < DB; ++d) {
-        uint32_t w[4][2];
-#pragma unroll
-        for (int g4 = 0; g4 < 4; ++g4) {
-            w[g4][0] = pack_bf16x2(o[d][g4 * 4 + 0] * inv, o[d][g4 * 4 + 1] * inv);
-            w[g4][1] = pack_bf16x2(o[d][g4 * 4 + 2] * inv, o[d][g4 * 4 + 3] * inv);
-        }
-#pragma unroll
-        for (int g = 0; g < 2; ++g)
-#pragma unroll
-            for (int k = 0; k < 2; ++k) {
-                const auto sw = __builtin_amdgcn_permlane32_swap(w[g][k], w[g + 2][k], false, false);
-                pc[d][g][k] = sw[0]; pc[d][g][2 + k] = sw[1];
-            }
-    }
-    if (q < L) {
-        uint16_t* orow = ctx + (int64_t)(t0 + q) * H + h * DH + 16 * hh;
-#pragma unroll
-        for (int d = 0; d < DB; ++d) {
-            *reinterpret_cast<u32x4*>(orow + d * 32) = pc[d][0];
-            *reinterpret_cast<u32x4*>(orow + d * 32 + 8) = pc[d][1];
-        }
-    }
+    attention_tr_body<DH, HAS_BIAS>(qf, Ks, Vs, Bs, bst, L, Lk, q0, wid, ctx, t0, H, h, scale_log2e, dev_word);
 #ifdef ARX_DEV_VARIANTS
     if (dev_stamps && (threadIdx.x & 63) == 0) atomicMax(&dev_stamps[4 * lin + 2], (unsigned long long)wall_clock64());
 #endif
diff --git a/arxiv_rag_amd/csrc/qkv_attention.h b/arxiv_rag_amd/csrc/qkv_attention.h
--- /dev/null
+++ b/arxiv_rag_amd/csrc/qkv_attention.h
@@ -0,0 +1,234 @@
+#pragma once
+#include "encoder_kernels.h"
+#include "gemm8.h"
+
+struct QkvAttnSmem {
+    static constexpr int A_HALF = 128 * 128, B0_HALF = 128 * 128, B1_HALF = 64 * 128;
+    static constexpr int A_OFF = 0, B0_OFF = 2 * A_HALF, B1_OFF = B0_OFF + B0_HALF, BUF_BYTES = B1_OFF + B1_HALF;
+    static constexpr int STAGE_OFF = 2 * BUF_BYTES;
+    static constexpr int BIAS_OFF = STAGE_OFF + 4 * 1024;
+    static constexpr int TILE = 256 * 128;
+    static constexpr int KS_OFF = 0, VS_OFF = TILE, QS_OFF = 2 * TILE;
+    static_assert(3 * TILE <= STAGE_OFF, "Q, K, V must fit the k-tile buffers");
+    static constexpr int total(bool has_bias) { return BIAS_OFF + (has_bias ? 4 * AttnSmem3<64>::bias_stride(256) * 4 : 0); }
+};
+
+template <int DH, bool HAS_BIAS, bool LN>
+__global__ __launch_bounds__(512) void qkv_attention_kernel(const uint16_t* __restrict__ x, const uint16_t* __restrict__ W,
+                                                             const float* __restrict__ bias, const float* __restrict__ s_vec,
+                                                             const float* __restrict__ a_mean, const float* __restrict__ a_rstd,
+                                                             uint16_t* __restrict__ ctx, const int32_t* __restrict__ cu,
+                                                             const float* __restrict__ bias_tbl, int H, int heads, int n_seqs,
+                                                             float scale_log2e, uint16_t* __restrict__ dev_qkv) {
+    static_assert(DH == 64, "one head slice is 3 x 64 W rows");
+    using S = QkvAttnSmem;
+    using ML = Gemm8Phase<bf16_t, 0>;
+    using vec = bf16x8;
+    extern __shared__ __attribute__((aligned(16))) char smem[];
+    const int xcd = blockIdx.x & 7, pos = blockIdx.x >> 3;
+    const int b = (pos / heads) * 8 + xcd, hd = pos % heads;
+    if (b >= n_seqs) return;
+    const int t0 = cu[b];
+    const int L = cu[b + 1] - t0;
+    if (L <= 0) return;
+    const int Lk = (L + 31) & ~31;
+    const int tid = threadIdx.x, lane = tid & 63, wid = __builtin_amdgcn_readfirstlane(tid >> 6);
+    const int wr = wid >> 2, wc = wid & 3;
+    const int K = H, nk = K >> 6;
+
+    {
+        char* stage = smem + S::STAGE_OFF;
+        if (LN) {
+            const int r = (wid & 3) * 64 + lane;
+            const float* src = (wid < 4 ? a_mean : a_rstd) + t0 + (r < L ? r : L - 1);
+            __builtin_amdgcn_global_load_lds((gbl_void_t*)src, (lds_void_t*)(stage + (wid < 4 ? 2048 : 3072) + (wid & 3) * 256), 4, 0, 0);
+        }
+        if (wid == 0 || (LN && wid == 1)) {
+            const int l = lane < 48 ? lane : lane - 16;
+            const float* src = (wid == 0 ? bias : s_vec) + (l >> 4) * H + hd * DH + (l & 15) * 4;
+            __builtin_amdgcn_global_load_lds((gbl_void_t*)src, (lds_void_t*)(stage + wid * 1024), 16, 0, 0);
+        }
+    }
+
+    f32x4 acc[3][8];
+#pragma unroll
+    for (int j = 0; j < 3; ++j)
+#pragma unroll
+        for (int i = 0; i < 8; ++i) acc[j][i] = f32x4{0.f, 0.f, 0.f, 0.f};
+    uint32_t aoff[2][2], b0off[2], b1off;
+#pragma unroll
+    for (int it = 0; it < 2; ++it) {
+        const int cid = it * 512 + tid, r = cid >> 3, c = (cid & 7) ^ ((r >> 1) & 7);
+#pragma unroll
+        for (int hf = 0; hf < 2; ++hf) {
+            int row = (r >> 6) * 128 + hf * 64 + (r & 63);
+            row = row < L ? row : L - 1;
+            aoff[hf][it] = ((uint32_t)(t0 + row) * (uint32_t)H + c * 8) * 2u;
+        }
+        const int rho = r & 31;
+        b0off[it] = ((uint32_t)((rho >> 4) * H + hd * DH + (r >> 5) * 16 + (rho & 15)) * (uint32_t)H + c * 8) * 2u;
+        if (it == 0) b1off = ((uint32_t)(2 * H + hd * DH + (r >> 4) * 16 + (r & 15)) * (uint32_t)H + c * 8) * 2u;
+    }
+    char* const wave_dst = smem + wid * 1024;
+    const __amdgpu_buffer_rsrc_t rsA = __builtin_amdgcn_make_buffer_rsrc((void*)x, 0, 0xffffffff, 0x00020000);
+    const __amdgpu_buffer_rsrc_t rsW = __builtin_amdgcn_make_buffer_rsrc((void*)W, 0, 0xffffffff, 0x00020000);
+    auto issue_a = [&](int hf, int kt, int buf) {
+        char* dst = wave_dst + buf * S::BUF_BYTES + S::A_OFF + hf * S::A_HALF;
+        __builtin_amdgcn_raw_ptr_buffer_load_lds(rsA, (lds_void_t*)dst, 16, aoff[hf][0], kt * 128, 0, 0);
+        __builtin_amdgcn_raw_ptr_buffer_load_lds(rsA, (lds_void_t*)(dst + 8192), 16, aoff[hf][1], kt * 128, 0, 0);
+    };
+    auto issue_b0 = [&](int kt, int buf) {
+        char* dst = wave_dst + buf * S::BUF_BYTES + S::B0_OFF;
+        __builtin_amdgcn_raw_ptr_buffer_load_lds(rsW, (lds_void_t*)dst, 16, b0off[0], kt * 128, 0, 0);
+        __builtin_amdgcn_raw_ptr_buffer_load_lds(rsW, (lds_void_t*)(dst + 8192), 16, b0off[1], kt * 128, 0, 0);
+    };
+    auto issue_b1 = [&](int kt, int buf) {
+        __builtin_amdgcn_raw_ptr_buffer_load_lds(rsW, (lds_void_t*)(wave_dst + buf * S::BUF_BYTES + S::B1_OFF), 16, b1off, kt * 128, 0, 0);
+    };
+    const int frow = lane & 15, fq = lane >> 4, sw = (lane >> 1) & 7;
+    const int fo0 = frow * 128 + (((0 + fq) ^ sw) << 4), fo1 = frow * 128 + (((4 + fq) ^ sw) << 4);
+    const int a_row = wr * 64 * 128;
+    vec af[4][2], wf0[2][2], wf1[2];
+    auto read_a = [&](const char* buf, int hf) {
+        const char* p = buf + S::A_OFF + hf * S::A_HALF + a_row;
+#pragma unroll
+        for (int i = 0; i < 4; ++i) {
+            af[i][0] = *reinterpret_cast<const vec*>(p + i * 2048 + fo0);
+            af[i][1] = *reinterpret_cast<const vec*>(p + i * 2048 + fo1);
+        }
+    };
+    auto read_b0 = [&](const char* buf) {
+        const char* p = buf + S::B0_OFF + wc * 32 * 128;
+#pragma unroll
+        for (int j = 0; j < 2; ++j) {
+            wf0[j][0] = *reinterpret_cast<const vec*>(p + j * 2048 + fo0);
+            wf0[j][1] = *reinterpret_cast<const vec*>(p + j * 2048 + fo1);
+        }
+    };
+    auto read_b1 = [&](const char* buf) {
+        const char* p = buf + S::B1_OFF + wc * 16 * 128;
+        wf1[0] = *reinterpret_cast<const vec*>(p + fo0);
+        wf1[1] = *reinterpret_cast<const vec*>(p + fo1);
+    };
+    auto quad_qk = [&](int hf) {
+        __builtin_amdgcn_s_setprio(1);
+#pragma unroll
+        for (int ks = 0; ks < 2; ++ks)
+#pragma unroll
+            for (int j = 0; j < 2; ++j)
+#pragma unroll
+                for (int i = 0; i < 4; ++i) acc[j][hf * 4 + i] = Mfma<bf16_t>::mma(wf0[j][ks], af[i][ks], acc[j][hf * 4 + i]);
+        __builtin_amdgcn_s_setprio(0);
+    };
+    auto quad_v = [&](int hf) {
+        __builtin_amdgcn_s_setprio(1);
+#pragma unroll
+        for (int ks = 0; ks < 2; ++ks)
+#pragma unroll
+            for (int i = 0; i < 4; ++i) acc[2][hf * 4 + i] = Mfma<bf16_t>::mma(wf1[ks], af[i][ks], acc[2][hf * 4 + i]);
+        __builtin_amdgcn_s_setprio(0);
+    };
+
+    issue_b0(0, 0); issue_a(0, 0, 0); issue_b1(0, 0); issue_a(1, 0, 0);
+    issue_b0(1, 1); issue_a(0, 1, 1); issue_b1(1, 1);
+    const int bst = AttnSmem3<DH>::bias_stride(Lk);
+    float* const Bs = reinterpret_cast<float*>(smem + S::BIAS_OFF);
+    if (HAS_BIAS) attention_tr_stage_bias<512>(Bs, bst, bias_tbl, hd, Lk, tid);
+    wait_vmcnt<5>();
+    ML::bar();
+    if (wr == 1) ML::bar();
+
+    for (int kt = 0; kt < nk; ++kt) {
+        const int pb = kt & 1;
+        const char* cur = smem + pb * S::BUF_BYTES;
+        const bool more1 = kt + 1 < nk, more2 = kt + 2 < nk;
+        read_b0(cur);
+        __builtin_amdgcn_sched_barrier(0);
+        read_a(cur, 0);
+        if (more1) issue_a(1, kt + 1, pb ^ 1);
+        asm volatile("s_waitcnt lgkmcnt(8)" ::: "memory");
+        ML::bar();
+        asm volatile("s_waitcnt lgkmcnt(0)" ::: "memory");
+        quad_qk(0);
+        ML::bar();
+        read_b1(cur);
+        if (more2) issue_b0(kt + 2, pb);
+        ML::bar();
+        asm volatile("s_waitcnt lgkmcnt(0)" ::: "memory");
+        quad_v(0);
+        ML::bar();
+        read_a(cur, 1);
+        if (more2) issue_a(0, kt + 2, pb);
+        ML::bar();
+        asm volatile("s_waitcnt lgkmcnt(0)" ::: "memory");
+        quad_v(1);
+        ML::bar();
+        if (more2) { issue_b1(kt + 2, pb); wait_vmcnt<5>(); }
+        else wait_vmcnt<0>();
+        ML::bar();
+        quad_qk(1);
+        if (more1 || wr == 0) ML::bar();
+    }
+    ML::bar();
+
+    {
+        const int mq = lane & 15, q = lane >> 4;
+        const float* sf = reinterpret_cast<const float*>(smem + S::STAGE_OFF);
+        const int chunk = wc * 2 + (q >> 1), sub = (q & 1) * 8;
+#pragma unroll
+        for (int part = 0; part < 3; ++part) {
+            const f32x4 b4 = *reinterpret_cast<const f32x4*>(sf + part * 64 + wc * 16 + q * 4);
+            const f32x2 bb[2] = {f32x2{b4[0], b4[1]}, f32x2{b4[2], b4[3]}};
+            f32x2 ss[2] = {f32x2{0.f, 0.f}, f32x2{0.f, 0.f}};
+            if (LN) {
+                const f32x4 s4 = *reinterpret_cast<const f32x4*>(sf + 256 + part * 64 + wc * 16 + q * 4);
+                ss[0] = f32x2{s4[0], s4[1]}; ss[1] = f32x2{s4[2], s4[3]};
+            }
+            char* tile = smem + (part == 0 ? S::QS_OFF : (part == 1 ? S::KS_OFF : S::VS_OFF));
+#pragma unroll
+            for (int i = 0; i < 8; ++i) {
+                const int rb = wr * 128 + i * 16 + mq;
+                const f32x4 a4 = acc[part][i];
+                f32x2 vv[2] = {f32x2{a4[0], a4[1]}, f32x2{a4[2], a4[3]}};
+                if (LN) {
+                    const float am = sf[512 + rb], ar = sf[768 + rb];
+                    const f32x2 nm = f32x2{-am, -am}, rs = f32x2{ar, ar};
+#pragma unroll
+                    for (int pi = 0; pi < 2; ++pi) vv[pi] = rs * (nm * ss[pi] + vv[pi]) + bb[pi];
+                } else {
+#pragma unroll
+                    for (int pi = 0; pi < 2; ++pi) vv[pi] = vv[pi] + bb[pi];
+                }
+                const u32x2 o = u32x2{pack_bf16x2(vv[0].x, vv[0].y), pack_bf16x2(vv[1].x, vv[1].y)};
+                const int swz = part == 2 ? (((rb >> 1) & 1) << 2) : (part == 1 ? ((rb >> 1) & 7) : (rb & 7));
+                *reinterpret_cast<u32x2*>(tile + rb * 128 + ((chunk ^ swz) << 4) + sub) = o;
+            }
+        }
+    }
+    __syncthreads();
+#ifdef ARX_DEV_VARIANTS
+    if (dev_qkv) {
+        for (int idx = tid; idx < 3 * 256 * 8; idx += 512) {
+            const int part = idx >> 11, row = (idx >> 3) & 255, c = idx & 7;
+            const int swz = part == 2 ? (((row >> 1) & 1) << 2) : (part == 1 ? ((row >> 1) & 7) : (row & 7));
+            const char* tile = smem + (part == 0 ? S::QS_OFF : (part == 1 ? S::KS_OFF : S::VS_OFF));
+            if (row < L)
+                *reinterpret_cast<u32x4*>(dev_qkv + (int64_t)(t0 + row) * 3 * H + part * H + hd * DH + c * 8) =
+                    *reinterpret_cast<const u32x4*>(tile + row * 128 + ((c ^ swz) << 4));
+        }
+        return;
+    }
+#else
+    (void)dev_qkv;
+#endif
+
+    if (wid * 32 >= L) return;
+    const int ql = lane & 31, hh = lane >> 5;
+    int qc = wid * 32 + ql;
+    qc = qc < L ? qc : L - 1;
+    bf16x8 qf[DH / 16];
+#pragma unroll
+    for (int ks = 0; ks < DH / 16; ++ks)
+        qf[ks] = *reinterpret_cast<const bf16x8*>(smem + S::QS_OFF + qc * 128 + (((2 * ks + hh) ^ (qc & 7)) << 4));
+    attention_tr_body<DH, HAS_BIAS>(qf, smem + S::KS_OFF, smem + S::VS_OFF, Bs, bst, L, Lk, 0, wid, ctx, t0, H, hd, scale_log2e, 0);
+}
diff --git a/arxiv_rag_amd/encoder.py b/arxiv_rag_amd/encoder.py
--- a/arxiv_rag_amd/encoder.py
+++ b/arxiv_rag_amd/encoder.py
@@ -87,6 +87,15 @@
         self._handle = h
         self._cap = (max_tokens, max_seqs)
         self._low_latency = False
+
+    def set_fused_attention(self, mode: int):
+        _lib.check(self.lib.arx_encoder_set_fused_attention(self._handle, int(mode)), "arx_encoder_set_fused_attention")
+
+    def last_ctx(self, n_tokens: int) -> torch.Tensor:
+        dst = torch.empty((n_tokens, self.cfg.hidden), dtype=torch.bfloat16, device=self.device)
+        _lib.check(self.lib.arx_encoder_debug_ctx(self._handle, dst.data_ptr(), n_tokens, torch.cuda.current_stream().cuda_stream),
+                   "arx_encoder_debug_ctx")
+        return dst
 
     def close(self):
         if getattr(self, "_handle", None) is not None and self._handle.value:
diff --git a/include/arx.h b/include/arx.h
--- a/include/arx.h
+++ b/include/arx.h
@@ -81,6 +81,9 @@
 int32_t arx_encoder_debug_hidden(arx_encoder* h, int32_t layer_slot, float* dst, int32_t n_tokens, void* stream);
 
 int32_t arx_encoder_set_low_latency(arx_encoder* h, int32_t on);
+
+int32_t arx_encoder_set_fused_attention(arx_encoder* h, int32_t on);
+int32_t arx_encoder_debug_ctx(arx_encoder* h, void* dst, int32_t n_tokens, void* stream);
 
 int32_t arx_encoder_set_tap(arx_encoder* h, int32_t layer);
 
@@ -243,7 +246,8 @@
 #define ARX_K_SEARCH_SELECT   9
 #define ARX_K_SEARCH_RESCORE 10
 #define ARX_K_GEMM_RAW       11
-#define ARX_K_CLASSES        12
+#define ARX_K_QKV_ATTENTION 12
+#define ARX_K_CLASSES        13
 int32_t arx_prof_enable(int32_t on);
 int32_t arx_prof_classes(uint32_t mask);
 int32_t arx_prof_reset(void);
```

New measurement: 22360 (median of 6 runs). No clear change (+0.9%).
